# BoloniniD/CSWin-UNet

Hardware: AMD Instinct MI355X
Metric: training images/sec (224x224, cswin_tiny) (higher is better)
Workload: dtype f32; 1 GPU; cswin_tiny_224_lite, synthetic 224x224 9-class, bs=24/GPU, fp32 matmul, fwd + 0.4CE+0.6Dice + bwd + SGD(momentum) step, drop_path 0.2; global_batch=24, img_size=224, parallelism=dp1, hip_graph=True

## Files before the change

### cswin_unet_amd/_lib.py

```python
import ctypes
import os
from ctypes import c_char_p, c_double, c_float, c_int, c_long, c_size_t, c_void_p

import torch

_HERE = os.path.dirname(os.path.abspath(__file__))
LIB_PATH = os.path.join(_HERE, "libcswin_hip.so")

P, I, F, SZ, L, D = c_void_p, c_int, c_float, c_size_t, c_long, c_double

ABI_VERSION = 4

SIGNATURES = {
    "cswin_last_error": (c_char_p, []),
    "cswin_abi_version": (I, []),
    "cswin_device_ok": (I, []),
    "cswin_attn_fwd": (I, [P, P, P, P, P, P, I, I, I, I, P, P, I, F, F, ctypes.c_ulonglong, P, I, P]),
    "cswin_attn_bwd_workspace": (SZ, [I, I, I, I, P, P, I]),
    "cswin_attn_bwd": (I, [P, P, P, P, P, P, P, P, P, P, SZ, I, I, I, I, P, P, I, F, P, F, ctypes.c_ulonglong, P, I, P]),
    "cswin_img2windows": (I, [P, P, I, I, I, I, I, I, P]),
    "cswin_windows2img": (I, [P, P, I, I, I, I, I, I, P]),
    "cswin_layernorm_fwd": (I, [P, P, P, P, P, P, I, I, F, I, P]),
    "cswin_layernorm_bwd_workspace": (SZ, [I, I]),
    "cswin_layernorm_bwd": (I, [P, P, P, P, P, P, P, P, P, P, SZ, I, I, P, P, P]),
    "cswin_linear_fwd": (I, [P, P, I, P, P, P, P, P, P, I, I, I, I, I, I, P]),
    "cswin_linear_bwd_data": (I, [P, P, P, P, I, P, P, I, P, I, I, I, I, I, P]),
    "cswin_linear_bwd_weight_workspace": (SZ, [I, I, I]),
    "cswin_linear_bwd_weight": (I, [P, P, P, I, P, I, P, P, P, SZ, I, I, I, P, I, P]),
    "cswin_linear_bwd_weight_batch": (I, [P, I, P, P, I, P]),
    "cswin_linear_bwd_tail": (I, [P, P, P, I, I, I, P, I, P, P, I, P]),
    "cswin_linear_bwd_weight_batch_masked": (I, [P, I, P, P, I, P, P, P]),
    "cswin_linear_bwd_tail_masked": (I, [P, P, P, I, I, I, P, I, P, P, I, P, P, P]),
    "cswin_rows_sum_multi": (I, [P, I, P]),
    "cswin_conv_tok_fwd": (I, [P, P, P, P, I, I, I, I, I, I, I, I, I, P]),
    "cswin_conv_tok_bwd_data": (I, [P, P, P, I, I, I, I, I, I, I, I, I, P]),
    "cswin_conv_tok_bwd_weight_workspace": (SZ, [I, I, I, I, I, I, I, I]),
    "cswin_conv_tok_bwd_weight": (I, [P, P, P, P, P, SZ, I, I, I, I, I, I, I, I, I, P, I, P]),
    "cswin_conv_weight_permute": (I, [P, P, P, I, I, I, I, P]),
    "cswin_conv_weight_unpermute": (I, [P, P, I, I, I, I, P]),
    "cswin_conv_weight_flipT": (I, [P, P, I, I, I, P]),
    "cswin_conv_weight_images": (I, [P, I, P]),
    "cswin_conv_tok_bwd_weight_cpad": (I, [P, P, P, P, P, SZ, I, I, I, I, I, I, I, I, I, P, I, P]),
    "cswin_nchw_to_tokens": (I, [P, P, I, I, I, I, I, P]),
    "cswin_tokens_to_nchw": (I, [P, P, I, I, I, I, I, P]),
    "cswin_carafe_fwd": (I, [P, P, P, P, P, I, I, I, I, I, P]),
    "cswin_carafe_bwd_workspace": (SZ, [I, I, I, I, I]),
    "cswin_carafe_bwd": (I, [P, P, P, P, P, P, P, SZ, I, I, I, I, I, P, P]),
    "cswin_carafe_fwd_nchw": (I, [P, P, P, P, P, I, I, I, I, I, I, P]),
    "cswin_carafe_bwd_nchw_ok": (I, [I, I, I, I]),
    "cswin_carafe_bwd_nchw": (I, [P, P, P, P, P, P, P, SZ, I, I, I, I, I, I, P, P]),
    "cswin_head_compose": (I, [P, P, P, P, P, I, I, I, I, P]),
    "cswin_head_compose_bwd": (I, [P, P, P, P, P, P, P, P, I, I, I, P]),
    "cswin_loss_workspace": (SZ, [I, I, L]),
    "cswin_loss_sums": (I, [P, P, P, P, SZ, I, I, L, I, P]),
    "cswin_loss_finalize": (I, [P, P, P, D, I, F, F, P, P]),
    "cswin_loss_bwd": (I, [P, P, P, P, P, F, F, I, I, L, I, P]),
    "cswin_cl_loss_workspace": (SZ, [I, I, L]),
    "cswin_cl_loss_sums": (I, [P, P, P, I, P, P, P, P, SZ, I, I, I, L, F, F, F, P]),
    "cswin_cl_loss_finalize": (I, [P, P, P, D, D, I, F, F, F, F, P]),
    "cswin_cl_loss_bwd": (I, [P, P, P, I, P, P, P, P, P, F, F, F, I, I, I, L, F, F, F, P]),
    "cswin_dropout": (I, [P, P, P, P, L, L, F, ctypes.c_ulonglong, P, P]),
    "cswin_sgd_flat": (I, [P, P, P, L, P, F, F, F, P, P]),
    "cswin_multi_copy": (I, [P, I, P]),
    "cswin_chunk_sumsq": (I, [P, P, P, I, P, P]),
    "cswin_norm_finalize": (I, [P, P, I, F, F, P, P, P]),
    "cswin_adamw_flat": (I, [P, P, P, P, P, I, P, P, P, D, D, D, F, F, D, D, P, P]),
    "cswin_rate_finalize": (I, [P, P, I, F, F, P, P, P, I, I, F, P, P, P, P, P]),
    "cswin_adam_flat": (I, [P, P, P, P, P, I, P, P, P, D, D, D, F, F, D, D, I, P, P]),
    "cswin_tpgm_chunk_stats": (I, [P, P, P, P, I, I, P, P]),
    "cswin_tpgm_finalize": (I, [P, P, I, I, P, P, P, P, D, D, D, D, I, P, P, P, P]),
    "cswin_tpgm_project": (I, [P, P, P, P, P, I, P, P]),
    "cswin_eb_tiles": (I, [P, P, I, P, P]),
    "cswin_eb_finalize": (I, [P, P, P, I, P, P]),
    "cswin_pack_bf16": (I, [P, P, L, P]),
    "cswin_pack_bf16_scaled": (I, [P, P, L, F, P]),
    "cswin_unpack_bf16": (I, [P, P, L, P]),
    "cswin_seg_metrics_nbins": (I, [I, I, I]),
    "cswin_seg_metrics_workspace": (SZ, [I, I, I, I, I]),
    "cswin_seg_metrics": (I, [P, P, P, P, P, SZ, I, I, I, I, I, P]),
    "cswin_components_workspace": (SZ, [I, I, I]),
    "cswin_components_label": (I, [P, P, P, P, SZ, I, I, I, I, P]),
    "cswin_components_filter": (I, [P, P, P, P, P, P, P, SZ, I, I, I, I, P]),
    "cswin_resize_banded": (I, [P, P, P, P, I, P, P, I, I, I, I, I, I, I, P]),
    "cswin_argmax_zoom_back": (I, [P, P, P, P, I, I, I, I, I, I, P]),
    "cswin_argmax_zoom_back_classes": (I, [P, P, P, P, P, I, I, I, I, I, I, I, P]),
    "cswin_class_counts": (I, [P, I, P, I, P, I, L, I, P]),
    "cswin_augment_gather": (I, [P, P, P, I, I, I, I, I, I, P]),
    "cswin_augment_labels": (I, [P, P, P, P, P, P, P, I, I, I, I, I, I, P]),
    "cswin_gaussian_blur": (I, [P, P, P, I, I, I, I, P]),
}



class WgradDesc(ctypes.Structure):
    _fields_ = [("dy", c_void_p), ("x", c_void_p), ("row_scale", c_void_p), ("dw", c_void_p), ("dbias", c_void_p),
                ("workspace", c_void_p), ("ws_bytes", c_size_t), ("rows_per_sample", c_int), ("M", c_int), ("N", c_int),
                ("K", c_int), ("precision", c_int), ("io_bf16", c_int)]


class ReduceJob(ctypes.Structure):
    _fields_ = [("part", c_void_p), ("out", c_void_p), ("out2", c_void_p), ("n_first", ctypes.c_longlong),
                ("n", ctypes.c_longlong), ("stride", ctypes.c_longlong), ("rows", c_int), ("reserved", c_int),
                ("conv_kk", c_int), ("conv_cin", c_int)]


class ConvImageJob(ctypes.Structure):
    _fields_ = [("w", c_void_p), ("w_perm", c_void_p), ("w_permT", c_void_p), ("w_flipT", c_void_p), ("Cout", c_int),
                ("Cin", c_int), ("ks", c_int), ("Cpad", c_int)]


class AugmentDesc(ctypes.Structure):
    _fields_ = [("kind", c_int), ("k", c_int), ("axis", c_int), ("src", c_int), ("map", c_void_p)]


_lib = None

PREC_FP32, PREC_BF16 = 0, 1
_state = {"precision": PREC_FP32, "act_bf16": True}


def precision():
    return _state["precision"]


def act_bf16():
    return _state["precision"] == PREC_BF16 and _state["act_bf16"]


def set_act_bf16(on):
    prev = _state["act_bf16"]
    _state["act_bf16"] = bool(on)
    return prev


_shadows = []


class _Shadow:

    def __init__(self, owner_obj, owner, seen):
        import weakref
        self.ref = weakref.ref(owner_obj)
        self.base, self.nbytes, self.seen = owner.data_ptr(), owner.numel() * 4, seen


def register_shadow(owner_obj, owner):
    _shadows[:] = [e for e in _shadows if e.ref() is not None and e.base != owner.data_ptr()]
    _shadows.append(_Shadow(owner_obj, owner, {p.data_ptr(): p._version for p in owner_obj.params}))


def shadow_ptr(w):
    if not _shadows or w is None:
        return None
    a = w.data_ptr()
    for e in _shadows:
        if e.base <= a < e.base + e.nbytes:
            opt = e.ref()
            if opt is None:
                return None
            if e.seen.get(a) != w._version:
                opt.refresh_shadow()
                e.seen.clear()
                e.seen.update({p.data_ptr(): p._version for p in opt.params})
                e.seen[a] = w._version
            return c_void_p(opt.flat_param16.data_ptr() + (a - e.base) // 2)
    return None


def shadows_current(opt):
    if _state["precision"] != PREC_BF16:
        return
    for e in _shadows:
        if e.ref() is opt:
            if any(e.seen.get(p.data_ptr()) != p._version for p in opt.params):
                opt.refresh_shadow()
                e.seen.clear()
                e.seen.update({p.data_ptr(): p._version for p in opt.params})
            return


def set_precision(mode):
    prev = _state["precision"]
    _state["precision"] = int(mode)
    if int(mode) == PREC_BF16 and prev != PREC_BF16:
        for e in _shadows:
            opt = e.ref()
            if opt is not None:
                opt.refresh_shadow()
    return prev


class CswinHipError(RuntimeError):
    pass


def lib():
    global _lib
    if _lib is None:
        if not os.path.exists(LIB_PATH):
            raise CswinHipError(f"{LIB_PATH} not found: build it with `python -c 'import __graft_entry__ as g; g.build()'` "
                                f"(or `make -C cswin_unet_amd/csrc`). There is no fallback path.")
        handle = ctypes.CDLL(LIB_PATH)
        for name, (res, args) in SIGNATURES.items():
            try:
                fn = getattr(handle, name)
            except AttributeError as e:
                raise CswinHipError(f"{LIB_PATH} does not export {name}") from e
            fn.restype, fn.argtypes = res, args
        have = handle.cswin_abi_version()
        if have != ABI_VERSION:
            raise CswinHipError(f"{LIB_PATH} was built for C ABI version {have}, this package binds version {ABI_VERSION}: rebuild it "
                                f"(`make -C cswin_unet_amd/csrc`)")
        _lib = handle
    return _lib


def call(name, *args):
    h = lib()
    rc = getattr(h, name)(*args)
    if rc != 0:
        raise CswinHipError(f"{name} failed ({rc}): {h.cswin_last_error().decode()}")


def ptr(t):
    return None if t is None else c_void_p(t.data_ptr())


def stream():
    return c_void_p(torch.cuda.current_stream().cuda_stream)


def dev_f32(t, what="tensor"):
    if t is None:
        return None
    if not t.is_cuda:
        raise CswinHipError(f"{what} is on {t.device}: the cswin_unet_amd ops run on a HIP device only (no CPU fallback)")
    if t.dtype != torch.float32:
        raise CswinHipError(f"{what} has dtype {t.dtype}; the HIP path computes in fp32")
    return t if t.is_contiguous() else t.contiguous()
```

### cswin_unet_amd/csrc/gemm.hip

```cpp
#include <stdlib.h>

#include <type_traits>
#include "common.h"
#include "gemm_epilogue.h"

int cswin_gemm16(int mode, int epi_mode, const void* A, const void* B, const void* epilogue, int M, int NO, int R, void* stream);
int cswin_wgrad16_batch(const cswin_wgrad_desc* d, int n, const int* splits, const int* rows_per_split, const cswin_reduce_job* pending,
                        int npending, void* stream, long long* stamps);

namespace {

constexpr int BKMAX = 64;

typedef __bf16 bf16x8 __attribute__((ext_vector_type(8)));

#define CSWIN_CHECK_PRECISION(p, who) CSWIN_REQUIRE((p) == 0 || (p) == 1, CSWIN_ERR_UNSUPPORTED, who ": precision %d (0 = fp32, 1 = bf16 operands)", (p))

struct PlainSrc {
    const float* p; long ld; int rows, cols;
    const float* row_scale; int rows_per_sample;
    int bf16;
    static constexpr bool fast_div = false;
    struct Row { const float* base; float s; };
    typedef int Col;
    __device__ Col col(int j) const { return j; }
    __device__ Row row(int i) const {
        Row r;
        r.base = (i < rows) ? p + (long)i * ld : nullptr;
        r.s = (row_scale && i < rows) ? row_scale[i / rows_per_sample] : 1.0f;
        return r;
    }
    __device__ const float* ptr(const Row& r, int j) const { return (r.base && j < cols) ? r.base + j : nullptr; }
};

template <class S> constexpr bool is_plain = std::is_same<S, PlainSrc>::value;
template <class S> __device__ __forceinline__ bool src_is_bf16(const S& s) {
    if constexpr (is_plain<S>) return s.bf16 != 0;
    else return false;
}
template <class S> __device__ __forceinline__ u32x2 src_load4_bf16(const S& s, const float* p) {
    if constexpr (is_plain<S>) return *reinterpret_cast<const u32x2*>(reinterpret_cast<const __bf16*>(s.p) + (p - s.p));
    else return u32x2{0u, 0u};
}
template <class S> __device__ __forceinline__ typename S::Row src_mapped_row(const S& s, int row, float f) {
    typename S::Row r{};
    if constexpr (is_plain<S>) {
        r.base = row >= 0 ? s.p + (long)row * s.ld : nullptr;
        r.s = f;
    }
    return r;
}
template <class S> __device__ __forceinline__ const float* src_row_scale(const S& s) {
    if constexpr (is_plain<S>) return s.row_scale;
    else return nullptr;
}

struct ConcatSrc {
    const float* p0; const float* p1; long ld0, ld1; int rows, cols, c0;
    static constexpr bool fast_div = false;
    struct Row { const float* b0; const float* b1; float s; };
    typedef int Col;
    __device__ Col col(int j) const { return j; }
    __device__ Row row(int i) const {
        Row r;
        r.b0 = (i < rows) ? p0 + (long)i * ld0 : nullptr;
        r.b1 = (i < rows) ? p1 + (long)i * ld1 : nullptr;
        r.s = 1.0f;
        return r;
    }
    __device__ const float* ptr(const Row& r, int j) const {
        if (!r.b0 || j >= cols) return nullptr;
        return j < c0 ? r.b0 + j : r.b1 + (j - c0);
    }
};

template <bool FAST> __device__ __forceinline__ int qdiv(int n, int d, unsigned m) {
    if constexpr (FAST) return fdiv1(n, m);
    else return n / d;
}
struct ConvMagics { unsigned img, w, c, ks, stride; };

template <bool FAST>
struct ConvSrcT {
    const float* x; int B, H, W, C, OH, OW, ks, stride, pad; int rows, cols;
    static constexpr bool fast_div = FAST;
    ConvMagics m;
    struct Row { int b, iy0, ix0; float s; };
    struct Col { int ky, kx, ci; };
    __device__ Row row(int i) const {
        Row r;
        r.s = 1.0f;
        if (i >= rows) { r.b = -1; r.iy0 = r.ix0 = 0; return r; }
        int ohw = OH * OW;
        r.b = qdiv<FAST>(i, ohw, m.img);
        int rem = i - r.b * ohw;
        int oy = qdiv<FAST>(rem, OW, m.w);
        r.iy0 = oy * stride - pad;
        r.ix0 = (rem - oy * OW) * stride - pad;
        return r;
    }
    __device__ Col col(int j) const {
        Col c;
        if (j >= cols) { c.ky = c.kx = 0; c.ci = -1; return c; }
        int tap = qdiv<FAST>(j, C, m.c);
        c.ci = j - tap * C;
        c.ky = qdiv<FAST>(tap, ks, m.ks);
        c.kx = tap - c.ky * ks;
        return c;
    }
    __device__ const float* ptr(const Row& r, const Col& c) const {
        if (r.b < 0 || c.ci < 0) return nullptr;
        int iy = r.iy0 + c.ky, ix = r.ix0 + c.kx;
        if ((unsigned)iy >= (unsigned)H || (unsigned)ix >= (unsigned)W) return nullptr;
        return x + ((long)(r.b * H + iy) * W + ix) * C + c.ci;
    }
};

template <bool FAST>
struct ConvTSrcT {
    const float* dy; int B, H, W, C, OH, OW, ks, stride, pad; int rows, cols;
    static constexpr bool fast_div = FAST;
    ConvMagics m;
    struct Row { int b, iy, ix; float s; };
    struct Col { int ky, kx, co; };
    __device__ Row row(int i) const {
        Row r;
        r.s = 1.0f;
        if (i >= rows) { r.b = -1; r.iy = r.ix = 0; return r; }
        int hw = H * W;
        r.b = qdiv<FAST>(i, hw, m.img);
        int rem = i - r.b * hw;
        r.iy = qdiv<FAST>(rem, W, m.w);
        r.ix = rem - r.iy * W;
        return r;
    }
    __device__ Col col(int j) const {
        Col c;
        if (j >= cols) { c.ky = c.kx = 0; c.co = -1; return c; }
        int tap = qdiv<FAST>(j, C, m.c);
        c.co = j - tap * C;
        c.ky = qdiv<FAST>(tap, ks, m.ks);
        c.kx = tap - c.ky * ks;
        return c;
    }
    __device__ const float* ptr(const Row& r, const Col& c) const {
        if (r.b < 0 || c.co < 0) return nullptr;
        int ty = r.iy + pad - c.ky, tx = r.ix + pad - c.kx;
        if (ty < 0 || tx < 0) return nullptr;
        int oy = qdiv<FAST>(ty, stride, m.stride), ox = qdiv<FAST>(tx, stride, m.stride);
        if (oy * stride != ty || ox * stride != tx || oy >= OH || ox >= OW) return nullptr;
        return dy + ((long)(r.b * OH + oy) * OW + ox) * C + c.co;
    }
};

template <bool FAST>
struct ConvTS2SrcT {
    const float* dy; int B, H, W, C, OH, OW, py, px, H2, W2, kys, kxs; int rows, cols;
    static constexpr bool fast_div = FAST;
    ConvMagics m;
    struct Row { int b, iy, ix; float s; };
    struct Col { int ky, kx, co; };
    __device__ Row row(int i) const {
        Row r;
        r.s = 1.0f;
        if (i >= rows) { r.b = -1; r.iy = r.ix = 0; return r; }
        const int hw = H2 * W2;
        r.b = qdiv<FAST>(i, hw, m.img);
        const int rem = i - r.b * hw;
        const int jy = qdiv<FAST>(rem, W2, m.w);
        r.iy = 2 * jy + py;
        r.ix = 2 * (rem - jy * W2) + px;
        return r;
    }
    __device__ Col col(int j) const {
        Col c;
        if (j >= cols) { c.ky = c.kx = 0; c.co = -1; return c; }
        const int t = qdiv<FAST>(j, C, m.c);
        c.co = j - t * C;
        c.ky = (kys >> (2 * t)) & 3;
        c.kx = (kxs >> (2 * t)) & 3;
        return c;
    }
    __device__ const float* ptr(const Row& r, const Col& c) const {
        if (r.b < 0 || c.co < 0) return nullptr;
        const int oy = (r.iy + 1 - c.ky) >> 1, ox = (r.ix + 1 - c.kx) >> 1;
        if (oy >= OH || ox >= OW) return nullptr;
        return dy + ((long)(r.b * OH + oy) * OW + ox) * C + c.co;
    }
};

template <bool FAST>
struct TapRowsSrcT {
    const float* w; int Cout, Cin, taps; int rows, cols;
    unsigned m_cout;
    struct Row { const float* base; float s; };
    typedef int Col;
    __device__ Row row(int i) const {
        Row r;
        r.s = 1.0f;
        if (i >= rows) { r.base = nullptr; return r; }
        const int t = qdiv<FAST>(i, Cout, m_cout), co = i - t * Cout;
        r.base = w + ((long)((taps >> (4 * t)) & 15) * Cout + co) * Cin;
        return r;
    }
    __device__ Col col(int j) const { return j; }
    __device__ const float* ptr(const Row& r, int j) const { return (r.base && j < cols) ? r.base + j : nullptr; }
};

template <int ROWS, int BK, bool RC_, int NTH>
struct OperandTile {
    static constexpr bool RC = RC_;
    static constexpr int LD = RC ? BK + 4 : ROWS + 4;
    static constexpr int ELEMS = (RC ? ROWS : BK) * LD;
    static constexpr int Q = ROWS * BK / (4 * NTH);
    static constexpr int CPR = RC ? BK / 4 : ROWS / 4;
    static constexpr int RPP = NTH / CPR;
    static_assert(Q >= 1, "tile too small for this many wave groups");
};

template <int BM_, int BN_, int BK_, int KW_, bool A_RC, bool B_RC>
struct Tile {
    static constexpr int BM = BM_, BN = BN_, BK = BK_, KW = KW_;
    static constexpr int WGM = BM >= 64 ? 2 : 1, WGN = BN >= 64 ? 2 : 1, NW = WGM * WGN;
    static constexpr int WM = BM / WGM, WN = BN / WGN;
    static constexpr int FM = WM / 32, FN = WN / 32;
    static constexpr int THREADS = 64 * NW * KW;
    typedef OperandTile<BM, BK, A_RC, THREADS> A;
    typedef OperandTile<BN, BK, B_RC, THREADS> B;
    static constexpr int LD16 = BK + 8;
    static constexpr int PATCH = FM * FN * 16 * 64;
    static constexpr int LDS_FLOATS = A::ELEMS + B::ELEMS > NW * EP_WAVE_FLOATS ? A::ELEMS + B::ELEMS : NW * EP_WAVE_FLOATS;
    static_assert((BK / KW) % 8 == 0, "tile too small for this many wave groups");
    static_assert(KW == 1 || (KW / 2) * NW * PATCH <= LDS_FLOATS, "LDS too small for the k-group reduction");
};

template <bool S16, bool SCALED> __device__ __forceinline__ u32x2 chunk_bf16(const f32x4& v, const u32x2& raw, float s) {
    if constexpr (S16 && !SCALED) return raw;
    else if constexpr (S16) return __builtin_bit_cast(u32x2, __builtin_convertvector(widen_bf16x4(raw) * s, bf16x4));
    else if constexpr (SCALED) return __builtin_bit_cast(u32x2, __builtin_convertvector(v * s, bf16x4));
    else return __builtin_bit_cast(u32x2, __builtin_convertvector(v, bf16x4));
}
template <int LD16> __device__ __forceinline__ void store_a_transposed(unsigned short* img16, int c, int row, u32x2 h) {
    unsigned short* col = &img16[4 * c * LD16 + row];
    col[0] = (unsigned short)(h[0] & 0xffffu);
    col[LD16] = (unsigned short)(h[0] >> 16);
    col[2 * LD16] = (unsigned short)(h[1] & 0xffffu);
    col[3 * LD16] = (unsigned short)(h[1] >> 16);
}
template <int BN> __device__ __forceinline__ void store_b_swizzled(unsigned short* img16, int c, int row, u32x2 h) {
    static_assert(BN == 64, "transposed-read B image is laid out for 64-column tiles");
    *reinterpret_cast<u32x2*>(&img16[row * BN + 8 * ((c >> 1) ^ (((row >> 1) & 1) << 2)) + 4 * (c & 1)]) = h;
}
template <class G, bool IS_A, int PREC, bool S16, bool SCALED, int LD16, int BN>
__device__ __forceinline__ void stash_operand(float* img, unsigned short* img16, int c, int r, const f32x4* p, const u32x2* p16, const float* ps) {
#pragma unroll
    for (int q = 0; q < G::Q; ++q) {
        const int row = r + q * G::RPP;
        float s = 1.0f;
        if constexpr (SCALED) s = ps[q];
        if constexpr (PREC == 1) {
            const u32x2 h = chunk_bf16<S16, SCALED>(p[q], p16[q], s);
            if constexpr (G::RC) *reinterpret_cast<u32x2*>(&img16[row * LD16 + 4 * c]) = h;
            else if constexpr (IS_A) store_a_transposed<LD16>(img16, c, row, h);
            else store_b_swizzled<BN>(img16, c, row, h);
        } else {
            f32x4 v = p[q];
            if constexpr (SCALED) v *= s;
            *reinterpret_cast<f32x4*>(&img[row * G::LD + 4 * c]) = v;
        }
    }
}
struct RowMask { const float* skip; int nsamples, rows_per_sample, splits; unsigned magic; };
constexpr int MASK_MAX_SAMPLES = 256;
struct KeptList { int n; int idx[MASK_MAX_SAMPLES]; float scale[MASK_MAX_SAMPLES]; };

__device__ __forceinline__ void build_kept_list(KeptList* kept, const RowMask& mk, const float* row_scale) {
    const int tid = threadIdx.x, lane = tid & 63;
    if (tid >= 64) return;
    int n = 0;
    for (int s0 = 0; s0 < mk.nsamples; s0 += 64) {
        const int s = s0 + lane;
        const bool keep = s < mk.nsamples && mk.skip[s] != 0.0f;
        const unsigned long long bal = __ballot(keep);
        if (keep) {
            const int at = n + __popcll(bal & ((1ull << lane) - 1ull));
            kept->idx[at] = s;
            kept->scale[at] = row_scale ? row_scale[s] : 1.0f;
        }
        n += __popcll(bal);
    }
    if (tid == 0) kept->n = n;
}

__device__ __forceinline__ void stamp(const Epilogue& epi, int row, int slot) {
    if (!epi.stamps || threadIdx.x != 0) return;
    long long* s = epi.stamps + 8L * row;
    s[slot] = __builtin_amdgcn_s_memtime();
    if (slot == 0) { s[4] = __builtin_amdgcn_s_getreg(6164); s[5] = __builtin_amdgcn_s_memrealtime(); }
    if (slot == 3) s[6] = __builtin_amdgcn_s_memrealtime();
}

template <class T, int VEC, int EPI, bool SCALE_A, int PREC, class ASrc, class BSrc, bool MASKED = false>
__device__ __forceinline__ void gemm_body(float* lds, const ASrc& A, const BSrc& B, const Epilogue& epi, int M, int N, int R,
                                          int r_per_split, int tiles_m, int tiles_n, int bid, int nblk, int stamp_row,
                                          const RowMask* mk = nullptr, KeptList* kept = nullptr) {
    typedef typename T::A TA;
    typedef typename T::B TB;
    constexpr int BM = T::BM, BN = T::BN, BK = T::BK, KW = T::KW, NW = T::NW, FM = T::FM, FN = T::FN, LD16 = T::LD16;
    constexpr bool A_RC = TA::RC, B_RC = TB::RC;
    float* As = lds;
    float* Bs = lds + TA::ELEMS;
    unsigned short* As16 = reinterpret_cast<unsigned short*>(lds);
    unsigned short* Bs16 = As16 + BM * LD16;
    static_assert(PREC == 0 || ((BM + BN) * LD16 * 2 <= T::LDS_FLOATS * 4 && (BK / KW) % 16 == 0), "bf16 tile does not fit");

    const int tid = threadIdx.x, lane = tid & 63, wave = (tid >> 6) % NW, kg = tid / (64 * NW);
    const int li = lane & 31, lh = lane >> 5;
    const int lb = xcd_block_order(bid, nblk);
    const int tiles = tiles_m * tiles_n;
    const int split = lb / tiles;
    const int tile = lb - split * tiles;
    const int m0 = (tile / tiles_n) * BM, n0 = (tile % tiles_n) * BN;
    if constexpr (MASKED) {
        static_assert(!A_RC && !B_RC && VEC == 4 && BM == BN && is_plain<ASrc> && is_plain<BSrc>,
                      "the sample mask serves weight gradients of plain matrices (one row mapping for both operands)");
        build_kept_list(kept, *mk, src_row_scale(A));
        __syncthreads();
        R = __builtin_amdgcn_readfirstlane(kept->n) * mk->rows_per_sample;
        r_per_split = ((R + mk->splits - 1) / mk->splits + 7) / 8 * 8;
    }
    const int r_begin = split * r_per_split;
    const int r_end = min(R, r_begin + r_per_split);
    const int wm0 = (wave / T::WGN) * T::WM, wn0 = (wave % T::WGN) * T::WN;

    const int a_c = tid % TA::CPR, a_r = tid / TA::CPR;
    const int b_c = tid % TB::CPR, b_r = tid / TB::CPR;

    typename ASrc::Row arow[TA::Q];
    typename BSrc::Row brow[TB::Q];
    if (A_RC) {
#pragma unroll
        for (int q = 0; q < TA::Q; ++q) arow[q] = A.row(m0 + a_r + q * TA::RPP);
    }
    if (B_RC) {
#pragma unroll
        for (int q = 0; q < TB::Q; ++q) brow[q] = B.row(n0 + b_r + q * TB::RPP);
    }

    const typename ASrc::Col acol = A.col(m0 + 4 * a_c);
    const typename BSrc::Col bcol = B.col(n0 + 4 * b_c);

    f32x4 pa[TA::Q], pb[TB::Q];
    u32x2 pa16[TA::Q], pb16[TB::Q];
    float pas[TA::Q];
    auto fetch = [&](int r0, auto a16, auto b16) {
        int mrow[TA::Q];
        float msc[TA::Q];
        if constexpr (MASKED) {
#pragma unroll
            for (int q = 0; q < TA::Q; ++q) {
                const int c = r0 + a_r + q * TA::RPP;
                mrow[q] = -1;
                msc[q] = 1.0f;
                if (c < r_end) {
                    const int j = fdiv1(c, mk->magic);
                    mrow[q] = kept->idx[j] * mk->rows_per_sample + (c - j * mk->rows_per_sample);
                    msc[q] = kept->scale[j];
                }
            }
        }
#pragma unroll
        for (int q = 0; q < TA::Q; ++q) {
            typename ASrc::Row rr;
            int j;
            if (A_RC) {
                rr = arow[q];
                j = r0 + 4 * a_c;
            } else {
                const int r = r0 + a_r + q * TA::RPP;
                if constexpr (MASKED) rr = src_mapped_row(A, mrow[q], msc[q]);
                else rr = A.row(r < r_end ? r : 0x7fffffff);
                j = m0 + 4 * a_c;
            }
            if (SCALE_A) pas[q] = rr.s;
            if (VEC == 4) {
                const float* p = A_RC ? (j < r_end ? A.ptr(rr, A.col(j)) : nullptr) : A.ptr(rr, acol);
                if constexpr (decltype(a16)::value) {
                    pa16[q] = u32x2{0u, 0u};
                    if (p) pa16[q] = src_load4_bf16(A, p);
                } else {
                    pa[q] = f32x4{0.f, 0.f, 0.f, 0.f};
                    if (p) pa[q] = *reinterpret_cast<const f32x4*>(p);
                }
            } else {
#pragma unroll
                for (int e = 0; e < 4; ++e) {
                    const float* p = (!A_RC || j + e < r_end) ? A.ptr(rr, A.col(j + e)) : nullptr;
                    pa[q][e] = p ? *p : 0.f;
                }
            }
        }
#pragma unroll
        for (int q = 0; q < TB::Q; ++q) {
            typename BSrc::Row rr;
            int j;
            if (B_RC) {
                rr = brow[q];
                j = r0 + 4 * b_c;
            } else {
                const int r = r0 + b_r + q * TB::RPP;
                if constexpr (MASKED) rr = src_mapped_row(B, mrow[q], 1.0f);
                else rr = B.row(r < r_end ? r : 0x7fffffff);
                j = n0 + 4 * b_c;
            }
            if (VEC == 4) {
                const float* p = B_RC ? (j < r_end ? B.ptr(rr, B.col(j)) : nullptr) : B.ptr(rr, bcol);
                if constexpr (decltype(b16)::value) {
                    pb16[q] = u32x2{0u, 0u};
                    if (p) pb16[q] = src_load4_bf16(B, p);
                } else {
                    pb[q] = f32x4{0.f, 0.f, 0.f, 0.f};
                    if (p) pb[q] = *reinterpret_cast<const f32x4*>(p);
                }
            } else {
#pragma unroll
                for (int e = 0; e < 4; ++e) {
                    const float* p = (!B_RC || j + e < r_end) ? B.ptr(rr, B.col(j + e)) : nullptr;
                    pb[q][e] = p ? *p : 0.f;
                }
            }
        }
    };
    auto stash = [&](auto a16, auto b16) {
        stash_operand<TA, true, PREC, decltype(a16)::value, SCALE_A, LD16, BN>(As, As16, a_c, a_r, pa, pa16, pas);
        stash_operand<TB, false, PREC, decltype(b16)::value, false, LD16, BN>(Bs, Bs16, b_c, b_r, pb, pb16, nullptr);
    };

    f32x16 acc[FM][FN];
#pragma unroll
    for (int i = 0; i < FM; ++i)
#pragma unroll
        for (int j = 0; j < FN; ++j)
#pragma unroll
            for (int e = 0; e < 16; ++e) acc[i][j][e] = 0.f;

    float csum = 0.f;
    const bool do_colsum = !A_RC && epi.colsum && n0 == 0 && tid < BM;

    stamp(epi, stamp_row, 0);
    auto main_loop = [&](auto a16, auto b16) {
        fetch(r_begin, a16, b16);
        stash(a16, b16);
        __syncthreads();
        stamp(epi, stamp_row, 1);
        for (int r0 = r_begin; r0 < r_end; r0 += BK) {
            const bool more = r0 + BK < r_end;
            if (more) fetch(r0 + BK, a16, b16);
            if (do_colsum) {
                if constexpr (PREC == 1) {
#pragma unroll 8
                    for (int r = 0; r < BK; ++r)
                        csum += __builtin_bit_cast(float, (unsigned)As16[tid * LD16 + r] << 16);
                } else {
#pragma unroll 8
                    for (int r = 0; r < BK; ++r) csum += As[r * TA::LD + tid];
                }
            }
            if constexpr (PREC == 1) {
#pragma unroll
                for (int kk = kg * (BK / KW); kk < (kg + 1) * (BK / KW); kk += 16) {
                    bf16x8 af[FM], bf[FN];
#pragma unroll
                    for (int i = 0; i < FM; ++i)
                        af[i] = *reinterpret_cast<const bf16x8*>(&As16[(wm0 + i * 32 + li) * LD16 + kk + 8 * lh]);
#pragma unroll
                    for (int j = 0; j < FN; ++j) {
                        if constexpr (B_RC) {
                            bf[j] = *reinterpret_cast<const bf16x8*>(&Bs16[(wn0 + j * 32 + li) * LD16 + kk + 8 * lh]);
                        } else {
                            typedef short s16x4 __attribute__((ext_vector_type(4)));
                            typedef short s16x8 __attribute__((ext_vector_type(8)));
                            typedef __attribute__((address_space(3))) s16x4 lds_s16x4;
                            const int col = wn0 + j * 32 + 16 * ((lane >> 4) & 1) + 4 * (lane & 3);
                            const int row = kk + 8 * lh + ((lane & 15) >> 2);
                            const int sw = ((row >> 1) & 1) << 2;
                            const unsigned short* a0 = &Bs16[row * BN + 8 * ((col >> 3) ^ sw) + (col & 7)];
                            const s16x4 v0 = __builtin_amdgcn_ds_read_tr16_b64_v4i16((lds_s16x4*)a0);
                            const s16x4 v1 = __builtin_amdgcn_ds_read_tr16_b64_v4i16((lds_s16x4*)(a0 + 4 * BN));
                            const s16x8 f = {v0[0], v0[1], v0[2], v0[3], v1[0], v1[1], v1[2], v1[3]};
                            bf[j] = __builtin_bit_cast(bf16x8, f);
                        }
                    }
#pragma unroll
                    for (int i = 0; i < FM; ++i)
#pragma unroll
                        for (int j = 0; j < FN; ++j)
                            acc[i][j] = __builtin_amdgcn_mfma_f32_32x32x16_bf16(af[i], bf[j], acc[i][j], 0, 0, 0);
                }
            } else
#pragma unroll
            for (int kk = kg * (BK / KW); kk < (kg + 1) * (BK / KW); kk += 8) {
                f32x4 af[FM], bf[FN];
#pragma unroll
                for (int i = 0; i < FM; ++i) {
                    if (A_RC) {
                        af[i] = *reinterpret_cast<const f32x4*>(&As[(wm0 + i * 32 + li) * TA::LD + kk + 4 * lh]);
                    } else {
#pragma unroll
                        for (int s = 0; s < 4; ++s) af[i][s] = As[(kk + 4 * lh + s) * TA::LD + wm0 + i * 32 + li];
                    }
                }
#pragma unroll
                for (int j = 0; j < FN; ++j) {
                    if (B_RC) {
                        bf[j] = *reinterpret_cast<const f32x4*>(&Bs[(wn0 + j * 32 + li) * TB::LD + kk + 4 * lh]);
                    } else {
#pragma unroll
                        for (int s = 0; s < 4; ++s) bf[j][s] = Bs[(kk + 4 * lh + s) * TB::LD + wn0 + j * 32 + li];
                    }
                }
#pragma unroll
                for (int s = 0; s < 4; ++s)
#pragma unroll
                    for (int i = 0; i < FM; ++i)
#pragma unroll
                        for (int j = 0; j < FN; ++j)
                            acc[i][j] = __builtin_amdgcn_mfma_f32_32x32x2f32(af[i][s], bf[j][s], acc[i][j], 0, 0, 0);
            }
            __syncthreads();
            if (more) {
                stash(a16, b16);
                __syncthreads();
            }
        }
    };
    if (r_begin < r_end) {
        constexpr bool CAN_A16 = PREC == 1 && A_RC && VEC == 4 && is_plain<ASrc>;
        constexpr bool CAN_B16 = PREC == 1 && A_RC && VEC == 4 && is_plain<BSrc>;
        const bool a_is16 = CAN_A16 && src_is_bf16(A), b_is16 = CAN_B16 && src_is_bf16(B);
        if constexpr (CAN_A16 && CAN_B16) {
            if (a_is16 && b_is16) main_loop(std::true_type{}, std::true_type{});
            else if (a_is16) main_loop(std::true_type{}, std::false_type{});
            else if (b_is16) main_loop(std::false_type{}, std::true_type{});
            else main_loop(std::false_type{}, std::false_type{});
        } else if constexpr (CAN_B16) {
            if (b_is16) main_loop(std::false_type{}, std::true_type{});
            else main_loop(std::false_type{}, std::false_type{});
        } else {
            main_loop(std::false_type{}, std::false_type{});
        }
    }

    stamp(epi, stamp_row, 2);
    if (KW > 1) {
#pragma unroll
        for (int half = KW / 2; half >= 1; half >>= 1) {
            if (kg >= half && kg < 2 * half) {
                float* dst = lds + ((kg - half) * NW + wave) * T::PATCH + lane;
#pragma unroll
                for (int i = 0; i < FM; ++i)
#pragma unroll
                    for (int j = 0; j < FN; ++j)
#pragma unroll
                        for (int g = 0; g < 16; ++g) dst[((i * FN + j) * 16 + g) * 64] = acc[i][j][g];
            }
            __syncthreads();
            if (kg < half) {
                const float* src = lds + (kg * NW + wave) * T::PATCH + lane;
#pragma unroll
                for (int i = 0; i < FM; ++i)
#pragma unroll
                    for (int j = 0; j < FN; ++j)
#pragma unroll
                        for (int g = 0; g < 16; ++g) acc[i][j][g] += src[((i * FN + j) * 16 + g) * 64];
            }
            __syncthreads();
        }
        if (kg != 0) return;
    }
    Epilogue e = epi;
    e.C += (long)split * e.split_stride;
    if constexpr (EPI == EPI_GELUBWD) {
        if (e.pre_bf16) run_epilogue<EPI, FM, FN, true>(e, acc, M, N, m0 + wm0, n0 + wn0, lane, lds + wave * EP_WAVE_FLOATS, e.vec_store != 0);
        else run_epilogue<EPI, FM, FN, false>(e, acc, M, N, m0 + wm0, n0 + wn0, lane, lds + wave * EP_WAVE_FLOATS, e.vec_store != 0);
    } else {
        if constexpr (ASrc::fast_div)
            run_epilogue<EPI, FM, FN, false, true>(e, acc, M, N, m0 + wm0, n0 + wn0, lane, lds + wave * EP_WAVE_FLOATS, e.vec_store != 0, A.m.img, A.m.w);
        else
            run_epilogue<EPI, FM, FN>(e, acc, M, N, m0 + wm0, n0 + wn0, lane, lds + wave * EP_WAVE_FLOATS, e.vec_store != 0);
    }
    stamp(epi, stamp_row, 3);
    if (do_colsum && m0 + tid < M) epi.colsum[(long)split * epi.colsum_stride + m0 + tid] = csum;
}

template <int BM, int BN, int BK, int KW, bool A_RC, bool B_RC, int VEC, int EPI, bool SCALE_A, int PREC, class ASrc, class BSrc>
__global__ __launch_bounds__((Tile<BM, BN, BK, KW, A_RC, B_RC>::THREADS)) void gemm_kernel(ASrc A, BSrc B, Epilogue epi, int M, int N, int R,
                                                    int r_per_split, int tiles_m, int tiles_n) {
    typedef Tile<BM, BN, BK, KW, A_RC, B_RC> T;
    __shared__ __attribute__((aligned(16))) float lds[T::LDS_FLOATS];
    gemm_body<T, VEC, EPI, SCALE_A, PREC, ASrc, BSrc>(lds, A, B, epi, M, N, R, r_per_split, tiles_m, tiles_n, (int)blockIdx.x, (int)gridDim.x,
                                                      (int)blockIdx.x);
}

constexpr int WGRAD_BATCH = 4;
template <class ASrc, class BSrc>
struct GemmBatch {
    ASrc A[WGRAD_BATCH];
    BSrc B[WGRAD_BATCH];
    Epilogue e[WGRAD_BATCH];
    int M[WGRAD_BATCH], N[WGRAD_BATCH], R[WGRAD_BATCH], rps[WGRAD_BATCH], tm[WGRAD_BATCH], tn[WGRAD_BATCH];
    int first[WGRAD_BATCH + 1];
    int n;
    RowMask mask[WGRAD_BATCH];
};
typedef GemmBatch<PlainSrc, PlainSrc> WgradBatch;

template <class ASrc, class BSrc> __device__ __forceinline__ int batch_problem(const GemmBatch<ASrc, BSrc>& b, int bid) {
    int p = 0;
    while (p + 1 < b.n && bid >= b.first[p + 1]) ++p;
    return p;
}
template <class T, bool SCALE_A, int PREC, bool MASKED = false, class ASrc, class BSrc>
__device__ __forceinline__ void batch_body(float* lds, const GemmBatch<ASrc, BSrc>& b, int p, int bid, KeptList* kept = nullptr) {
    gemm_body<T, 4, EPI_PLAIN, SCALE_A, PREC, ASrc, BSrc, MASKED>(lds, b.A[p], b.B[p], b.e[p], b.M[p], b.N[p], b.R[p], b.rps[p], b.tm[p], b.tn[p],
                                                                  bid - b.first[p], b.first[p + 1] - b.first[p], bid, MASKED ? &b.mask[p] : nullptr, kept);
}

typedef Tile<64, 64, 64, 2, false, false> WgradTile;
template <int PREC, bool MASKED>
__device__ __forceinline__ void wgrad_batch_body(float* lds, KeptList* kept, const WgradBatch& b, int bid) {
    const int p = batch_problem(b, bid);
    if constexpr (MASKED) {
        if (b.mask[p].skip) return batch_body<WgradTile, true, PREC, true>(lds, b, p, bid, kept);
    }
    batch_body<WgradTile, true, PREC>(lds, b, p, bid);
}

template <int PREC>
__global__ __launch_bounds__(WgradTile::THREADS) void gemm_wgrad_batch_kernel(WgradBatch b) {
    __shared__ __attribute__((aligned(16))) float lds[WgradTile::LDS_FLOATS];
    wgrad_batch_body<PREC, false>(lds, nullptr, b, (int)blockIdx.x);
}
__global__ __launch_bounds__(WgradTile::THREADS) void gemm_wgrad_batch_masked_kernel(WgradBatch b) {
    __shared__ __attribute__((aligned(16))) float lds[WgradTile::LDS_FLOATS];
    __shared__ KeptList kept;
    wgrad_batch_body<0, true>(lds, &kept, b, (int)blockIdx.x);
}

struct BlockTail {
    PlainSrc dA, dB;
    Epilogue de;
    int dM, dN, dR, drps, dtm, dtn, nd;
    WgradBatch w;
    ReduceRiders r;
};
typedef Tile<64, 64, 64, 2, true, false> TailDgradTile;
static_assert(TailDgradTile::THREADS == WgradTile::THREADS, "one workgroup size for both halves of the block tail");
constexpr int BLOCK_TAIL_LDS = TailDgradTile::LDS_FLOATS > WgradTile::LDS_FLOATS ? TailDgradTile::LDS_FLOATS : WgradTile::LDS_FLOATS;
template <bool MASKED>
__device__ __forceinline__ void block_tail_body(float (&lds)[BLOCK_TAIL_LDS], KeptList* kept, const BlockTail& t) {
    const int bid = (int)blockIdx.x, nw = t.w.first[t.w.n];
    if (bid >= nw + t.nd) {
        if (threadIdx.x >= 256) return;
        static_assert(sizeof(lds) >= sizeof(float) * RS_G * (RS_COLS + 1), "reduction scratch");
        rows_sum_dispatch(t.r.j, t.r.first_block, t.r.njobs, bid - nw - t.nd, reinterpret_cast<float(*)[RS_COLS + 1]>(lds));
        return;
    }
    if (bid >= nw) {
        gemm_body<TailDgradTile, 4, EPI_PLAIN, false, 0, PlainSrc, PlainSrc>(lds, t.dA, t.dB, t.de, t.dM, t.dN, t.dR, t.drps, t.dtm, t.dtn, bid - nw,
                                                                             t.nd, bid);
        return;
    }
    wgrad_batch_body<0, MASKED>(lds, kept, t.w, bid);
}
__global__ __launch_bounds__(WgradTile::THREADS) void gemm_block_tail_kernel(BlockTail t) {
    __shared__ __attribute__((aligned(16))) float lds[BLOCK_TAIL_LDS];
    block_tail_body<false>(lds, nullptr, t);
}
__global__ __launch_bounds__(WgradTile::THREADS) void gemm_block_tail_masked_kernel(BlockTail t) {
    __shared__ __attribute__((aligned(16))) float lds[BLOCK_TAIL_LDS];
    __shared__ KeptList kept;
    block_tail_body<true>(lds, &kept, t);
}

template <int KW> using S2DgradTile = Tile<64, 64, (KW == 1 ? 32 : 64), KW, true, false>;
template <int KW, int PREC, bool FAST>
__global__ __launch_bounds__(S2DgradTile<KW>::THREADS) void gemm_conv_s2_dgrad_batch_kernel(GemmBatch<ConvTS2SrcT<FAST>, TapRowsSrcT<FAST>> b) {
    __shared__ __attribute__((aligned(16))) float lds[S2DgradTile<KW>::LDS_FLOATS];
    batch_body<S2DgradTile<KW>, false, PREC>(lds, b, batch_problem(b, (int)blockIdx.x), (int)blockIdx.x);
}

template <int BM, int BN, int BK, int KW, bool A_RC, bool B_RC, int VEC, int EPI, bool SCALE_A, int PREC, class ASrc, class BSrc>
void launch_cfg(const ASrc& A, const BSrc& B, const Epilogue& epi, int M, int N, int R, int splits, int r_per_split,
                hipStream_t st) {
    int tm = cdiv(M, BM), tn = cdiv(N, BN);
    dim3 grid(tm * tn * splits);
    const int pad_lds = cswin_tuning().gemm_pad_lds;
    hipLaunchKernelGGL((gemm_kernel<BM, BN, BK, KW, A_RC, B_RC, VEC, EPI, SCALE_A, PREC, ASrc, BSrc>), grid, dim3((Tile<BM, BN, BK, KW, A_RC, B_RC>::THREADS)), pad_lds, st, A, B, epi,
                       M, N, R, r_per_split, tm, tn);
}

int k_groups(long blocks, int r_len) {
    if (blocks < 320 && r_len >= 512) return 4;
    if (blocks < 640 && r_len >= 256) return 2;
    return 1;
}

int one_split(int R) { return cdiv(R, BKMAX) * BKMAX; }

template <bool A_RC, bool B_RC, int VEC, int EPI, bool SCALE_A, class ASrc, class BSrc>
void launch_gemm(const ASrc& A, const BSrc& B, const Epilogue& epi_in, int M, int N, int R, int splits, int r_per_split,
                 int precision, hipStream_t st) {
    Epilogue epi = epi_in;
    epi.vec_store = epilogue_vec_ok(epi, N);
    auto blocks = [&](int bm, int bn) { return (long)cdiv(M, bm) * cdiv(N, bn) * splits; };
    const int forced_kw = cswin_tuning().gemm_kw;
    const int forced_tile = cswin_tuning().gemm_tile;
    const double pen2 = cswin_tuning().gemm_pen2;
    auto cost = [&](int bm, int bn, double pen) { return (double)((blocks(bm, bn) + 255) / 256) * bm * bn * pen; };
    int tile = 1;
    if (splits == 1 && cost(64, 32, pen2) < cost(64, 64, 1.0)) tile = 2;
    if (forced_tile) tile = forced_tile;
    const int r_len = r_per_split < R ? r_per_split : R;
    const bool wgrad = !A_RC && !B_RC;
    if (precision == 1) {
        if (k_groups(blocks(64, 64), r_len) >= 2 || (wgrad && r_len >= 256))
            launch_cfg<64, 64, 64, 2, A_RC, B_RC, VEC, EPI, SCALE_A, 1>(A, B, epi, M, N, R, splits, r_per_split, st);
        else launch_cfg<64, 64, 64, 1, A_RC, B_RC, VEC, EPI, SCALE_A, 1>(A, B, epi, M, N, R, splits, r_per_split, st);
        return;
    }
    if (tile == 2) {
        if (k_groups(blocks(64, 32), r_len) >= 2)
            return launch_cfg<64, 32, 64, 2, A_RC, B_RC, VEC, EPI, SCALE_A, 0>(A, B, epi, M, N, R, splits, r_per_split, st);
        return launch_cfg<64, 32, 32, 1, A_RC, B_RC, VEC, EPI, SCALE_A, 0>(A, B, epi, M, N, R, splits, r_per_split, st);
    }
    int kw = k_groups(blocks(64, 64), r_len);
    if (wgrad && r_len >= 256 && kw < 2) kw = 2;
    if (forced_kw) kw = forced_kw;
    if (kw == 4) launch_cfg<64, 64, 64, 4, A_RC, B_RC, VEC, EPI, SCALE_A, 0>(A, B, epi, M, N, R, splits, r_per_split, st);
    else if (kw == 2) launch_cfg<64, 64, 64, 2, A_RC, B_RC, VEC, EPI, SCALE_A, 0>(A, B, epi, M, N, R, splits, r_per_split, st);
    else launch_cfg<64, 64, 32, 1, A_RC, B_RC, VEC, EPI, SCALE_A, 0>(A, B, epi, M, N, R, splits, r_per_split, st);
}

template <bool A_RC, bool B_RC, int EPI, bool SCALE_A, class ASrc, class BSrc>
void launch_gemm_vec(bool vec, const ASrc& A, const BSrc& B, const Epilogue& epi, int M, int N, int R, int splits, int r_per_split,
                     int precision, hipStream_t st) {
    if (vec) launch_gemm<A_RC, B_RC, 4, EPI, SCALE_A>(A, B, epi, M, N, R, splits, r_per_split, precision, st);
    else launch_gemm<A_RC, B_RC, 1, EPI, SCALE_A>(A, B, epi, M, N, R, splits, r_per_split, precision, st);
}

long long* g_stamps = nullptr;

Epilogue plain_epilogue(float* C, long ldc) {
    Epilogue e = {};
    e.C = C;
    e.ldc = ldc;
    e.stamps = g_stamps;
    return e;
}

template <class ASrc, class BSrc>
void push(GemmBatch<ASrc, BSrc>& b, const ASrc& A, const BSrc& B, Epilogue e, int M, int N, int R, int rps, int splits) {
    const int i = b.n++;
    e.vec_store = epilogue_vec_ok(e, N);
    b.A[i] = A; b.B[i] = B; b.e[i] = e;
    b.M[i] = M; b.N[i] = N; b.R[i] = R; b.rps[i] = rps;
    b.tm[i] = cdiv(M, 64); b.tn[i] = cdiv(N, 64);
    b.first[i + 1] = b.first[i] + b.tm[i] * b.tn[i] * splits;
}

void choose_split(int M, int out_rows, int out_cols, int* splits, int* r_per_split, int target_override = 0) {
    const int target_env = cswin_tuning().gemm_split_wgs;
    const int target = target_override > 0 ? target_override : target_env;
    long tiles = (long)cdiv(out_rows, 64) * cdiv(out_cols, 64);
    int s = (int)(target / tiles);
    if (s < 1) s = 1;
    int max_s = cdiv(M, 2 * BKMAX);
    if (s > max_s) s = max_s;
    if (s < 1) s = 1;
    int rps = cdiv(cdiv(M, s), 8) * 8;
    *splits = cdiv(M, rps);
    *r_per_split = rps;
}

struct WgradSlabs {
    float* base; long stride; int N, K;
    WgradSlabs(void* workspace, int N_, int K_) : base((float*)workspace), stride(wgrad_slab_stride(N_, K_)), N(N_), K(K_) {}
    static size_t bytes(int M, int N, int K) {
        int s0, s1, rps;
        choose_split(M, N, K, &s0, &rps);
        choose_split(M, N, K, &s1, &rps, 1024);
        return (size_t)(s0 > s1 ? s0 : s1) * wgrad_slab_stride(N, K) * sizeof(float);
    }
    Epilogue epilogue(bool with_dbias) const {
        Epilogue e = plain_epilogue(base, K);
        e.split_stride = stride;
        e.colsum = with_dbias ? base + (long)N * K : nullptr;
        e.colsum_stride = (int)stride;
        return e;
    }
    cswin_reduce_job job(float* dw, float* dbias, int splits, int conv_kk = 0, int conv_cin = 0) const {
        const long nk = (long)N * K;
        return cswin_reduce_job{base, dw, dbias, nk, nk + (dbias ? N : 0), stride, splits, 0, conv_kk, conv_cin};
    }
};

int rows_sum_multi(const cswin_reduce_job* jobs, int njobs, void* stream) {
    CSWIN_REQUIRE(jobs && njobs > 0 && njobs <= CSWIN_MAX_REDUCE_JOBS, CSWIN_ERR_SHAPE, "rows_sum_multi: 1..%d jobs", CSWIN_MAX_REDUCE_JOBS);
    ReduceJobs J = {};
    const int blocks = fill_reduce_table(jobs, njobs, J.j, J.first_block);
    CSWIN_REQUIRE(blocks >= 0, CSWIN_ERR_SHAPE, "rows_sum_multi: bad job (part / out / n / rows, or conv_kk without conv_cin)");
    J.njobs = njobs;
    hipLaunchKernelGGL(rows_sum_multi_kernel, dim3(blocks), dim3(256), 0, (hipStream_t)stream, J);
    CSWIN_LAUNCH_CHECK();
    return CSWIN_OK;
}

int wgrad_tiled(const float* dy, const float* x, const float* x2, int k_split, const float* row_scale, int rows_per_sample, float* dw,
                float* dbias, void* workspace, int M, int N, int K, cswin_reduce_job* deferred, int precision, hipStream_t st) {
    int splits, rps;
    choose_split(M, N, K, &splits, &rps);
    const WgradSlabs slabs(workspace, N, K);
    const Epilogue e = slabs.epilogue(dbias != nullptr);
    PlainSrc A = {dy, N, M, N, row_scale, rows_per_sample};
    if (x2) {
        ConcatSrc B = {x, x2, k_split, K - k_split, M, K, k_split};
        bool vec = (N % 4 == 0) && (K % 4 == 0) && (k_split % 4 == 0) && aligned16(dy) && aligned16(x) && aligned16(x2);
        launch_gemm_vec<false, false, EPI_PLAIN, true>(vec, A, B, e, N, K, M, splits, rps, precision, st);
    } else {
        PlainSrc B = {x, K, M, K, nullptr, 1};
        bool vec = (N % 4 == 0) && (K % 4 == 0) && aligned16(dy) && aligned16(x);
        if (row_scale) launch_gemm_vec<false, false, EPI_PLAIN, true>(vec, A, B, e, N, K, M, splits, rps, precision, st);
        else launch_gemm_vec<false, false, EPI_PLAIN, false>(vec, A, B, e, N, K, M, splits, rps, precision, st);
    }
    CSWIN_LAUNCH_CHECK();
    reduce_now_or_defer(slabs.job(dw, dbias, splits), deferred, st);
    CSWIN_LAUNCH_CHECK();
    return CSWIN_OK;
}

bool wgrad_aligned(const cswin_wgrad_desc& p) {
    return p.N % 4 == 0 && p.K % 4 == 0 && aligned16(p.dy) && aligned16(p.x) && aligned16(p.workspace);
}

struct TailExtras {
    const char* who; const float* dy; const float* w; float* dx; int M, N, K; const cswin_reduce_job* jobs; int njobs;
    const float* const* skip; const int* nsamples;
};

int wgrad_batch_impl(const cswin_wgrad_desc* d, int n, cswin_reduce_job* deferred, const TailExtras& x, void* stream) {
    CSWIN_REQUIRE(x.njobs >= 0 && x.njobs <= CSWIN_TAIL_RIDER_JOBS && (x.njobs == 0 || x.jobs), CSWIN_ERR_SHAPE,
                  "%s: 0..%d pending reductions", x.who, CSWIN_TAIL_RIDER_JOBS);
    CSWIN_REQUIRE(d && deferred && n >= 1 && n <= WGRAD_BATCH, CSWIN_ERR_SHAPE, "linear_bwd_weight_batch: 1..%d problems and their deferred slots", WGRAD_BATCH);
    bool fast = true, any_bf16 = false, any_mask = false;
    const int precision = d[0].precision;
    CSWIN_CHECK_PRECISION(precision, "linear_bwd_weight_batch");
    for (int i = 0; i < n; ++i) {
        CSWIN_REQUIRE(d[i].precision == precision, CSWIN_ERR_UNSUPPORTED, "linear_bwd_weight_batch: problems of one launch share one precision");
        CSWIN_REQUIRE(d[i].io_bf16 == 0 || (precision == 1 && (d[i].io_bf16 & ~3) == 0), CSWIN_ERR_UNSUPPORTED, "linear_bwd_weight_batch: bf16 storage needs precision 1");
        CSWIN_REQUIRE(d[i].dy && d[i].x && d[i].dw && d[i].M > 0 && d[i].N > 0 && d[i].K > 0, CSWIN_ERR_SHAPE, "linear_bwd_weight_batch: bad problem %d", i);
        CSWIN_REQUIRE(!d[i].row_scale || d[i].rows_per_sample > 0, CSWIN_ERR_SHAPE, "linear_bwd_weight_batch: rows_per_sample must be > 0");
        size_t need = WgradSlabs::bytes(d[i].M, d[i].N, d[i].K);
        CSWIN_REQUIRE(d[i].workspace && d[i].ws_bytes >= need, CSWIN_ERR_WORKSPACE, "linear_bwd_weight_batch: workspace %zu < %zu", d[i].ws_bytes, need);
        fast = fast && wgrad_aligned(d[i]);
        any_bf16 = any_bf16 || d[i].io_bf16;
        if (x.skip && x.skip[i]) {
            any_mask = true;
            CSWIN_REQUIRE(precision == 0, CSWIN_ERR_UNSUPPORTED, "%s: a sample mask needs precision 0", x.who);
            CSWIN_REQUIRE(x.nsamples && x.nsamples[i] >= 1 && x.nsamples[i] <= MASK_MAX_SAMPLES, CSWIN_ERR_SHAPE,
                          "%s: problem %d's mask must have 1..%d samples", x.who, i, MASK_MAX_SAMPLES);
            CSWIN_REQUIRE(d[i].rows_per_sample > 0 && (long)x.nsamples[i] * d[i].rows_per_sample == d[i].M, CSWIN_ERR_SHAPE,
                          "%s: problem %d's mask: nsamples * rows_per_sample != M", x.who, i);
            CSWIN_REQUIRE(fdiv_exact(d[i].M, d[i].rows_per_sample), CSWIN_ERR_UNSUPPORTED,
                          "%s: problem %d's mask: M * rows_per_sample must stay below 2^32", x.who, i);
        }
    }
    CSWIN_REQUIRE(!any_mask || fast, CSWIN_ERR_ALIGN, "%s: a sample mask needs N, K multiples of 4 and 16-B aligned operands", x.who);
    const bool has_dgrad = x.dy != nullptr, extra = has_dgrad || x.njobs > 0;
    const PlainSrc gA = {x.dy, x.N, x.M, x.N, nullptr, 1, 0}, gB = {x.w, x.K, x.N, x.K, nullptr, 1, 0};
    const bool g_vec = x.N % 4 == 0 && x.K % 4 == 0 && aligned16(x.dy) && aligned16(x.w);
    const bool merge_on = cswin_tuning().gemm_tail_merge != 0;
    const bool ride = extra && merge_on && fast && precision == 0 && (!has_dgrad || (g_vec && aligned16(x.dx)));
    const bool w16_path = fast && precision == 1 && (cswin_tuning().wgrad16_on || any_bf16);
    const bool jobs_ride16 = merge_on && w16_path && x.njobs > 0;
    if (extra && !ride) {
        if (has_dgrad) {
            launch_gemm_vec<true, false, EPI_PLAIN, false>(g_vec, gA, gB, plain_epilogue(x.dx, x.K), x.M, x.K, x.N, 1, one_split(x.N), precision,
                                                           (hipStream_t)stream);
            CSWIN_LAUNCH_CHECK();
        }
        if (x.njobs > 0 && !jobs_ride16) {
            int rc = rows_sum_multi(x.jobs, x.njobs, stream);
            if (rc) return rc;
        }
    }
    if (!fast) {
        for (int i = 0; i < n; ++i) CSWIN_REQUIRE(d[i].io_bf16 == 0, CSWIN_ERR_ALIGN, "linear_bwd_weight_batch: bf16 storage needs N, K multiples of 4 and 16-B alignment");
        const TailExtras none = {x.who};
        for (int i = 0; i < n; ++i) {
            int rc = precision == 1 && wgrad_aligned(d[i])
                         ? wgrad_batch_impl(&d[i], 1, &deferred[i], none, stream)
                         : wgrad_tiled(d[i].dy, d[i].x, nullptr, 0, d[i].row_scale, d[i].rows_per_sample, d[i].dw, d[i].dbias, d[i].workspace,
                                       d[i].M, d[i].N, d[i].K, &deferred[i], precision, (hipStream_t)stream);
            if (rc) return rc;
        }
        return CSWIN_OK;
    }
    if (w16_path) {
        int splits[WGRAD_BATCH], rps[WGRAD_BATCH];
        double work_total = 0.0;
        for (int i = 0; i < n; ++i) work_total += (double)d[i].M * cdiv(d[i].N, 128) * cdiv(d[i].K, 128);
        for (int i = 0; i < n; ++i) {
            const int M = d[i].M, N = d[i].N, K = d[i].K;
            const WgradSlabs slabs(d[i].workspace, N, K);
            const int tiles = cdiv(N, 128) * cdiv(K, 128);
            const int w16_wgs = cswin_tuning().w16_wgs, w16_even = cswin_tuning().w16_even;
            int s = w16_even ? (w16_wgs / n) / tiles : (int)(w16_wgs * ((double)M * tiles / work_total) / tiles + 0.5);
            const int cap = (int)(d[i].ws_bytes / (slabs.stride * (long)sizeof(float)));
            if (s > cap) s = cap;
            if (s > M / 64) s = M / 64;
            if (s < 1) s = 1;
            rps[i] = cdiv(cdiv(M, s), 32) * 32;
            splits[i] = cdiv(M, rps[i]);
            deferred[i] = slabs.job(d[i].dw, d[i].dbias, splits[i]);
        }
        CSWIN_REQUIRE(cswin_wgrad16_batch(d, n, splits, rps, jobs_ride16 ? x.jobs : nullptr, jobs_ride16 ? x.njobs : 0, stream, g_stamps) == 0,
                      CSWIN_ERR_SHAPE, "linear_bwd_weight_batch: bad pending reduction");
        CSWIN_LAUNCH_CHECK();
        return CSWIN_OK;
    }
    WgradBatch b = {};
    for (int i = 0; i < n; ++i) {
        const int M = d[i].M, N = d[i].N, K = d[i].K;
        int splits, rps;
        const int batch_env = cswin_tuning().gemm_batch_wgs;
        const int batch_even = cswin_tuning().gemm_batch_even;
        const int total_wgs = batch_env > 0 ? (batch_env < 1024 ? batch_env : 1024) * n : 1024;
        int batch_target = total_wgs / n;
        if (!batch_even) {
            double work = 0.0;
            for (int j = 0; j < n; ++j) work += (double)d[j].M * cdiv(d[j].N, 64) * cdiv(d[j].K, 64);
            batch_target = (int)(total_wgs * ((double)M * cdiv(N, 64) * cdiv(K, 64) / work) + 0.5);
            if (batch_target > 1024) batch_target = 1024;
            if (batch_target < 1) batch_target = 1;
        }
        choose_split(M, N, K, &splits, &rps, batch_target);
        const WgradSlabs slabs(d[i].workspace, N, K);
        CSWIN_REQUIRE((size_t)splits * slabs.stride * sizeof(float) <= d[i].ws_bytes, CSWIN_ERR_WORKSPACE,
                      "linear_bwd_weight_batch: %d slabs do not fit problem %d's workspace", splits, i);
        push(b, PlainSrc{d[i].dy, N, M, N, d[i].row_scale, d[i].row_scale ? d[i].rows_per_sample : 1},
             PlainSrc{d[i].x, K, M, K, nullptr, 1}, slabs.epilogue(d[i].dbias != nullptr), N, K, M, rps, splits);
        deferred[i] = slabs.job(d[i].dw, d[i].dbias, splits);
        if (x.skip && x.skip[i]) b.mask[i] = RowMask{x.skip[i], x.nsamples[i], d[i].rows_per_sample, splits, fdiv_magic(d[i].rows_per_sample)};
    }
    const int blocks = b.first[n];
    if (ride) {
        BlockTail t = {};
        if (has_dgrad) {
            t.dA = gA; t.dB = gB;
            t.de = plain_epilogue(x.dx, x.K);
            t.de.vec_store = epilogue_vec_ok(t.de, x.K);
            t.dM = x.M; t.dN = x.K; t.dR = x.N; t.drps = one_split(x.N);
            t.dtm = cdiv(x.M, 64); t.dtn = cdiv(x.K, 64);
            t.nd = t.dtm * t.dtn;
        }
        t.w = b;
        int rblocks = 0;
        if (x.njobs > 0) {
            rblocks = fill_reduce_table(x.jobs, x.njobs, t.r.j, t.r.first_block);
            CSWIN_REQUIRE(rblocks >= 0, CSWIN_ERR_SHAPE, "linear_bwd_tail: bad pending reduction");
            t.r.njobs = x.njobs;
        }
        static_assert(sizeof(BlockTail) <= 4096, "kernel argument block");
        if (any_mask) hipLaunchKernelGGL(gemm_block_tail_masked_kernel, dim3(blocks + t.nd + rblocks), dim3(512), 0, (hipStream_t)stream, t);
        else hipLaunchKernelGGL(gemm_block_tail_kernel, dim3(blocks + t.nd + rblocks), dim3(512), 0, (hipStream_t)stream, t);
    } else if (any_mask) {
        hipLaunchKernelGGL(gemm_wgrad_batch_masked_kernel, dim3(blocks), dim3(512), 0, (hipStream_t)stream, b);
    } else if (precision == 1) {
        hipLaunchKernelGGL(gemm_wgrad_batch_kernel<1>, dim3(blocks), dim3(512), 0, (hipStream_t)stream, b);
    } else {
        hipLaunchKernelGGL(gemm_wgrad_batch_kernel<0>, dim3(blocks), dim3(512), 0, (hipStream_t)stream, b);
    }
    CSWIN_LAUNCH_CHECK();
    return CSWIN_OK;
}

bool conv_magics(ConvMagics* m, long nrows, int img, int w, long ncols, int c, int ks, int cmax, int stride) {
    *m = ConvMagics{fdiv_magic(img), fdiv_magic(w), fdiv_magic(c), fdiv_magic(ks), fdiv_magic(stride)};
    return fdiv_exact(nrows + 63, img) && fdiv_exact(img - 1, w) && fdiv_exact(ncols - 1, c) && fdiv_exact((long)ks * ks - 1, ks) &&
           (stride == 0 || fdiv_exact(cmax, stride));
}
template <class F> void with_fast_div(bool fast, F f) {
    if (fast) f(std::true_type{});
    else f(std::false_type{});
}

int conv_wgrad_impl(const float* dy, const float* x, float* dw_perm, float* dbias, void* workspace, size_t ws_bytes, int B, int H,
                    int W, int Cin, int Cout, int ks, int stride, int pad, int torch_layout, int Cin_param,
                    cswin_reduce_job* deferred, int precision, void* stream) {
    CSWIN_CHECK_PRECISION(precision, "conv_tok_bwd_weight");
    CSWIN_REQUIRE(dy && x && dw_perm, CSWIN_ERR_SHAPE, "conv_tok_bwd_weight: null pointer");
    CSWIN_REQUIRE(Cin % 4 == 0 && Cout % 4 == 0 && aligned16(dy) && aligned16(x), CSWIN_ERR_ALIGN, "conv_tok_bwd_weight: channels %% 4 and 16-B alignment required");
    CSWIN_REQUIRE(!torch_layout || Cin < 65536, CSWIN_ERR_UNSUPPORTED, "conv_tok_bwd_weight: torch_layout needs Cin < 65536");
    int OH = (H + 2 * pad - ks) / stride + 1, OW = (W + 2 * pad - ks) / stride + 1;
    int M = B * OH * OW, K = ks * ks * Cin;
    size_t need = WgradSlabs::bytes(M, Cout, K);
    CSWIN_REQUIRE(workspace && ws_bytes >= need, CSWIN_ERR_WORKSPACE, "conv_tok_bwd_weight: workspace %zu < %zu", ws_bytes, need);
    hipStream_t st = (hipStream_t)stream;
    int splits, rps;
    choose_split(M, Cout, K, &splits, &rps);
    const WgradSlabs slabs(workspace, Cout, K);
    PlainSrc A = {dy, Cout, M, Cout, nullptr, 1};
    ConvMagics mg;
    with_fast_div(conv_magics(&mg, M, OH * OW, OW, K, Cin, ks, 0, 0), [&](auto fast) {
        ConvSrcT<decltype(fast)::value> Bm = {x, B, H, W, Cin, OH, OW, ks, stride, pad, M, K, mg};
        launch_gemm<false, false, 4, EPI_PLAIN, false>(A, Bm, slabs.epilogue(dbias != nullptr), Cout, K, M, splits, rps, precision, st);
    });
    CSWIN_LAUNCH_CHECK();
    reduce_now_or_defer(slabs.job(dw_perm, dbias, splits, torch_layout ? ks * ks : 0,
                                  torch_layout ? (Cin | (Cin_param != Cin ? Cin_param << 16 : 0)) : 0), deferred, st);
    CSWIN_LAUNCH_CHECK();
    return CSWIN_OK;
}

}

extern "C" {

void cswin_debug_set_stamps(void* p) { g_stamps = (long long*)p; }

int cswin_linear_bwd_weight_batch_masked(const cswin_wgrad_desc* d, int n, cswin_reduce_job* deferred, const cswin_reduce_job* pending,
                                         int npending, const float* const* skip, const int* nsamples, void* stream);
int cswin_linear_bwd_tail_masked(const float* dy, const float* w, float* dx, int M, int N, int K, const cswin_wgrad_desc* d, int n,
                                 cswin_reduce_job* deferred, const cswin_reduce_job* pending, int npending, const float* const* skip,
                                 const int* nsamples, void* stream);

int cswin_linear_fwd(const float* x, const float* x2, int k_split, const float* w, const float* bias, float* y,
                     float* y_act, const float* residual, const float* row_scale, int rows_per_sample, int M, int N,
                     int K, int precision, int io_bf16, void* stream) {
    CSWIN_CHECK_PRECISION(precision, "linear_fwd");
    CSWIN_REQUIRE(io_bf16 == 0 || (precision == 1 && (!x2 || !(io_bf16 & 1)) && (io_bf16 & ~7) == 0 && K % 4 == 0 && N % 4 == 0 && !((io_bf16 & 2) && residual)), CSWIN_ERR_UNSUPPORTED,
                  "linear_fwd: bf16 storage (io_bf16 = %d: 1 = x, 2 = y / y_act, 4 = w) needs precision 1, a plain input for bit 1, K and N multiples of 4; a residual output stays fp32", io_bf16);
    CSWIN_REQUIRE(x && w && y && M > 0 && N > 0 && K > 0, CSWIN_ERR_SHAPE, "linear_fwd: bad arguments M=%d N=%d K=%d", M, N, K);
    CSWIN_REQUIRE(!x2 || (k_split > 0 && k_split < K), CSWIN_ERR_SHAPE, "linear_fwd: bad concat split %d of K=%d", k_split, K);
    CSWIN_REQUIRE(!row_scale || rows_per_sample > 0, CSWIN_ERR_SHAPE, "linear_fwd: rows_per_sample must be > 0");
    hipStream_t st = (hipStream_t)stream;
    Epilogue e = plain_epilogue(y, N);
    e.bias = bias;
    e.Cact = y_act; e.ldact = N;
    e.residual = residual; e.ldres = N;
    e.row_scale = row_scale; e.rows_per_sample = rows_per_sample;
    e.c_bf16 = (io_bf16 & 2) != 0;
    PlainSrc B = {w, K, N, K, nullptr, 1, (io_bf16 >> 2) & 1};
    CSWIN_REQUIRE(!(y_act && residual), CSWIN_ERR_UNSUPPORTED, "linear_fwd: activation and residual epilogues are exclusive");
    const int rk = one_split(K);
    if (x2) {
        CSWIN_REQUIRE(!y_act, CSWIN_ERR_UNSUPPORTED, "linear_fwd: concat input does not support the activation epilogue");
        ConcatSrc A = {x, x2, k_split, K - k_split, M, K, k_split};
        bool vec = (k_split % 4 == 0) && (K % 4 == 0) && aligned16(x) && aligned16(x2) && aligned16(w);
        CSWIN_REQUIRE(io_bf16 == 0 || (io_bf16 == 4 && vec), CSWIN_ERR_UNSUPPORTED, "linear_fwd: a concat input takes only the bf16 weight flag (4), with 16-B aligned operands");
        if (residual) launch_gemm_vec<true, true, EPI_RES, false>(vec, A, B, e, M, N, K, 1, rk, precision, st);
        else launch_gemm_vec<true, true, EPI_PLAIN, false>(vec, A, B, e, M, N, K, 1, rk, precision, st);
    } else {
        if (precision == 1 && (io_bf16 & 5) == 5) {
            if (cswin_gemm16(0, y_act ? EPI_ACT : (residual ? EPI_RES : EPI_PLAIN), x, w, &e, M, N, K, stream) == 0) {
                CSWIN_LAUNCH_CHECK();
                return CSWIN_OK;
            }
        }
        PlainSrc A = {x, K, M, K, nullptr, 1, io_bf16 & 1};
        bool vec = (K % 4 == 0) && aligned16(x) && aligned16(w);
        CSWIN_REQUIRE(io_bf16 == 0 || (vec && aligned16(y) && (!y_act || aligned16(y_act)) && (!bias || aligned16(bias))), CSWIN_ERR_ALIGN,
                      "linear_fwd: bf16 storage needs 16-B aligned operands");
        if (y_act) launch_gemm_vec<true, true, EPI_ACT, false>(vec, A, B, e, M, N, K, 1, rk, precision, st);
        else if (residual) launch_gemm_vec<true, true, EPI_RES, false>(vec, A, B, e, M, N, K, 1, rk, precision, st);
        else launch_gemm_vec<true, true, EPI_PLAIN, false>(vec, A, B, e, M, N, K, 1, rk, precision, st);
    }
    CSWIN_LAUNCH_CHECK();
    return CSWIN_OK;
}

int cswin_linear_bwd_data(const float* dy, const float* w, float* dx, float* dx2, int k_split, const float* gelu_pre,
                          const float* row_scale, int rows_per_sample, const float* add, int M, int N, int K,
                          int precision, int io_bf16, void* stream) {
    CSWIN_CHECK_PRECISION(precision, "linear_bwd_data");
    CSWIN_REQUIRE(io_bf16 == 0 || (precision == 1 && ((!dx2 && !add) || (io_bf16 & ~4) == 0) && (io_bf16 & ~15) == 0 && K % 4 == 0 && N % 4 == 0), CSWIN_ERR_UNSUPPORTED,
                  "linear_bwd_data: bf16 storage (io_bf16 = %d: 1 = dy, 2 = dx, 4 = w, 8 = gelu_pre) needs precision 1, K and N multiples of 4; split / add outputs take only the weight flag", io_bf16);
    CSWIN_REQUIRE(dy && w && dx && M > 0 && N > 0 && K > 0, CSWIN_ERR_SHAPE, "linear_bwd_data: bad arguments");
    CSWIN_REQUIRE(!dx2 || (k_split > 0 && k_split < K), CSWIN_ERR_SHAPE, "linear_bwd_data: bad concat split");
    CSWIN_REQUIRE(!row_scale || rows_per_sample > 0, CSWIN_ERR_SHAPE, "linear_bwd_data: rows_per_sample must be > 0");
    hipStream_t st = (hipStream_t)stream;
    Epilogue e = plain_epilogue(dx, dx2 ? k_split : K);
    e.C2 = dx2; e.ldc2 = K - k_split; e.col_split = dx2 ? k_split : 0;
    e.gelu_pre = gelu_pre; e.ldpre = K;
    e.row_scale = row_scale; e.rows_per_sample = rows_per_sample;
    e.residual = add; e.ldres = K;
    e.c_bf16 = (io_bf16 & 2) != 0;
    e.pre_bf16 = (io_bf16 & 8) != 0;
    CSWIN_REQUIRE(io_bf16 == 0 || (aligned16(dy) && aligned16(w) && aligned16(dx) && (!gelu_pre || aligned16(gelu_pre))), CSWIN_ERR_ALIGN,
                  "linear_bwd_data: bf16 storage needs 16-B aligned operands");
    PlainSrc A = {dy, N, M, N, nullptr, 1, io_bf16 & 1};
    PlainSrc B = {w, K, N, K, nullptr, 1, (io_bf16 >> 2) & 1};
    bool vec = (N % 4 == 0) && (K % 4 == 0) && aligned16(dy) && aligned16(w);
    const int rn = one_split(N);
    const int modes = (dx2 != nullptr) + (gelu_pre != nullptr) + (add != nullptr);
    CSWIN_REQUIRE(modes <= 1, CSWIN_ERR_UNSUPPORTED, "linear_bwd_data: dx2 / gelu_pre / add are mutually exclusive");
    if (precision == 1 && !dx2 && !add && (io_bf16 & 5) == 5) {
        if (cswin_gemm16(1, gelu_pre ? EPI_GELUBWD : EPI_PLAIN, dy, w, &e, M, K, N, stream) == 0) {
            CSWIN_LAUNCH_CHECK();
            return CSWIN_OK;
        }
    }
    if (dx2) launch_gemm_vec<true, false, EPI_SPLIT2, false>(vec, A, B, e, M, K, N, 1, rn, precision, st);
    else if (gelu_pre) launch_gemm_vec<true, false, EPI_GELUBWD, false>(vec, A, B, e, M, K, N, 1, rn, precision, st);
    else if (add) launch_gemm_vec<true, false, EPI_RES, false>(vec, A, B, e, M, K, N, 1, rn, precision, st);
    else launch_gemm_vec<true, false, EPI_PLAIN, false>(vec, A, B, e, M, K, N, 1, rn, precision, st);
    CSWIN_LAUNCH_CHECK();
    return CSWIN_OK;
}

size_t cswin_linear_bwd_weight_workspace(int M, int N, int K) { return WgradSlabs::bytes(M, N, K); }

int cswin_linear_bwd_weight(const float* dy, const float* x, const float* x2, int k_split, const float* row_scale,
                            int rows_per_sample, float* dw, float* dbias, void* workspace, size_t ws_bytes, int M,
                            int N, int K, cswin_reduce_job* deferred, int precision, void* stream) {
    CSWIN_CHECK_PRECISION(precision, "linear_bwd_weight");
    CSWIN_REQUIRE(dy && x && dw && M > 0 && N > 0 && K > 0, CSWIN_ERR_SHAPE, "linear_bwd_weight: bad arguments");
    CSWIN_REQUIRE(!x2 || (k_split > 0 && k_split < K), CSWIN_ERR_SHAPE, "linear_bwd_weight: bad concat split");
    CSWIN_REQUIRE(!row_scale || rows_per_sample > 0, CSWIN_ERR_SHAPE, "linear_bwd_weight: rows_per_sample must be > 0");
    size_t need = WgradSlabs::bytes(M, N, K);
    CSWIN_REQUIRE(workspace && ws_bytes >= need, CSWIN_ERR_WORKSPACE, "linear_bwd_weight: workspace %zu < %zu", ws_bytes, need);
    hipStream_t st = (hipStream_t)stream;
    const cswin_wgrad_desc d1 = {dy, x, row_scale, dw, dbias, workspace, ws_bytes, rows_per_sample, M, N, K, precision, 0};
    if (precision == 1 && !x2 && wgrad_aligned(d1)) {
        cswin_reduce_job job;
        int rc = wgrad_batch_impl(&d1, 1, &job, TailExtras{"linear_bwd_weight_batch"}, stream);
        if (rc) return rc;
        reduce_now_or_defer(job, deferred, st);
        CSWIN_LAUNCH_CHECK();
        return CSWIN_OK;
    }
    return wgrad_tiled(dy, x, x2, k_split, row_scale, rows_per_sample, dw, dbias, workspace, M, N, K, deferred, precision, st);
}

int cswin_linear_bwd_weight_batch(const cswin_wgrad_desc* d, int n, cswin_reduce_job* deferred, const cswin_reduce_job* pending, int npending,
                                  void* stream) {
    return cswin_linear_bwd_weight_batch_masked(d, n, deferred, pending, npending, nullptr, nullptr, stream);
}

int cswin_linear_bwd_weight_batch_masked(const cswin_wgrad_desc* d, int n, cswin_reduce_job* deferred, const cswin_reduce_job* pending,
                                         int npending, const float* const* skip, const int* nsamples, void* stream) {
    return wgrad_batch_impl(d, n, deferred,
                            TailExtras{"linear_bwd_weight_batch", nullptr, nullptr, nullptr, 0, 0, 0, pending, npending, skip, nsamples}, stream);
}

int cswin_linear_bwd_tail(const float* dy, const float* w, float* dx, int M, int N, int K, const cswin_wgrad_desc* d, int n,
                          cswin_reduce_job* deferred, const cswin_reduce_job* pending, int npending, void* stream) {
    return cswin_linear_bwd_tail_masked(dy, w, dx, M, N, K, d, n, deferred, pending, npending, nullptr, nullptr, stream);
}

int cswin_linear_bwd_tail_masked(const float* dy, const float* w, float* dx, int M, int N, int K, const cswin_wgrad_desc* d, int n,
                                 cswin_reduce_job* deferred, const cswin_reduce_job* pending, int npending, const float* const* skip,
                                 const int* nsamples, void* stream) {
    CSWIN_REQUIRE(dy && w && dx && M > 0 && N > 0 && K > 0, CSWIN_ERR_SHAPE, "linear_bwd_tail: bad data-gradient arguments");
    return wgrad_batch_impl(d, n, deferred, TailExtras{"linear_bwd_tail", dy, w, dx, M, N, K, pending, npending, skip, nsamples}, stream);
}

int cswin_conv_tok_fwd(const float* x, const float* w_perm, const float* bias, float* y, int B, int H, int W, int Cin,
                       int Cout, int ks, int stride, int pad, int precision, void* stream) {
    CSWIN_CHECK_PRECISION(precision, "conv_tok_fwd");
    CSWIN_REQUIRE(x && w_perm && y && B > 0 && H > 0 && W > 0 && Cin > 0 && Cout > 0, CSWIN_ERR_SHAPE, "conv_tok_fwd: bad arguments");
    CSWIN_REQUIRE(Cin % 4 == 0 && aligned16(x) && aligned16(w_perm), CSWIN_ERR_ALIGN, "conv_tok_fwd: Cin %% 4 and 16-B alignment required");
    int OH = (H + 2 * pad - ks) / stride + 1, OW = (W + 2 * pad - ks) / stride + 1;
    int M = B * OH * OW, R = ks * ks * Cin;
    PlainSrc Bm = {w_perm, R, Cout, R, nullptr, 1};
    Epilogue e = plain_epilogue(y, Cout);
    e.bias = bias;
    ConvMagics mg;
    with_fast_div(conv_magics(&mg, M, OH * OW, OW, R, Cin, ks, 0, 0), [&](auto fast) {
        ConvSrcT<decltype(fast)::value> A = {x, B, H, W, Cin, OH, OW, ks, stride, pad, M, R, mg};
        launch_gemm<true, true, 4, EPI_PLAIN, false>(A, Bm, e, M, Cout, R, 1, one_split(R), precision, (hipStream_t)stream);
    });
    CSWIN_LAUNCH_CHECK();
    return CSWIN_OK;
}

int cswin_conv_tok_bwd_data(const float* dy, const float* w_permT, float* dx, int B, int H, int W, int Cin, int Cout,
                            int ks, int stride, int pad, int precision, void* stream) {
    CSWIN_CHECK_PRECISION(precision, "conv_tok_bwd_data");
    CSWIN_REQUIRE(dy && w_permT && dx, CSWIN_ERR_SHAPE, "conv_tok_bwd_data: null pointer");
    CSWIN_REQUIRE(Cin % 4 == 0 && Cout % 4 == 0 && aligned16(dy) && aligned16(w_permT), CSWIN_ERR_ALIGN, "conv_tok_bwd_data: channels %% 4 and 16-B alignment required");
    int OH = (H + 2 * pad - ks) / stride + 1, OW = (W + 2 * pad - ks) / stride + 1;
    if (ks == 3 && stride == 2 && pad == 1) {
        bool fast_ok = true;
        for (int py = 0; py < 2; ++py)
            for (int px = 0; px < 2; ++px) {
                const int H2 = (H - py + 1) / 2, W2 = (W - px + 1) / 2;
                ConvMagics mg;
                if (H2 > 0 && W2 > 0) fast_ok = fast_ok && conv_magics(&mg, (long)B * H2 * W2, H2 * W2, W2, 4L * Cout, Cout, 1, 0, 0);
            }
        with_fast_div(fast_ok, [&](auto fast) {
            constexpr bool FAST = decltype(fast)::value;
            GemmBatch<ConvTS2SrcT<FAST>, TapRowsSrcT<FAST>> b = {};
            int rmax = 0;
            for (int py = 0; py < 2; ++py)
                for (int px = 0; px < 2; ++px) {
                    const int H2 = (H - py + 1) / 2, W2 = (W - px + 1) / 2;
                    if (H2 <= 0 || W2 <= 0) continue;
                    int kys = 0, kxs = 0, taps = 0, nt = 0;
                    for (int ky = (py ? 0 : 1); ky < 3; ky += 2)
                        for (int kx = (px ? 0 : 1); kx < 3; kx += 2) {
                            kys |= ky << (2 * nt);
                            kxs |= kx << (2 * nt);
                            taps |= (ky * 3 + kx) << (4 * nt);
                            ++nt;
                        }
                    const int Mc = B * H2 * W2, Rc = nt * Cout;
                    Epilogue e = plain_epilogue(dx, Cin);
                    e.rm_on = 1; e.rm_H = H; e.rm_W = W; e.rm_H2 = H2; e.rm_W2 = W2; e.rm_py = py; e.rm_px = px;
                    ConvMagics mg;
                    conv_magics(&mg, Mc, H2 * W2, W2, Rc, Cout, 1, 0, 0);
                    push(b, ConvTS2SrcT<FAST>{dy, B, H, W, Cout, OH, OW, py, px, H2, W2, kys, kxs, Mc, Rc, mg},
                         TapRowsSrcT<FAST>{w_permT, Cout, Cin, taps, Rc, Cin, mg.c}, e, Mc, Cin, Rc, one_split(Rc), 1);
                    rmax = Rc > rmax ? Rc : rmax;
                }
            if (b.n > 0) {
                const int blocks = b.first[b.n];
                hipStream_t st = (hipStream_t)stream;
                const int kw = k_groups(blocks, rmax);
                if (precision == 1) hipLaunchKernelGGL((gemm_conv_s2_dgrad_batch_kernel<2, 1, FAST>), dim3(blocks), dim3(512), 0, st, b);
                else if (kw == 4) hipLaunchKernelGGL((gemm_conv_s2_dgrad_batch_kernel<4, 0, FAST>), dim3(blocks), dim3(1024), 0, st, b);
                else if (kw == 2) hipLaunchKernelGGL((gemm_conv_s2_dgrad_batch_kernel<2, 0, FAST>), dim3(blocks), dim3(512), 0, st, b);
                else hipLaunchKernelGGL((gemm_conv_s2_dgrad_batch_kernel<1, 0, FAST>), dim3(blocks), dim3(256), 0, st, b);
            }
        });
        CSWIN_LAUNCH_CHECK();
        return CSWIN_OK;
    }
    int M = B * H * W, R = ks * ks * Cout;
    PlainSrc Bm = {w_permT, Cin, R, Cin, nullptr, 1};
    Epilogue e = plain_epilogue(dx, Cin);
    ConvMagics mg;
    with_fast_div(conv_magics(&mg, M, H * W, W, R, Cout, ks, (H > W ? H : W) + pad, stride), [&](auto fast) {
        ConvTSrcT<decltype(fast)::value> A = {dy, B, H, W, Cout, OH, OW, ks, stride, pad, M, R, mg};
        launch_gemm<true, false, 4, EPI_PLAIN, false>(A, Bm, e, M, Cin, R, 1, one_split(R), precision, (hipStream_t)stream);
    });
    CSWIN_LAUNCH_CHECK();
    return CSWIN_OK;
}

size_t cswin_conv_tok_bwd_weight_workspace(int B, int H, int W, int Cin, int Cout, int ks, int stride, int pad) {
    int OH = (H + 2 * pad - ks) / stride + 1, OW = (W + 2 * pad - ks) / stride + 1;
    return WgradSlabs::bytes(B * OH * OW, Cout, ks * ks * Cin);
}

int cswin_conv_tok_bwd_weight(const float* dy, const float* x, float* dw_perm, float* dbias, void* workspace,
                              size_t ws_bytes, int B, int H, int W, int Cin, int Cout, int ks, int stride, int pad,
                              int torch_layout, cswin_reduce_job* deferred, int precision, void* stream) {
    return conv_wgrad_impl(dy, x, dw_perm, dbias, workspace, ws_bytes, B, H, W, Cin, Cout, ks, stride, pad, torch_layout, Cin, deferred,
                           precision, stream);
}

int cswin_conv_tok_bwd_weight_cpad(const float* dy, const float* x, float* dw, float* dbias, void* workspace, size_t ws_bytes,
                                   int B, int H, int W, int Cin, int Cin_param, int Cout, int ks, int stride, int pad,
                                   cswin_reduce_job* deferred, int precision, void* stream) {
    CSWIN_REQUIRE(Cin_param > 0 && Cin_param <= Cin && Cin < 65536, CSWIN_ERR_SHAPE, "conv_tok_bwd_weight_cpad: 0 < Cin_param <= Cin < 65536");
    return conv_wgrad_impl(dy, x, dw, dbias, workspace, ws_bytes, B, H, W, Cin, Cout, ks, stride, pad, 1, Cin_param, deferred, precision,
                           stream);
}

int cswin_rows_sum_multi(const cswin_reduce_job* jobs, int njobs, void* stream) { return rows_sum_multi(jobs, njobs, stream); }

}
```

### cswin_unet_amd/csrc/gemm_epilogue.h

```cpp
#pragma once
#include "common.h"

namespace {

__device__ __forceinline__ f32x4 widen_bf16x4(u32x2 raw) {
    return f32x4{__builtin_bit_cast(float, raw[0] << 16), __builtin_bit_cast(float, raw[0] & 0xffff0000u),
                 __builtin_bit_cast(float, raw[1] << 16), __builtin_bit_cast(float, raw[1] & 0xffff0000u)};
}
__device__ __forceinline__ void epi_store4(float* base, long idx, f32x4 v, int bf16) {
    if (bf16) *reinterpret_cast<bf16x4*>(reinterpret_cast<__bf16*>(base) + idx) = __builtin_convertvector(v, bf16x4);
    else *reinterpret_cast<f32x4*>(base + idx) = v;
}

enum { EPI_PLAIN = 0, EPI_ACT = 1, EPI_RES = 2, EPI_GELUBWD = 3, EPI_SPLIT2 = 4 };

struct Epilogue {
    float* C; long ldc;
    float* C2; long ldc2; int col_split;
    const float* bias;
    float* Cact; long ldact;
    const float* residual; long ldres;
    const float* row_scale; int rows_per_sample;
    const float* gelu_pre; long ldpre;
    long split_stride;
    float* colsum; int colsum_stride;
    int rm_on, rm_H, rm_W, rm_H2, rm_W2, rm_py, rm_px;
    int vec_store;
    int c_bf16;
    int pre_bf16;
    long long* stamps;
};

constexpr int EP_LD = 36;
constexpr int EP_WAVE_FLOATS = 32 * EP_LD;

template <int EPI, int FM, int FN, bool PRE16 = false, bool FDIV = false>
__device__ __forceinline__ void run_epilogue(const Epilogue& e, f32x16 (&acc)[FM][FN], int M, int N, int mb, int nb,
                                             int lane, float* wbuf, bool vec, unsigned m_hw = 0, unsigned m_w2 = 0) {
    const int li = lane & 31, lh = lane >> 5;
    const int rrow = lane >> 3, rcol = (lane & 7) * 4;
    const bool has_rs = e.row_scale != nullptr;
    auto out_row = [&](int m) -> long {
        if (!e.rm_on) return m;
        const int hw = e.rm_H2 * e.rm_W2;
        int b, jy;
        if constexpr (FDIV) { b = fdiv1(m, m_hw); jy = fdiv1(m - b * hw, m_w2); }
        else { b = m / hw; jy = (m - b * hw) / e.rm_W2; }
        const int rem = m - b * hw;
        return ((long)b * e.rm_H + 2 * jy + e.rm_py) * e.rm_W + 2 * (rem - jy * e.rm_W2) + e.rm_px;
    };
#pragma unroll
    for (int i = 0; i < FM; ++i) {
#pragma unroll
        for (int j = 0; j < FN; ++j) {
#pragma unroll
            for (int g = 0; g < 16; ++g) wbuf[((g & 3) + 8 * (g >> 2) + 4 * lh) * EP_LD + li] = acc[i][j][g];
            __builtin_amdgcn_fence(__ATOMIC_RELEASE, "wavefront");
            __builtin_amdgcn_wave_barrier();
            __builtin_amdgcn_fence(__ATOMIC_ACQUIRE, "wavefront");
            const int n = nb + j * 32 + rcol;
            if (vec) {
                f32x4 bias_v = {0.f, 0.f, 0.f, 0.f};
                if (e.bias && n < N) bias_v = *reinterpret_cast<const f32x4*>(e.bias + n);
                f32x4 v[4], aux[4];
                u32x2 aux16[4];
                float rs[4];
#pragma unroll
                for (int p = 0; p < 4; ++p) {
                    const int m = mb + i * 32 + rrow + 8 * p;
                    const bool ok = m < M && n < N;
                    v[p] = *reinterpret_cast<const f32x4*>(&wbuf[(rrow + 8 * p) * EP_LD + rcol]);
                    rs[p] = (has_rs && ok) ? e.row_scale[m / e.rows_per_sample] : 1.0f;
                    if (EPI == EPI_RES || EPI == EPI_GELUBWD) {
                        const float* ap = EPI == EPI_RES ? e.residual : e.gelu_pre;
                        const long ld = EPI == EPI_RES ? e.ldres : e.ldpre;
                        aux[p] = f32x4{0.f, 0.f, 0.f, 0.f};
                        aux16[p] = u32x2{0u, 0u};
                        if (ok) {
                            if constexpr (PRE16) aux16[p] = *reinterpret_cast<const u32x2*>(reinterpret_cast<const __bf16*>(ap) + (long)m * ld + n);
                            else aux[p] = *reinterpret_cast<const f32x4*>(ap + (long)m * ld + n);
                        }
                    }
                }
#pragma unroll
                for (int p = 0; p < 4; ++p) {
                    const int m = mb + i * 32 + rrow + 8 * p;
                    if (m >= M || n >= N) continue;
                    f32x4 o = v[p] + bias_v;
                    if (EPI == EPI_GELUBWD) {
                        const f32x4 pre = PRE16 ? widen_bf16x4(aux16[p]) : aux[p];
#pragma unroll
                        for (int c = 0; c < 4; ++c) o[c] *= gelu_grad_f(pre[c]);
                    }
                    if (has_rs) o *= rs[p];
                    if (EPI == EPI_RES) o += aux[p];
                    if (EPI == EPI_SPLIT2 && n >= e.col_split)
                        *reinterpret_cast<f32x4*>(e.C2 + (long)m * e.ldc2 + (n - e.col_split)) = o;
                    else
                        epi_store4(e.C, out_row(m) * e.ldc + n, o, e.c_bf16);
                    if (EPI == EPI_ACT) {
                        f32x4 a;
#pragma unroll
                        for (int c = 0; c < 4; ++c) a[c] = gelu_f(o[c]);
                        epi_store4(e.Cact, (long)m * e.ldact + n, a, e.c_bf16);
                    }
                }
            } else {
#pragma unroll
                for (int p = 0; p < 4; ++p) {
                    const int m = mb + i * 32 + rrow + 8 * p;
                    if (m >= M) continue;
                    const float rsv = has_rs ? e.row_scale[m / e.rows_per_sample] : 1.0f;
#pragma unroll
                    for (int c = 0; c < 4; ++c) {
                        const int nn = n + c;
                        if (nn >= N) continue;
                        float o = wbuf[(rrow + 8 * p) * EP_LD + rcol + c] + (e.bias ? e.bias[nn] : 0.f);
                        if (EPI == EPI_GELUBWD) o *= gelu_grad_f(e.gelu_pre[(long)m * e.ldpre + nn]);
                        o *= rsv;
                        if (EPI == EPI_RES) o += e.residual[(long)m * e.ldres + nn];
                        if (EPI == EPI_SPLIT2 && nn >= e.col_split) e.C2[(long)m * e.ldc2 + (nn - e.col_split)] = o;
                        else e.C[out_row(m) * e.ldc + nn] = o;
                        if (EPI == EPI_ACT) e.Cact[(long)m * e.ldact + nn] = gelu_f(o);
                    }
                }
            }
            __builtin_amdgcn_fence(__ATOMIC_RELEASE, "wavefront");
            __builtin_amdgcn_wave_barrier();
        }
    }
}


inline bool aligned16(const void* p) { return (reinterpret_cast<uintptr_t>(p) & 15) == 0; }

inline int epilogue_vec_ok(const Epilogue& e, int n_out) {
    auto ok = [](const void* p, long ld) { return !p || (aligned16(p) && ld % 4 == 0); };
    return n_out % 4 == 0 && aligned16(e.C) && e.ldc % 4 == 0 && ok(e.C2, e.ldc2) && (!e.C2 || e.col_split % 4 == 0) &&
           ok(e.bias, 4) && ok(e.Cact, e.ldact) && ok(e.residual, e.ldres) && ok(e.gelu_pre, e.ldpre) &&
           e.split_stride % 4 == 0;
}

}
```

### cswin_unet_amd/networks/cswin_unet.py

```python
import math

import numpy as np
import torch
import torch.nn as nn
import torch.utils.checkpoint as checkpoint

from .. import ops
from ..layers import DropPath, TokenRearrange, trunc_normal_


def _square_side(n_tokens):
    side = int(math.isqrt(n_tokens))
    if side * side != n_tokens:
        raise ValueError(f"token count {n_tokens} is not a square map")
    return side


class Mlp(nn.Module):
    def __init__(self, in_features, hidden_features=None, out_features=None, act_layer=nn.GELU, drop=0.):
        super().__init__()
        out_features = out_features or in_features
        hidden_features = hidden_features or in_features
        self.fc1 = nn.Linear(in_features, hidden_features)
        self.act = act_layer()
        self.fc2 = nn.Linear(hidden_features, out_features)
        self.drop = nn.Dropout(drop)
        if not isinstance(self.act, nn.GELU) or getattr(self.act, "approximate", "none") != "none":
            raise NotImplementedError("the HIP Mlp kernel fuses the exact (erf) GELU only")

    def forward(self, x, residual=None, row_scale=None):
        p = self.drop.p if self.training else 0.0
        return ops.mlp(x, self.fc1.weight, self.fc1.bias, self.fc2.weight, self.fc2.bias, residual, row_scale, drop_p=p)


class LePEAttention(nn.Module):

    def __init__(self, dim, resolution, idx, split_size, dim_out=None, num_heads=9, attn_drop=0., proj_drop=0.,
                 qk_scale=None):
        super().__init__()
        if idx not in (-1, 0, 1):
            raise ValueError(f"ERROR MODE {idx}")
        self.dim, self.dim_out = dim, dim_out or dim
        self.resolution, self.split_size, self.num_heads, self.idx = resolution, split_size, num_heads, idx
        self.scale = qk_scale or (dim // num_heads) ** -0.5
        self.H_sp = resolution if idx in (-1, 0) else split_size
        self.W_sp = resolution if idx in (-1, 1) else split_size
        self.get_v = nn.Conv2d(dim, dim, kernel_size=3, stride=1, padding=1, groups=dim)
        self.attn_drop = nn.Dropout(attn_drop)

    def forward(self, qkv):
        q, k, v = qkv[0], qkv[1], qkv[2]
        if q.shape[1] != self.resolution * self.resolution:
            raise AssertionError("flatten img_tokens has wrong size")
        packed = torch.cat([q, k, v], dim=-1)
        return ops.stripe_attention(packed, self.resolution, self.split_size, [self.idx], [self.num_heads],
                                    [self.get_v.weight], [self.get_v.bias], self.scale,
                                    attn_drop=self.attn_drop.p if self.training else 0.0)


class CSWinBlock(nn.Module):
    def __init__(self, dim, reso, num_heads, split_size, mlp_ratio=4., qkv_bias=False, qk_scale=None, drop=0.,
                 attn_drop=0., drop_path=0., act_layer=nn.GELU, norm_layer=nn.LayerNorm, last_stage=False):
        super().__init__()
        self.dim, self.num_heads, self.patches_resolution = dim, num_heads, reso
        self.split_size, self.mlp_ratio = split_size, mlp_ratio
        self.qkv = nn.Linear(dim, dim * 3, bias=qkv_bias)
        self.norm1 = norm_layer(dim)
        single = last_stage or reso == split_size
        self.branch_num = 1 if single else 2
        self.proj = nn.Linear(dim, dim)
        self.proj_drop = nn.Dropout(drop)
        bdim, bheads = (dim, num_heads) if single else (dim // 2, num_heads // 2)
        self.attns = nn.ModuleList(
            LePEAttention(bdim, resolution=reso, idx=(-1 if single else i), split_size=split_size, num_heads=bheads,
                          dim_out=bdim, qk_scale=qk_scale, attn_drop=attn_drop, proj_drop=drop)
            for i in range(self.branch_num))
        self.drop_path = DropPath(drop_path) if drop_path > 0. else nn.Identity()
        self.mlp = Mlp(in_features=dim, hidden_features=int(dim * mlp_ratio), out_features=dim, act_layer=act_layer,
                       drop=drop)
        self.norm2 = norm_layer(dim)

    def _keep_scales(self, x):
        dp = self.drop_path
        if isinstance(dp, DropPath) and self.training and dp.drop_prob > 0.:
            preset = getattr(self, "_dp_preset", None)
            if preset:
                return preset[0], preset[1]
            return dp.sample_scale(x.shape[0], x.device), dp.sample_scale(x.shape[0], x.device)
        return None, None

    def forward(self, x):
        B, L, C = x.shape
        if L != self.patches_resolution ** 2:
            raise AssertionError("flatten img_tokens has wrong size")
        a = self.attns
        ad = a[0].attn_drop.p if self.training else 0.0
        if type(self.norm1) is not nn.LayerNorm or type(self.norm2) is not nn.LayerNorm:
            raise NotImplementedError("the HIP block fuses nn.LayerNorm only")
        rs1, rs2 = self._keep_scales(x)
        if self.training and (self.proj_drop.p > 0 or self.mlp.drop.p > 0):
            n1, n2 = self.norm1, self.norm2
            qkv = ops.linear(ops.layer_norm(x, n1.weight, n1.bias, n1.eps), self.qkv.weight, self.qkv.bias)
            att = ops.stripe_attention(qkv, self.patches_resolution, self.split_size, [m.idx for m in a], [m.num_heads for m in a],
                                       [m.get_v.weight for m in a], [m.get_v.bias for m in a], a[0].scale, attn_drop=ad)
            x = ops.dropout(ops.linear(att, self.proj.weight, self.proj.bias), self.proj_drop.p, residual=x, row_scale=rs1)
            return self.mlp(ops.layer_norm(x, n2.weight, n2.bias, n2.eps), residual=x, row_scale=rs2)
        return ops.cswin_block(x, self.patches_resolution, self.split_size, [m.idx for m in a], [m.num_heads for m in a],
                               a[0].scale, self.norm1, self.qkv, self.proj, self.norm2, self.mlp.fc1, self.mlp.fc2,
                               [m.get_v.weight for m in a], [m.get_v.bias for m in a], rs1, rs2, attn_drop=ad)


def img2windows(img, H_sp, W_sp):
    return ops.img2windows(img, H_sp, W_sp)


def windows2img(img_splits_hw, H_sp, W_sp, H, W):
    return ops.windows2img(img_splits_hw, H_sp, W_sp, H, W)


class Merge_Block(nn.Module):
    def __init__(self, dim, dim_out, norm_layer=nn.LayerNorm):
        super().__init__()
        self.conv = nn.Conv2d(dim, dim_out, 3, 2, 1)
        self.norm = norm_layer(dim_out)

    def forward(self, x):
        side = _square_side(x.shape[1])
        y = ops.conv_tokens(x, self.conv.weight, self.conv.bias, side, side, 2, 1)
        return ops.layer_norm(y, self.norm.weight, self.norm.bias, self.norm.eps)


class _CarafeBase(nn.Module):
    def __init__(self, dim, dim_out, kernel_size, up_factor):
        super().__init__()
        if kernel_size != 3:
            raise NotImplementedError("the HIP reassembly kernel is written for the 3x3 neighbourhood the reference uses")
        self.kernel_size, self.up_factor = kernel_size, up_factor
        self.down = nn.Conv2d(dim, dim // 4, 1)
        self.encoder = nn.Conv2d(dim // 4, up_factor ** 2 * kernel_size ** 2, kernel_size, 1, kernel_size // 2)
        self.out = nn.Conv2d(dim, dim_out, 1)

    def kernel_logits(self, x, side):
        mid = ops.linear(x, self.down.weight.flatten(1), self.down.bias)
        return ops.conv_tokens(mid, self.encoder.weight, self.encoder.bias, side, side, 1, 1)

    def forward(self, x):
        side = _square_side(x.shape[1])
        mid, z = ops.linear_pair(x, self.down.weight.flatten(1), self.down.bias, self.out.weight.flatten(1), None)
        e = ops.conv_tokens(mid, self.encoder.weight, self.encoder.bias, side, side, 1, 1)
        return ops.carafe_reassemble(e, z, self.out.bias, side, side, self.up_factor)


class CARAFE(_CarafeBase):
    def __init__(self, dim, dim_out, kernel_size=3, up_factor=2):
        super().__init__(dim, dim_out, kernel_size, up_factor)


class CARAFE4(_CarafeBase):
    def __init__(self, dim, dim_out, kernel_size=3, up_factor=4):
        super().__init__(dim, dim_out, kernel_size, up_factor)


class _SumInputChannels(torch.autograd.Function):

    @staticmethod
    def forward(ctx, w):
        ctx.cin = w.shape[1]
        return w.sum(1, keepdim=True)

    @staticmethod
    def backward(ctx, g):
        return g.repeat(1, ctx.cin, 1, 1)


class _PatchEmbed(nn.Sequential):

    def conv_weight(self, img):
        w = self[0].weight
        if img.shape[1] == 1 and w.shape[1] > 1:
            w = _SumInputChannels.apply(w)
        return w

    def forward(self, img, w=None):
        conv, norm = self[0], self[2]
        if w is None:
            w = self.conv_weight(img)
        tok = ops.patch_embed_conv(img, w, conv.bias, conv.stride[0], conv.padding[0])
        return ops.layer_norm(tok, norm.weight, norm.bias, norm.eps)


class CSWinTransformer(nn.Module):

    def __init__(self, img_size=224, patch_size=16, in_chans=3, num_classes=8, embed_dim=64, depth=[1, 2, 9, 1],
                 split_size=[1, 2, 7, 7], num_heads=12, mlp_ratio=4., qkv_bias=True, qk_scale=None, drop_rate=0.,
                 attn_drop_rate=0., drop_path_rate=0, hybrid_backbone=None, norm_layer=nn.LayerNorm, use_chk=False):
        super().__init__()
        self.use_chk, self.num_classes = use_chk, num_classes
        self.num_features = self.embed_dim = embed_dim
        heads = num_heads
        E = embed_dim
        self.img_size = img_size

        self.stage1_conv_embed = _PatchEmbed(nn.Conv2d(in_chans, E, 7, 4, 2), TokenRearrange(), nn.LayerNorm(E))
        self.pos_drop = nn.Dropout(p=drop_rate)

        rates = torch.linspace(0, drop_path_rate, int(np.sum(depth))).tolist()
        first = np.concatenate([[0], np.cumsum(depth)]).astype(int)

        def make_stage(si, last=False):
            return nn.ModuleList(
                CSWinBlock(dim=E << si, num_heads=heads[si], reso=img_size // (4 << si), mlp_ratio=mlp_ratio,
                           qkv_bias=qkv_bias, qk_scale=qk_scale, split_size=split_size[si], drop=drop_rate,
                           attn_drop=attn_drop_rate, drop_path=rates[first[si] + i], norm_layer=norm_layer,
                           last_stage=last)
                for i in range(depth[si]))

        self.stage1 = make_stage(0)
        self.merge1 = Merge_Block(E, 2 * E)
        self.stage2 = make_stage(1)
        self.merge2 = Merge_Block(2 * E, 4 * E)
        self.stage3 = make_stage(2)
        self.merge3 = Merge_Block(4 * E, 8 * E)
        self.stage4 = make_stage(3, last=True)
        self.norm = norm_layer(8 * E)
        self.stage_up4 = make_stage(3, last=True)
        self.upsample4 = CARAFE(8 * E, 4 * E)
        self.concat_linear4 = nn.Linear(8 * E, 4 * E)
        self.stage_up3 = make_stage(2)
        self.upsample3 = CARAFE(4 * E, 2 * E)
        self.concat_linear3 = nn.Linear(4 * E, 2 * E)
        self.stage_up2 = make_stage(1)
        self.upsample2 = CARAFE(2 * E, E)
        self.concat_linear2 = nn.Linear(2 * E, E)
        self.stage_up1 = make_stage(0)
        self.upsample1 = CARAFE4(E, E)
        self.norm_up = norm_layer(E)
        self.output = nn.Conv2d(in_channels=E, out_channels=self.num_classes, kernel_size=1, bias=False)

        self.apply(self._init_weights)

    def _init_weights(self, m):
        if isinstance(m, nn.Linear):
            trunc_normal_(m.weight, std=.02)
            if m.bias is not None:
                nn.init.constant_(m.bias, 0)
        elif isinstance(m, (nn.LayerNorm, nn.BatchNorm2d)):
            nn.init.constant_(m.bias, 0)
            nn.init.constant_(m.weight, 1.0)

    @torch.jit.ignore
    def no_weight_decay(self):
        return {'pos_embed', 'cls_token'}

    @torch.jit.ignore
    def no_weight_decay_keywords(self):
        return {'relative_position_bias_table'}

    def _run(self, blocks, x):
        for blk in blocks:
            x = checkpoint.checkpoint(blk, x, use_reentrant=False) if self.use_chk else blk(x)
        return x

    def _predraw_drop_path(self, batch, device):
        blocks = [b for st in (self.stage1, self.stage2, self.stage3, self.stage4, self.stage_up4, self.stage_up3,
                               self.stage_up2, self.stage_up1) for b in st]
        live = [b for b in blocks if isinstance(b.drop_path, DropPath) and b.drop_path.drop_prob > 0.]
        for b in blocks:
            b._dp_preset = None
        if not (self.training and live):
            return
        cache = getattr(self, "_dp_keep", None)
        if cache is None or cache.device != device or cache.shape[0] != 2 * len(live):
            cache = torch.tensor([1.0 - b.drop_path.drop_prob for b in live for _ in (0, 1)], dtype=torch.float32,
                                 device=device)[:, None]
            self._dp_keep = cache
        keep = cache
        scales = (torch.rand(keep.shape[0], batch, device=device) < keep).to(torch.float32) / keep
        for i, b in enumerate(live):
            b._dp_preset = [scales[2 * i], scales[2 * i + 1]]

    def forward_features(self, x, pe_weight=None):
        self._predraw_drop_path(x.shape[0], x.device)
        ops.clear_twins()
        x = self.stage1_conv_embed(x, pe_weight)
        if self.pos_drop.p > 0 and self.training:
            x = ops.dropout(x, self.pos_drop.p)
        x = self._run(self.stage1, x)
        self.x1 = x
        x = self._run(self.stage2, self.merge1(x))
        self.x2 = x
        self.enc_mid_in = None
        if getattr(self, "detach_decoder_inputs", False) and torch.is_grad_enabled():
            x = x.detach().requires_grad_()
            self.enc_mid_in = x
        x = self._run(self.stage3, self.merge2(x))
        self.x3 = x
        x = self._run(self.stage4, self.merge3(x))
        return ops.layer_norm(x, self.norm.weight, self.norm.bias, self.norm.eps)

    def forward_up_features(self, x):
        _, s1, s2, s3 = getattr(self, "dec_in", None) or (None, self.x1, self.x2, self.x3)
        for blocks, up, cl, skip in ((self.stage_up4, self.upsample4, self.concat_linear4, s3),
                                    (self.stage_up3, self.upsample3, self.concat_linear3, s2),
                                    (self.stage_up2, self.upsample2, self.concat_linear2, s1)):
            x = up(self._run(blocks, x))
            x = ops.linear(skip, cl.weight, cl.bias, x2=x)
        x = self._run(self.stage_up1, x)
        return ops.layer_norm(x, self.norm_up.weight, self.norm_up.bias, self.norm_up.eps)

    def up_x4(self, x):
        up, head = self.upsample1, self.output
        side = _square_side(x.shape[1])
        ncls = head.out_channels
        cpad = max(16, 1 << (ncls - 1).bit_length())
        w_fused, b_fused = ops.head_compose(head.weight, up.out.weight, up.out.bias, cpad)
        mid, z = ops.linear_pair(x, up.down.weight.flatten(1), up.down.bias, w_fused, None)
        e = ops.conv_tokens(mid, up.encoder.weight, up.encoder.bias, side, side, 1, 1)
        return ops.carafe_reassemble_nchw(e, z, b_fused, side, side, up.up_factor, ncls)

    def _conv_specs(self, pe_weight):
        pe = self.stage1_conv_embed[0]
        specs = [(pe_weight, (pe_weight.shape[1] + 3) // 4 * 4, pe.stride[0], pe.padding[0])]
        specs += [(m.conv.weight, m.conv.weight.shape[1], 2, 1) for m in (self.merge1, self.merge2, self.merge3)]
        specs += [(u.encoder.weight, u.encoder.weight.shape[1], 1, 1)
                  for u in (self.upsample4, self.upsample3, self.upsample2, self.upsample1)]
        return specs

    def forward(self, x):
        pe_weight = self.stage1_conv_embed.conv_weight(x)
        with ops.conv_weight_images(self._conv_specs(pe_weight)):
            return self._forward(x, pe_weight)

    def _forward(self, x, pe_weight):
        x = self.forward_features(x, pe_weight)
        self.xb = x
        bound = [x, self.x1, self.x2, self.x3]
        if getattr(self, "detach_decoder_inputs", False) and torch.is_grad_enabled():
            bound = [t.detach().requires_grad_() for t in bound]
        self.dec_in = bound
        x = self.forward_up_features(bound[0])
        return self.up_x4(x)
```

### cswin_unet_amd/ops.py

```python
import ctypes
import math
import types

import numpy as np
import torch
from torch.autograd import Function
from torch.autograd.function import once_differentiable

from ._lib import AugmentDesc, ConvImageJob, CswinHipError, ReduceJob, WgradDesc, act_bf16, call, dev_f32, lib, precision, ptr, shadow_ptr, stream

__all__ = ["layer_norm", "linear", "linear_pair", "mlp", "stripe_attention", "cswin_block", "conv_tokens", "patch_embed_conv", "carafe_reassemble",
           "carafe_reassemble_nchw", "conv_weight_images", "head_compose", "tokens_to_nchw", "matmul_nn", "ce_dice_loss", "continual_loss", "dropout", "img2windows", "windows2img",
           "seg_metrics", "connected_components", "filter_components", "COMPONENT_TILE", "resize_slices", "argmax_zoom_back", "augment_batch", "class_counts", "gaussian_blur"]


MAX_REDUCE_JOBS = 48
TAIL_RIDER_JOBS = 16


class engine_backward:

    def __init__(self, opt=None):
        self._flat = opt.flat_grad if opt is not None else None
        self._slots = {p.data_ptr(): (o, p.numel()) for p, o in zip(opt.params, opt.offsets)} if opt is not None else {}
        self._queue = []
        self._given = set()

    def __enter__(self):
        global _pass
        self._outer, _pass = _pass, self
        return self

    def __exit__(self, *exc):
        global _pass
        _pass = self._outer
        if exc[0] is None:
            self.flush()
        return False

    def grad(self, param_key, shape, device):
        if param_key is None:
            return None
        n = math.prod(shape)
        o, numel = self._slots.get(param_key, (0, -1)) if param_key else (0, -1)
        if numel != n:
            return torch.empty(tuple(shape), dtype=torch.float32, device=device)
        if o in self._given:
            raise CswinHipError(f"engine_backward: two ops of one backward pass use the leaf parameter at offset {o} of flat_grad; "
                                f"the first gradient is already placed there and its reduction may still be waiting")
        self._given.add(o)
        return self._flat[o:o + n].view(shape)

    def _in_flat(self, address):
        return self._flat is not None and 0 <= address - self._flat.data_ptr() < 4 * self._flat.numel()

    def reduce(self, jobs, reads):
        now = []
        for j in jobs:
            if j.part and all(self._in_flat(a) for a in (j.out, j.out2) if a):
                self._queue.append((ReduceJob.from_buffer_copy(j), reads))
            elif j.part:
                now.append(j)
        if now:
            _rows_sum((ReduceJob * len(now))(*now))

    def queued_outputs(self):
        return [a for j, _ in self._queue for a in (j.out, j.out2) if a]

    def take_pending(self, maxn=TAIL_RIDER_JOBS):
        taken, self._queue = self._queue[:maxn], self._queue[maxn:]
        arr = (ReduceJob * len(taken))(*[j for j, _ in taken])
        return (_job_ptr(arr) if taken else None), len(taken), (arr, taken)

    def flush(self):
        while self._queue:
            _rows_sum(self.take_pending(MAX_REDUCE_JOBS)[2][0])


_pass = engine_backward()


def _param_keys(*ts):
    return tuple(None if t is None else t.data_ptr() if t.is_leaf else 0 for t in ts)


def _job_ptr(jobs, i=0):
    return ctypes.c_void_p(ctypes.addressof(jobs) + i * ctypes.sizeof(ReduceJob))


def _rows_sum(jobs):
    call("cswin_rows_sum_multi", _job_ptr(jobs), len(jobs), stream())


def _ws(nbytes, device):
    return torch.empty(max(int(nbytes), 16) // 4 + 4, dtype=torch.float32, device=device)


def _reduced(nbytes, device, launch, njobs=1):
    ws, jobs = _ws(nbytes, device), (ReduceJob * njobs)()
    launch(ptr(ws), nbytes, _job_ptr(jobs))
    _pass.reduce(jobs, (ws,))


def _int_array(vals):
    return (ctypes.c_int * len(vals))(*vals)


def _ptr_array(tensors):
    return (ctypes.c_void_p * len(tensors))(*[t.data_ptr() for t in tensors])


def _stored16(*ts):
    return sum(1 << i for i, t in enumerate(ts) if t is not None and t.dtype == torch.bfloat16)


def _rows_per_sample(t):
    return t.numel() // (t.shape[0] * t.shape[-1])


def _layernorm_fwd(x, gamma, beta, eps, dtype=torch.float32):
    C = x.shape[-1]
    M = x.numel() // C
    y = torch.empty_like(x, dtype=dtype)
    mean = torch.empty(M, dtype=torch.float32, device=x.device)
    rstd = torch.empty_like(mean)
    call("cswin_layernorm_fwd", ptr(x), ptr(gamma), ptr(beta), ptr(y), ptr(mean), ptr(rstd), M, C, eps, _stored16(y), stream())
    return y, mean, rstd


def _layernorm_bwd(dy, x, mean, rstd, gamma, dx, dg, db, slab=None, *, dres=None, dx16=None):
    C = x.shape[-1]
    M = x.numel() // C
    if slab is None:
        return _reduced(lib().cswin_layernorm_bwd_workspace(M, C), x.device,
                        lambda *s: _layernorm_bwd(dy, x, mean, rstd, gamma, dx, dg, db, s, dres=dres, dx16=dx16))
    ws, nbytes, job = slab
    call("cswin_layernorm_bwd", ptr(dy), ptr(x), ptr(mean), ptr(rstd), ptr(gamma), ptr(dres), ptr(dx), ptr(dg), ptr(db), ws, nbytes,
         M, C, job, ptr(dx16), stream())


class _LayerNorm(Function):
    @staticmethod
    def forward(ctx, x, gamma, beta, eps):
        x, gamma, beta = dev_f32(x, "layer_norm input"), dev_f32(gamma), dev_f32(beta)
        y, mean, rstd = _layernorm_fwd(x, gamma, beta, eps)
        ctx.save_for_backward(x, gamma, mean, rstd)
        ctx.keys = _param_keys(gamma, beta)
        return y

    @staticmethod
    @once_differentiable
    def backward(ctx, dy):
        x, gamma, mean, rstd = ctx.saved_tensors
        dx = torch.empty_like(x)
        dg, db = (_pass.grad(k, gamma.shape, gamma.device) for k in ctx.keys)
        _layernorm_bwd(dev_f32(dy), x, mean, rstd, gamma, dx, dg, db)
        return dx, dg, db, None


def layer_norm(x, gamma, beta, eps=1e-5):
    return _LayerNorm.apply(x, gamma, beta, eps)


_twins = {}


def _twin_put(t, t16):
    _twins[t.data_ptr()] = (t, t16)


def _twin_take(t):
    e = _twins.pop(t.data_ptr(), None)
    return e[1] if e is not None and e[0]._cdata == t._cdata else None


def clear_twins():
    _twins.clear()


def _wsrc(w):
    if act_bf16() and w.shape[0] % 4 == 0 and w.shape[1] % 4 == 0:
        sp = shadow_ptr(w)
        if sp is not None:
            return sp, 4
    return ptr(w), 0


def _linear_fwd(x, w, b, N, *, dtype=torch.float32, gelu=False, x2=None, residual=None, row_scale=None):
    pw, w16 = w if isinstance(w, tuple) else (ptr(w), 0)
    K1 = x.shape[-1]
    K = K1 + (x2.shape[-1] if x2 is not None else 0)
    y = torch.empty(x.shape[:-1] + (N,), dtype=dtype, device=x.device)
    y_act = torch.empty_like(y) if gelu else None
    call("cswin_linear_fwd", ptr(x), ptr(x2), K1 if x2 is not None else 0, pw, ptr(b), ptr(y), ptr(y_act), ptr(residual), ptr(row_scale),
         _rows_per_sample(x), x.numel() // K1, N, K, precision(), _stored16(x, y) | w16, stream())
    return (y, y_act) if gelu else y


def _linear_bwd_data(dy, w, dx, *, dx2=None, gelu_pre=None, row_scale=None, add=None):
    pw, w16 = w if isinstance(w, tuple) else (ptr(w), 0)
    N, K1 = dy.shape[-1], dx.shape[-1]
    K = K1 + (dx2.shape[-1] if dx2 is not None else 0)
    call("cswin_linear_bwd_data", ptr(dy), pw, ptr(dx), ptr(dx2), K1 if dx2 is not None else 0, ptr(gelu_pre), ptr(row_scale),
         _rows_per_sample(dy), ptr(add), dy.numel() // N, N, K, precision(), _stored16(dy, dx, None, gelu_pre) | w16, stream())


def _linear_bwd_weight(dy, x, dw, db, slab=None, *, x2=None, row_scale=None):
    N, K1 = dy.shape[-1], x.shape[-1]
    K = K1 + (x2.shape[-1] if x2 is not None else 0)
    M = dy.numel() // N
    if slab is None:
        return _reduced(lib().cswin_linear_bwd_weight_workspace(M, N, K), dy.device,
                        lambda *s: _linear_bwd_weight(dy, x, dw, db, s, x2=x2, row_scale=row_scale))
    ws, nbytes, job = slab
    call("cswin_linear_bwd_weight", ptr(dy), ptr(x), ptr(x2), K1 if x2 is not None else 0, ptr(row_scale), _rows_per_sample(dy),
         ptr(dw), ptr(db), ws, nbytes, M, N, K, job, precision(), stream())


MAX_MASK_SAMPLES = 256


def _fill_wgrad(d, dy, x, row_scale, dw, dbias, workspace, ws_bytes):
    d.dy, d.x, d.row_scale, d.dw, d.dbias = (t.data_ptr() if t is not None else None for t in (dy, x, row_scale, dw, dbias))
    d.workspace, d.ws_bytes, d.rows_per_sample = workspace, ws_bytes, _rows_per_sample(dy)
    d.N, d.K = dy.shape[-1], x.shape[-1]
    d.M, d.precision, d.io_bf16 = dy.numel() // d.N, precision(), _stored16(dy, x)


def _linear_bwd_weight_batch(wg, jobs, pending=(None, 0)):
    call("cswin_linear_bwd_weight_batch", ctypes.cast(wg, ctypes.c_void_p), len(wg), _job_ptr(jobs), *pending, stream())


class _Linear(Function):
    @staticmethod
    def forward(ctx, x, w, b, x2, residual, row_scale):
        x, w = dev_f32(x, "linear input"), dev_f32(w, "linear weight")
        b, x2, residual, row_scale = dev_f32(b), dev_f32(x2), dev_f32(residual), dev_f32(row_scale)
        K = x.shape[-1] + (x2.shape[-1] if x2 is not None else 0)
        assert w.shape[1] == K, f"linear: weight {tuple(w.shape)} vs input features {K}"
        y = _linear_fwd(x, _wsrc(w), b, w.shape[0], x2=x2, residual=residual, row_scale=row_scale)
        ctx.save_for_backward(x, w, x2, row_scale)
        ctx.has_res, ctx.keys = residual is not None, _param_keys(w, b)
        return y

    @staticmethod
    @once_differentiable
    def backward(ctx, dy):
        x, w, x2, row_scale = ctx.saved_tensors
        dy = dev_f32(dy)
        need = ctx.needs_input_grad
        dx = dx2 = dw = db = None
        if need[0] or (x2 is not None and need[3]):
            dx = torch.empty_like(x)
            dx2 = torch.empty_like(x2) if x2 is not None else None
            _linear_bwd_data(dy, _wsrc(w), dx, dx2=dx2, row_scale=row_scale)
        if need[1]:
            dw = _pass.grad(ctx.keys[0], w.shape, w.device)
            db = _pass.grad(ctx.keys[1], w.shape[:1], w.device)
            _linear_bwd_weight(dy, x, dw, db, x2=x2, row_scale=row_scale)
        return dx, dw, db, dx2, (dy if ctx.has_res else None), None


def linear(x, w, b=None, x2=None, residual=None, row_scale=None):
    return _Linear.apply(x, w, b, x2, residual, row_scale)


class _LinearPair(Function):

    @staticmethod
    def forward(ctx, x, w1, b1, w2, b2):
        x, w1, b1, w2, b2 = (dev_f32(t) for t in (x, w1, b1, w2, b2))
        assert w1.shape[1] == w2.shape[1] == x.shape[-1]
        ctx.save_for_backward(x, w1, w2)
        ctx.keys = _param_keys(w1, b1, w2, b2)
        return tuple(_linear_fwd(x, w, b, w.shape[0]) for w, b in ((w1, b1), (w2, b2)))

    @staticmethod
    @once_differentiable
    def backward(ctx, dy1, dy2):
        x, w1, w2 = ctx.saved_tensors
        dy1, dy2 = dev_f32(dy1), dev_f32(dy2)
        K = x.shape[-1]
        M = x.numel() // K
        dx = None
        if ctx.needs_input_grad[0]:
            dx = torch.empty_like(x)
            _linear_bwd_data(dy1, w1, dx)
            _linear_bwd_data(dy2, w2, dx, add=dx)
        grads, keep = [], []
        wg, jobs = (WgradDesc * 2)(), (ReduceJob * 2)()
        for i, (dy, w) in enumerate(((dy1, w1), (dy2, w2))):
            dw = _pass.grad(ctx.keys[2 * i], w.shape, w.device)
            db = _pass.grad(ctx.keys[2 * i + 1], w.shape[:1], w.device)
            nbytes = lib().cswin_linear_bwd_weight_workspace(M, w.shape[0], K)
            keep.append(_ws(nbytes, w.device))
            _fill_wgrad(wg[i], dy, x, None, dw, db, ptr(keep[-1]), nbytes)
            grads += [dw, db]
        _linear_bwd_weight_batch(wg, jobs)
        _pass.reduce(jobs, keep)
        return (dx,) + tuple(grads)


def linear_pair(x, w1, b1, w2, b2):
    return _LinearPair.apply(x, w1, b1, w2, b2)


_epoch = {}


def dropout_epoch(device):
    t = _epoch.get(device)
    if t is None:
        t = _epoch[device] = torch.zeros(1, dtype=torch.int64, device=device)
    return t


def advance_dropout_epoch(device):
    dropout_epoch(device).add_(1)


def _draw_seeds(n):
    return tuple(int(v) for v in torch.randint(0, 2 ** 62, (n,)).tolist())


def _dropout(x, y, p, seed, *, residual=None, row_scale=None):
    call("cswin_dropout", ptr(x), ptr(residual), ptr(row_scale), ptr(y), x.numel(), x.numel() // x.shape[0], float(p), int(seed),
         ptr(dropout_epoch(x.device)), stream())


class _Mlp(Function):

    @staticmethod
    def forward(ctx, x, w1, b1, w2, b2, residual, row_scale, drop_p, seeds):
        x, w1, b1, w2, b2 = (dev_f32(t) for t in (x, w1, b1, w2, b2))
        residual, row_scale = dev_f32(residual), dev_f32(row_scale)
        s1, s2 = _wsrc(w1), _wsrc(w2)
        pre, act = _linear_fwd(x, s1, b1, w1.shape[0], gelu=True)
        if drop_p > 0:
            _dropout(act, act, drop_p, seeds[0])
            y = _linear_fwd(act, s2, b2, w2.shape[0])
            _dropout(y, y, drop_p, seeds[1], residual=residual, row_scale=row_scale)
        else:
            y = _linear_fwd(act, s2, b2, w2.shape[0], residual=residual, row_scale=row_scale)
        ctx.save_for_backward(x, w1, w2, pre, act, row_scale)
        ctx.has_res, ctx.keys = residual is not None, _param_keys(w1, b1, w2, b2)
        ctx.drop = (float(drop_p), seeds)
        return y

    @staticmethod
    @once_differentiable
    def backward(ctx, dy):
        x, w1, w2, pre, act, row_scale = ctx.saved_tensors
        dy = dev_f32(dy)
        K = x.shape[-1]
        Hd, N = w1.shape[0], w2.shape[0]
        M = x.numel() // K
        dev = x.device
        drop_p, seeds = ctx.drop
        dyl, rs_gemm = dy, row_scale
        if drop_p > 0:
            dyl = torch.empty_like(dy)
            _dropout(dy, dyl, drop_p, seeds[1], row_scale=row_scale)
            rs_gemm = None
        dpre = torch.empty_like(pre)
        _linear_bwd_data(dyl, w2, dpre, gelu_pre=pre, row_scale=rs_gemm)
        if drop_p > 0:
            _dropout(dpre, dpre, drop_p, seeds[0])
        dx = None
        if ctx.needs_input_grad[0]:
            dx = torch.empty_like(x)
            _linear_bwd_data(dpre, w1, dx)
        k1, kb1, k2, kb2 = ctx.keys
        dw2, db2 = _pass.grad(k2, w2.shape, dev), _pass.grad(kb2, (N,), dev)
        nbytes = max(lib().cswin_linear_bwd_weight_workspace(M, N, Hd), lib().cswin_linear_bwd_weight_workspace(M, Hd, K))
        ws, ws1 = _ws(nbytes, dev), _ws(nbytes, dev)
        jobs = (ReduceJob * 2)()
        _linear_bwd_weight(dyl, act, dw2, db2, (ptr(ws), nbytes, _job_ptr(jobs, 0)), row_scale=rs_gemm)
        dw1, db1 = _pass.grad(k1, w1.shape, dev), _pass.grad(kb1, (Hd,), dev)
        _linear_bwd_weight(dpre, x, dw1, db1, (ptr(ws1), nbytes, _job_ptr(jobs, 1)))
        _pass.reduce(jobs, (ws, ws1))
        return dx, dw1, db1, dw2, db2, (dy if ctx.has_res else None), None, None, None


def mlp(x, w1, b1, w2, b2, residual=None, row_scale=None, drop_p=0.0):
    return _Mlp.apply(x, w1, b1, w2, b2, residual, row_scale, float(drop_p), _draw_seeds(2) if drop_p > 0 else (0, 0))


class _MatmulNN(Function):

    @staticmethod
    def forward(ctx, a, b):
        a, b = dev_f32(a), dev_f32(b)
        c = torch.empty(a.shape[0], b.shape[1], dtype=torch.float32, device=a.device)
        _linear_bwd_data(a, b, c)
        ctx.save_for_backward(a, b)
        return c

    @staticmethod
    @once_differentiable
    def backward(ctx, dc):
        a, b = ctx.saved_tensors
        dc = dev_f32(dc)
        da = _linear_fwd(dc, b, None, a.shape[1])
        db = torch.empty_like(b)
        _linear_bwd_weight(a, dc, db, None)
        return da, db


def matmul_nn(a, b):
    return _MatmulNN.apply(a, b)


ATTN_FP32, ATTN_QKV16, ATTN_IO16, ATTN_MFMA16 = 0, 1, 3, 7


def _attn_drop_args(drop, device):
    return drop[0], drop[1], ptr(dropout_epoch(device)) if drop[0] > 0 else None


def _attn_fwd(qkv, lw, lb, y, y0, lse, reso, split, idx, heads, scale, drop, mode):
    B, _, C3 = qkv.shape
    call("cswin_attn_fwd", ptr(qkv), _ptr_array(lw), _ptr_array(lb), ptr(y), ptr(y0), ptr(lse), B, reso, C3 // 3, len(idx),
         _int_array(heads), _int_array(idx), split, float(scale or 0.0), *_attn_drop_args(drop, qkv.device), mode, stream())


def _attn_bwd(qkv, lw, lb, lse, y0, dy, dqkv, dlw, dlb, reso, split, idx, heads, scale, drop, mode, slab=None):
    B, _, C3 = qkv.shape
    ha, ia = _int_array(heads), _int_array(idx)
    if slab is None:
        nbytes = lib().cswin_attn_bwd_workspace(B, reso, C3 // 3, len(idx), ha, ia, split)
        again = lambda *s: _attn_bwd(qkv, lw, lb, lse, y0, dy, dqkv, dlw, dlb, reso, split, idx, heads, scale, drop, mode, s)
        return _reduced(nbytes, qkv.device, again, njobs=2)
    ws, nbytes, jobs = slab
    call("cswin_attn_bwd", ptr(qkv), _ptr_array(lw), _ptr_array(lb), ptr(lse), ptr(y0), ptr(dy), ptr(dqkv), _ptr_array(dlw),
         _ptr_array(dlb), ws, nbytes, B, reso, C3 // 3, len(idx), ha, ia, split, float(scale or 0.0), jobs,
         *_attn_drop_args(drop, qkv.device), mode, stream())


class _StripeAttention(Function):
    @staticmethod
    def forward(ctx, qkv, reso, split, idx, heads, scale, drop, *wb):
        q16 = qkv.dtype == torch.bfloat16 and qkv.is_cuda
        qkv = qkv.contiguous() if q16 else dev_f32(qkv, "attention qkv")
        nb = len(idx)
        ws_ = [dev_f32(t).view(t.shape[0], 9) for t in wb[:nb]]
        bs_ = [dev_f32(t) for t in wb[nb:]]
        B, L, C3 = qkv.shape
        if L != reso * reso:
            raise ValueError("flatten img_tokens has wrong size")
        y = torch.empty(B, L, C3 // 3, dtype=torch.float32, device=qkv.device)
        y0 = torch.empty_like(y) if any(ctx.needs_input_grad) else None
        lse = torch.empty(B, sum(heads), L, dtype=torch.float32, device=qkv.device)
        ctx.meta = (reso, split, tuple(idx), tuple(heads), scale, drop, ATTN_QKV16 if q16 else ATTN_FP32)
        _attn_fwd(qkv, ws_, bs_, y, y0, lse, *ctx.meta)
        ctx.save_for_backward(qkv, lse, y0, *ws_, *bs_)
        ctx.keys = _param_keys(*wb)
        return y

    @staticmethod
    @once_differentiable
    def backward(ctx, dy):
        qkv, lse, y0, *wb_ = ctx.saved_tensors
        nb = len(wb_) // 2
        ws_, bs_ = wb_[:nb], wb_[nb:]
        dqkv = torch.empty_like(qkv)
        dws = [_pass.grad(k, t.shape, t.device) for k, t in zip(ctx.keys[:nb], ws_)]
        dbs = [_pass.grad(k, t.shape, t.device) for k, t in zip(ctx.keys[nb:], bs_)]
        _attn_bwd(qkv, ws_, bs_, lse, y0, dev_f32(dy), dqkv, dws, dbs, *ctx.meta)
        return (dqkv, None, None, None, None, None, None) + tuple(d.view(d.shape[0], 1, 3, 3) for d in dws) + tuple(dbs)


def _attn_drop(p):
    p = float(p)
    return (p, _draw_seeds(1)[0]) if p > 0 else (0.0, 0)


def stripe_attention(qkv, reso, split, idx, heads, lepe_w, lepe_b, scale=None, attn_drop=0.0):
    return _StripeAttention.apply(qkv, reso, split, tuple(idx), tuple(heads), scale, _attn_drop(attn_drop), *lepe_w, *lepe_b)


class _CSWinBlock(Function):

    @staticmethod
    def forward(ctx, x, reso, split, idx, heads, scale, eps1, eps2, rs1, rs2, drop, g1, b1, wqkv, bqkv, wp, bp, g2, b2, w1, bb1,
                w2, bb2, *lepe):
        x = dev_f32(x, "block input")
        B, L, C = x.shape
        if L != reso * reso:
            raise ValueError("flatten img_tokens has wrong size")
        dev = x.device
        nb = len(idx)
        lw = [dev_f32(t).view(t.shape[0], 9) for t in lepe[:nb]]
        lb = [dev_f32(t) for t in lepe[nb:]]
        rs1, rs2 = dev_f32(rs1), dev_f32(rs2)
        s16 = act_bf16() and C % 4 == 0
        t16 = torch.bfloat16 if s16 else torch.float32
        E16 = lambda *shape: torch.empty(*shape, dtype=t16, device=dev)
        sq, sp, s1, s2 = (_wsrc(w) if s16 else w for w in (wqkv, wp, w1, w2))
        attn = (reso, split, tuple(idx), tuple(heads), scale, drop, ATTN_MFMA16 if s16 else ATTN_FP32)
        h1, m1, r1 = _layernorm_fwd(x, g1, b1, eps1, t16)
        qkv = _linear_fwd(h1, sq, bqkv, 3 * C, dtype=t16)
        att, lse = E16(B, L, C), torch.empty(B, sum(heads), L, dtype=torch.float32, device=dev)
        att0 = E16(B, L, C) if any(ctx.needs_input_grad) else None
        _attn_fwd(qkv, lw, lb, att, att0, lse, *attn)
        x1 = _linear_fwd(att, sp, bp, C, residual=x, row_scale=rs1)
        h2, m2, r2 = _layernorm_fwd(x1, g2, b2, eps2, t16)
        pre, act = _linear_fwd(h2, s1, bb1, w1.shape[0], dtype=t16, gelu=True)
        y = _linear_fwd(act, s2, bb2, C, residual=x1, row_scale=rs2)
        ctx.save_for_backward(x, m1, r1, h1, qkv, lse, att, att0, x1, m2, r2, h2, pre, act, rs1, rs2, g1, wqkv, wp, g2, w1, w2, *lw, *lb)
        ctx.attn = attn
        ctx.keys = _param_keys(g1, b1, wqkv, bqkv, wp, bp, g2, b2, w1, bb1, w2, bb2, *lepe)
        return y

    @staticmethod
    @once_differentiable
    def backward(ctx, dy):
        (x, m1, r1, h1, qkv, lse, att, att0, x1, m2, r2, h2, pre, act, rs1, rs2, g1, wqkv, wp, g2, w1, w2, *lwb) = ctx.saved_tensors
        nb = len(lwb) // 2
        lw, lb = lwb[:nb], lwb[nb:]
        dy = dev_f32(dy)
        B, L, C = x.shape
        M, Hd = B * L, w1.shape[0]
        dev, h = x.device, lib()
        s16 = h1.dtype == torch.bfloat16
        wq, lq = h.cswin_linear_bwd_weight_workspace, h.cswin_layernorm_bwd_workspace
        sizes = [wq(M, C, Hd), wq(M, Hd, C), lq(M, C), wq(M, C, C), wq(M, 3 * C, C), lq(M, C)]
        sizes = [(n + 255) // 256 * 256 for n in sizes]
        ws = _ws(sum(sizes), dev)
        wsp = [ctypes.c_void_p(ws.data_ptr() + sum(sizes[:i])) for i in range(6)]
        jobs = (ReduceJob * 8)()
        sq, sp, s1, s2 = (_wsrc(w) if s16 else w for w in (wqkv, wp, w1, w2))
        dy16 = _twin_take(dy) if s16 else None
        dyg = dy16 if dy16 is not None else dy
        dpre = torch.empty_like(pre)
        _linear_bwd_data(dyg, s2, dpre, gelu_pre=pre, row_scale=rs2)
        wg = (WgradDesc * 4)()
        kg1, kb1, kwqkv, kbqkv, kwp, kbp, kg2, kb2, kw1, kbb1, kw2, kbb2, *klepe = ctx.keys
        G = lambda key, *shape: _pass.grad(key, shape, dev)
        dw2, db2 = G(kw2, *w2.shape), G(kbb2, C)
        _fill_wgrad(wg[0], dyg, act, rs2, dw2, db2, wsp[0], sizes[0])
        dw1, db1 = G(kw1, *w1.shape), G(kbb1, Hd)
        _fill_wgrad(wg[1], dpre, h2, None, dw1, db1, wsp[1], sizes[1])
        dh2 = torch.empty_like(x)
        _linear_bwd_data(dpre, s1, dh2)
        dx1, dg2, dbt2 = torch.empty_like(x), G(kg2, C), G(kb2, C)
        dx1_16 = torch.empty_like(x, dtype=torch.bfloat16) if s16 else None
        _layernorm_bwd(dh2, x1, m2, r2, g2, dx1, dg2, dbt2, (wsp[2], sizes[2], _job_ptr(jobs, 2)), dres=dy, dx16=dx1_16)
        dx1g = dx1_16 if s16 else dx1
        datt = dh2
        _linear_bwd_data(dx1g, sp, datt, row_scale=rs1)
        dwp, dbp = G(kwp, *wp.shape), G(kbp, C)
        _fill_wgrad(wg[2], dx1g, att, rs1, dwp, dbp, wsp[3], sizes[3])
        dqkv = torch.empty_like(qkv)
        dlw = [G(k, *t.shape) for k, t in zip(klepe[:nb], lw)]
        dlb = [G(k, *t.shape) for k, t in zip(klepe[nb:], lb)]
        reso, split, idx, heads = ctx.attn[:4]
        naw = h.cswin_attn_bwd_workspace(B, reso, C, nb, _int_array(heads), _int_array(idx), split)
        aws = _ws(naw, dev)
        _attn_bwd(qkv, lw, lb, lse, att0, datt, dqkv, dlw, dlb, *ctx.attn, (ptr(aws), naw, _job_ptr(jobs, 6)))
        dwqkv, dbqkv = G(kwqkv, *wqkv.shape), G(kbqkv, 3 * C)
        _fill_wgrad(wg[3], dqkv, h1, None, dwqkv, dbqkv, wsp[4], sizes[4])
        wjobs = (ReduceJob * 4)()
        dh1 = datt
        pend, npend, riders = _pass.take_pending()
        if precision() == 0:
            tail = (ptr(dqkv), ptr(wqkv), ptr(dh1), M, 3 * C, C, ctypes.cast(wg, ctypes.c_void_p), 4, _job_ptr(wjobs), pend, npend)
            masks = (rs2, rs2, rs1, rs1) if B <= MAX_MASK_SAMPLES else (None,) * 4
            if any(m is not None for m in masks):
                skip = (ctypes.c_void_p * 4)(*[m.data_ptr() if m is not None else None for m in masks])
                call("cswin_linear_bwd_tail_masked", *tail, skip, _int_array([B] * 4), stream())
            else:
                call("cswin_linear_bwd_tail", *tail, stream())
        else:
            _linear_bwd_weight_batch(wg, wjobs, (pend, npend))
            _linear_bwd_data(dqkv, sq, dh1)
        for slot, ji in enumerate((0, 1, 3, 4)):
            jobs[ji] = wjobs[slot]
        dx, dg1, dbt1 = torch.empty_like(x), G(kg1, C), G(kb1, C)
        dx16 = torch.empty_like(x, dtype=torch.bfloat16) if s16 else None
        _layernorm_bwd(dh1, x, m1, r1, g1, dx, dg1, dbt1, (wsp[5], sizes[5], _job_ptr(jobs, 5)), dres=dx1, dx16=dx16)
        if s16:
            _twin_put(dx, dx16)
        _pass.reduce(jobs, (ws, aws))
        grads = (dx, None, None, None, None, None, None, None, None, None, None, dg1, dbt1, dwqkv, dbqkv, dwp, dbp, dg2, dbt2, dw1, db1,
                 dw2, db2)
        return grads + tuple(d.view(d.shape[0], 1, 3, 3) for d in dlw) + tuple(dlb)


def cswin_block(x, reso, split, idx, heads, scale, norm1, qkv, proj, norm2, fc1, fc2, lepe_w, lepe_b, rs1=None, rs2=None, attn_drop=0.0):
    return _CSWinBlock.apply(x, reso, split, tuple(idx), tuple(heads), scale, norm1.eps, norm2.eps, rs1, rs2, _attn_drop(attn_drop),
                             norm1.weight, norm1.bias, qkv.weight, qkv.bias, proj.weight, proj.bias, norm2.weight,
                             norm2.bias, fc1.weight, fc1.bias, fc2.weight, fc2.bias, *lepe_w, *lepe_b)


MAX_CONV_IMAGE_JOBS = 16
_conv_images = {}


def _same_conv(w, stride, pad):
    return stride == 1 and 2 * pad == w.shape[2] - 1 and w.shape[0] % 4 == 0


class conv_weight_images:

    def __init__(self, specs):
        self._specs = [sp for sp in specs if sp[0] is not None and sp[0].is_cuda and sp[0].dtype == torch.float32 and sp[0].is_contiguous()]

    def __enter__(self):
        global _conv_images
        self._outer = _conv_images
        images, jobs = {}, []
        grad = torch.is_grad_enabled()
        for w, cpad, stride, pad in self._specs[:MAX_CONV_IMAGE_JOBS]:
            Cout, Cin, ks, _ = w.shape
            E = lambda *shape: torch.empty(*shape, dtype=torch.float32, device=w.device)
            same = _same_conv(w, stride, pad)
            need_dx = grad and cpad == Cin
            wp = E(Cout, ks * ks, cpad)
            wpt = E(ks * ks, Cout, cpad) if need_dx and not same else None
            wf = E(Cin, ks * ks, Cout) if need_dx and same else None
            images[w.data_ptr()] = (w, cpad, wp, wpt, wf)
            jobs.append(ConvImageJob(w.data_ptr(), wp.data_ptr(), wpt.data_ptr() if wpt is not None else None,
                                     wf.data_ptr() if wf is not None else None, Cout, Cin, ks, cpad))
        if jobs:
            arr = (ConvImageJob * len(jobs))(*jobs)
            call("cswin_conv_weight_images", ctypes.cast(arr, ctypes.c_void_p), len(jobs), stream())
        _conv_images = images
        return self

    def __exit__(self, *exc):
        global _conv_images
        _conv_images = self._outer
        return False


def _images_of(w, cpad):
    e = _conv_images.get(w.data_ptr())
    if e is not None and e[0].shape == w.shape and e[1] == cpad:
        return e[2:]
    return None


def _permute_w(w, cpad, want_t):
    Cout, Cin, ks, _ = w.shape
    wp = torch.empty(Cout, ks * ks, cpad, dtype=torch.float32, device=w.device)
    wpt = torch.empty(ks * ks, Cout, cpad, dtype=torch.float32, device=w.device) if want_t else None
    call("cswin_conv_weight_permute", ptr(w), ptr(wp), ptr(wpt), Cout, Cin, ks, cpad, stream())
    return wp, wpt


def _conv_tok_fwd(x, w_img, b, y, H, W, ks, stride, pad):
    call("cswin_conv_tok_fwd", ptr(x), ptr(w_img), ptr(b), ptr(y), x.shape[0], H, W, x.shape[-1], y.shape[-1], ks, stride, pad,
         precision(), stream())


class _ConvTokens(Function):
    @staticmethod
    def forward(ctx, x, w, b, H, W, stride, pad):
        x, w, b = dev_f32(x, "conv input"), dev_f32(w), dev_f32(b)
        B, L, Cin = x.shape
        assert L == H * W and w.shape[1] == Cin
        Cout, ks = w.shape[0], w.shape[2]
        OH, OW = (H + 2 * pad - ks) // stride + 1, (W + 2 * pad - ks) // stride + 1
        need_dx = ctx.needs_input_grad[0]
        same = _same_conv(w, stride, pad)
        img = _images_of(w, Cin)
        wf = None
        if img is not None and (img[1] is not None or same or not need_dx):
            wp, wpt, wf = img
        else:
            wp, wpt = _permute_w(w, Cin, need_dx and not same)
        y = torch.empty(B, OH * OW, Cout, dtype=torch.float32, device=x.device)
        _conv_tok_fwd(x, wp, b, y, H, W, ks, stride, pad)
        ctx.save_for_backward(x, w, wpt, wf if need_dx else None)
        ctx.meta = (H, W, stride, pad)
        ctx.keys = _param_keys(w, b)
        return y

    @staticmethod
    @once_differentiable
    def backward(ctx, dy):
        x, w, wpt, wf = ctx.saved_tensors
        H, W, stride, pad = ctx.meta
        dy = dev_f32(dy)
        B, L, Cin = x.shape
        Cout, ks = w.shape[0], w.shape[2]
        dx = None
        if ctx.needs_input_grad[0]:
            dx = torch.empty_like(x)
            if _same_conv(w, stride, pad):
                if wf is None:
                    wf = torch.empty(Cin, ks * ks, Cout, dtype=torch.float32, device=x.device)
                    call("cswin_conv_weight_flipT", ptr(w), ptr(wf), Cout, Cin, ks, stream())
                _conv_tok_fwd(dy, wf, None, dx, H, W, ks, 1, pad)
            else:
                if wpt is None:
                    _, wpt = _permute_w(w, Cin, True)
                call("cswin_conv_tok_bwd_data", ptr(dy), ptr(wpt), ptr(dx), B, H, W, Cin, Cout, ks, stride, pad, precision(), stream())
        dw = _pass.grad(ctx.keys[0], w.shape, x.device)
        db = _pass.grad(ctx.keys[1], (Cout,), x.device)
        _reduced(lib().cswin_conv_tok_bwd_weight_workspace(B, H, W, Cin, Cout, ks, stride, pad), x.device,
                 lambda ws, nbytes, job: call("cswin_conv_tok_bwd_weight", ptr(dy), ptr(x), ptr(dw), ptr(db), ws, nbytes, B, H, W, Cin,
                                              Cout, ks, stride, pad, 1, job, precision(), stream()))
        return dx, dw, db, None, None, None, None


def conv_tokens(x, w, b, H, W, stride, pad):
    return _ConvTokens.apply(x, w, b, H, W, stride, pad)


class _PatchEmbedConv(Function):

    @staticmethod
    def forward(ctx, img, w, b, stride, pad):
        img, w, b = dev_f32(img, "image"), dev_f32(w), dev_f32(b)
        B, Cin, H, W = img.shape
        Cout, ks = w.shape[0], w.shape[2]
        cpad = (Cin + 3) // 4 * 4
        st = stream()
        x = torch.empty(B, H * W, cpad, dtype=torch.float32, device=img.device)
        call("cswin_nchw_to_tokens", ptr(img), ptr(x), B, Cin, H, W, cpad, st)
        images = _images_of(w, cpad)
        wp = images[0] if images is not None else _permute_w(w, cpad, False)[0]
        OH, OW = (H + 2 * pad - ks) // stride + 1, (W + 2 * pad - ks) // stride + 1
        y = torch.empty(B, OH * OW, Cout, dtype=torch.float32, device=img.device)
        _conv_tok_fwd(x, wp, b, y, H, W, ks, stride, pad)
        ctx.save_for_backward(x, w)
        ctx.meta = (H, W, stride, pad)
        ctx.keys = _param_keys(w, b)
        return y

    @staticmethod
    @once_differentiable
    def backward(ctx, dy):
        x, w = ctx.saved_tensors
        H, W, stride, pad = ctx.meta
        dy = dev_f32(dy)
        B, cpad = x.shape[0], x.shape[-1]
        Cout, Cin, ks, _ = w.shape
        dw = _pass.grad(ctx.keys[0], w.shape, x.device)
        db = _pass.grad(ctx.keys[1], (Cout,), x.device)
        _reduced(lib().cswin_conv_tok_bwd_weight_workspace(B, H, W, cpad, Cout, ks, stride, pad), x.device,
                 lambda ws, nbytes, job: call("cswin_conv_tok_bwd_weight_cpad", ptr(dy), ptr(x), ptr(dw), ptr(db), ws, nbytes, B, H, W,
                                              cpad, Cin, Cout, ks, stride, pad, job, precision(), stream()))
        return None, dw, db, None, None


def patch_embed_conv(img, w, b, stride=4, pad=2):
    return _PatchEmbedConv.apply(img, w, b, stride, pad)


class _CarafeReassemble(Function):

    @staticmethod
    def forward(ctx, e, z, bias, H, W, S, C):
        e, z, bias = dev_f32(e, "carafe kernel logits"), dev_f32(z, "carafe features"), dev_f32(bias)
        B, L, Cz = z.shape
        assert L == H * W and e.shape == (B, L, 9 * S * S) and (C is None or 0 < C <= Cz)
        out = torch.empty((B, L * S * S, Cz) if C is None else (B, C, S * H, S * W), dtype=torch.float32, device=z.device)
        wt = torch.empty_like(e)
        if C is None:
            call("cswin_carafe_fwd", ptr(e), ptr(z), ptr(bias), ptr(out), ptr(wt), B, H, W, Cz, S, stream())
        else:
            call("cswin_carafe_fwd_nchw", ptr(e), ptr(z), ptr(bias), ptr(out), ptr(wt), B, H, W, Cz, C, S, stream())
        ctx.save_for_backward(z, wt)
        ctx.meta = (H, W, S, C)
        ctx.keys = _param_keys(bias)
        return out

    @staticmethod
    @once_differentiable
    def backward(ctx, dout):
        z, wt = ctx.saved_tensors
        H, W, S, C = ctx.meta
        dout = dev_f32(dout)
        B, L, Cz = z.shape
        de = torch.empty_like(wt)
        dz = torch.empty_like(z)
        db = _pass.grad(ctx.keys[0], (Cz,), z.device)
        io = (ptr(dout), ptr(z), ptr(wt), ptr(de), ptr(dz), ptr(db))
        if C is None:
            launch = lambda ws, nbytes, job: call("cswin_carafe_bwd", *io, ws, nbytes, B, H, W, Cz, S, job, stream())
        else:
            launch = lambda ws, nbytes, job: call("cswin_carafe_bwd_nchw", *io, ws, nbytes, B, H, W, Cz, C, S, job, stream())
        _reduced(lib().cswin_carafe_bwd_workspace(B, H, W, Cz, S), z.device, launch)
        return de, dz, db, None, None, None, None


def carafe_reassemble(e, z, bias, H, W, S):
    return _CarafeReassemble.apply(e, z, bias, H, W, S, None)


def carafe_reassemble_nchw(e, z, bias, H, W, S, C):
    if lib().cswin_carafe_bwd_nchw_ok(H, W, z.shape[-1], S):
        return _CarafeReassemble.apply(e, z, bias, H, W, S, C)
    return tokens_to_nchw(carafe_reassemble(e, z, bias, H, W, S), C, S * H, S * W)


class _HeadCompose(Function):

    @staticmethod
    def forward(ctx, w_head, w_out, b_out, cpad):
        w_head, w_out, b_out = dev_f32(w_head, "head weight"), dev_f32(w_out, "out weight"), dev_f32(b_out)
        ncls, E = w_head.shape[0], w_head.numel() // w_head.shape[0]
        C = w_out.numel() // w_out.shape[0]
        assert w_out.shape[0] == E and cpad >= ncls and (b_out is None or b_out.numel() == E)
        wf = torch.empty(cpad, C, dtype=torch.float32, device=w_head.device)
        bf = torch.empty(cpad, dtype=torch.float32, device=w_head.device)
        call("cswin_head_compose", ptr(w_head), ptr(w_out), ptr(b_out), ptr(wf), ptr(bf), ncls, E, C, cpad, stream())
        ctx.save_for_backward(w_head, w_out, b_out)
        ctx.keys = _param_keys(w_head, w_out, b_out)
        return wf, bf

    @staticmethod
    @once_differentiable
    def backward(ctx, dwf, dbf):
        w_head, w_out, b_out = ctx.saved_tensors
        ncls, E = w_head.shape[0], w_head.numel() // w_head.shape[0]
        C = w_out.numel() // w_out.shape[0]
        dev = w_head.device
        dwf = dev_f32(dwf) if dwf is not None else torch.zeros(ncls, C, dtype=torch.float32, device=dev)
        dbf = dev_f32(dbf)
        dwh = _pass.grad(ctx.keys[0], w_head.shape, dev)
        dwo = _pass.grad(ctx.keys[1], w_out.shape, dev)
        dbo = _pass.grad(ctx.keys[2], (E,), dev)
        call("cswin_head_compose_bwd", ptr(w_head), ptr(w_out), ptr(b_out), ptr(dwf), ptr(dbf), ptr(dwh), ptr(dwo), ptr(dbo),
             ncls, E, C, stream())
        return dwh, dwo, dbo, None


def head_compose(w_head, w_out, b_out, cpad):
    return _HeadCompose.apply(w_head, w_out, b_out, int(cpad))


class _TokensToNchw(Function):
    @staticmethod
    def forward(ctx, x, C, H, W):
        x = dev_f32(x)
        B, L, Cpad = x.shape
        assert L == H * W and C <= Cpad
        y = torch.empty(B, C, H, W, dtype=torch.float32, device=x.device)
        call("cswin_tokens_to_nchw", ptr(x), ptr(y), B, C, H, W, Cpad, stream())
        ctx.meta = (C, H, W, Cpad)
        return y

    @staticmethod
    @once_differentiable
    def backward(ctx, dy):
        C, H, W, Cpad = ctx.meta
        dy = dev_f32(dy)
        B = dy.shape[0]
        dx = torch.empty(B, H * W, Cpad, dtype=torch.float32, device=dy.device)
        call("cswin_nchw_to_tokens", ptr(dy), ptr(dx), B, C, H, W, Cpad, stream())
        return dx, None, None, None


def tokens_to_nchw(x, C, H, W):
    return _TokensToNchw.apply(x, C, H, W)


def img2windows(img, H_sp, W_sp):
    img = dev_f32(img, "img2windows input")
    B, C, H, W = img.shape
    out = torch.empty(B * (H // H_sp) * (W // W_sp), H_sp * W_sp, C, dtype=torch.float32, device=img.device)
    call("cswin_img2windows", ptr(img), ptr(out), B, C, H, W, H_sp, W_sp, stream())
    return out


def windows2img(img_splits_hw, H_sp, W_sp, H, W):
    x = dev_f32(img_splits_hw, "windows2img input")
    C = x.shape[-1]
    B = int(x.shape[0] / (H * W / H_sp / W_sp))
    out = torch.empty(B, H, W, C, dtype=torch.float32, device=x.device)
    call("cswin_windows2img", ptr(x), ptr(out), B, C, H, W, H_sp, W_sp, stream())
    return out


def _pixels(logits):
    B, ncls = logits.shape[:2]
    return B, ncls, logits.numel() // (B * ncls)


class CeDiceObjective:
    n_stats = 3

    def __init__(self, w_ce=0.4, w_dice=0.6, class_weight=None, probs=False):
        self.w_ce, self.w_dice, self.class_weight, self.probs = w_ce, w_dice, class_weight, probs

    @staticmethod
    def n_sums(ncls):
        return 1 + 3 * ncls

    def sums(self, logits, labels, sums, teacher=None):
# ... 375 lines not shown
```

### include/cswin_hip.h

```cpp
#ifndef CSWIN_HIP_H
#define CSWIN_HIP_H

#include <stddef.h>

#ifdef __cplusplus
extern "C" {
#endif

#define CSWIN_ABI_VERSION 4

#define CSWIN_OK 0
#define CSWIN_ERR_SHAPE (-1)
#define CSWIN_ERR_ALIGN (-2)
#define CSWIN_ERR_WORKSPACE (-3)
#define CSWIN_ERR_HIP (-4)
#define CSWIN_ERR_UNSUPPORTED (-5)

typedef struct cswin_reduce_job {
    const float* part;
    float* out;
    float* out2;
    long long n_first, n, stride;
    int rows, reserved;
    int conv_kk, conv_cin;
} cswin_reduce_job;

const char* cswin_last_error(void);
int cswin_abi_version(void);
int cswin_device_ok(void);

int cswin_attn_fwd(const float* qkv, const float* const* lepe_w, const float* const* lepe_b, float* y, float* y0, float* lse,
                   int B, int reso, int C, int nbranch, const int* heads, const int* idx, int split, float scale,
                   float drop_p, unsigned long long drop_seed, const unsigned long long* drop_epoch, int qkv_bf16, void* stream);
size_t cswin_attn_bwd_workspace(int B, int reso, int C, int nbranch, const int* heads, const int* idx, int split);
int cswin_attn_bwd(const float* qkv, const float* const* lepe_w, const float* const* lepe_b, const float* lse,
                   const float* y0, const float* dy, float* dqkv, float* const* dlepe_w, float* const* dlepe_b,
                   void* workspace, size_t ws_bytes, int B, int reso, int C, int nbranch, const int* heads, const int* idx,
                   int split, float scale, cswin_reduce_job* deferred, float drop_p, unsigned long long drop_seed,
                   const unsigned long long* drop_epoch, int qkv_bf16, void* stream);

int cswin_img2windows(const float* img, float* out, int B, int C, int H, int W, int H_sp, int W_sp, void* stream);
int cswin_windows2img(const float* win, float* out, int B, int C, int H, int W, int H_sp, int W_sp, void* stream);

int cswin_layernorm_fwd(const float* x, const float* gamma, const float* beta, float* y, float* mean, float* rstd,
                        int M, int C, float eps, int y_bf16, void* stream);
size_t cswin_layernorm_bwd_workspace(int M, int C);
int cswin_layernorm_bwd(const float* dy, const float* x, const float* mean, const float* rstd, const float* gamma,
                        const float* dres, float* dx, float* dgamma, float* dbeta, void* workspace, size_t ws_bytes,
                        int M, int C, cswin_reduce_job* deferred, void* dx_bf16, void* stream);

int cswin_linear_fwd(const float* x, const float* x2, int k_split, const float* w, const float* bias, float* y,
                     float* y_act, const float* residual, const float* row_scale, int rows_per_sample, int M, int N,
                     int K, int precision, int io_bf16, void* stream);
int cswin_linear_bwd_data(const float* dy, const float* w, float* dx, float* dx2, int k_split, const float* gelu_pre,
                          const float* row_scale, int rows_per_sample, const float* add, int M, int N, int K,
                          int precision, int io_bf16, void* stream);
size_t cswin_linear_bwd_weight_workspace(int M, int N, int K);
int cswin_linear_bwd_weight(const float* dy, const float* x, const float* x2, int k_split, const float* row_scale,
                            int rows_per_sample, float* dw, float* dbias, void* workspace, size_t ws_bytes, int M,
                            int N, int K, cswin_reduce_job* deferred, int precision, void* stream);
typedef struct cswin_wgrad_desc {
    const float* dy;
    const float* x;
    const float* row_scale;
    float* dw;
    float* dbias;
    void* workspace;
    size_t ws_bytes;
    int rows_per_sample, M, N, K;
    int precision;
    int io_bf16;
} cswin_wgrad_desc;
int cswin_linear_bwd_weight_batch(const cswin_wgrad_desc* problems, int n, cswin_reduce_job* deferred, const cswin_reduce_job* pending,
                                  int npending, void* stream);
int cswin_linear_bwd_tail(const float* dy, const float* w, float* dx, int M, int N, int K, const cswin_wgrad_desc* problems, int n,
                          cswin_reduce_job* deferred, const cswin_reduce_job* pending, int npending, void* stream);
int cswin_linear_bwd_weight_batch_masked(const cswin_wgrad_desc* problems, int n, cswin_reduce_job* deferred,
                                         const cswin_reduce_job* pending, int npending, const float* const* skip, const int* nsamples,
                                         void* stream);
int cswin_linear_bwd_tail_masked(const float* dy, const float* w, float* dx, int M, int N, int K, const cswin_wgrad_desc* problems, int n,
                                 cswin_reduce_job* deferred, const cswin_reduce_job* pending, int npending, const float* const* skip,
                                 const int* nsamples, void* stream);
int cswin_rows_sum_multi(const cswin_reduce_job* jobs, int njobs, void* stream);

int cswin_conv_tok_fwd(const float* x, const float* w_perm, const float* bias, float* y, int B, int H, int W, int Cin,
                       int Cout, int ks, int stride, int pad, int precision, void* stream);
int cswin_conv_tok_bwd_data(const float* dy, const float* w_permT, float* dx, int B, int H, int W, int Cin, int Cout,
                            int ks, int stride, int pad, int precision, void* stream);
size_t cswin_conv_tok_bwd_weight_workspace(int B, int H, int W, int Cin, int Cout, int ks, int stride, int pad);
int cswin_conv_tok_bwd_weight(const float* dy, const float* x, float* dw, float* dbias, void* workspace,
                              size_t ws_bytes, int B, int H, int W, int Cin, int Cout, int ks, int stride, int pad,
                              int torch_layout, cswin_reduce_job* deferred, int precision, void* stream);
int cswin_conv_weight_permute(const float* w, float* w_perm, float* w_permT, int Cout, int Cin, int ks, int Cpad,
                              void* stream);
int cswin_conv_weight_unpermute(const float* dw_perm, float* dw, int Cout, int Cin, int ks, int Cpad, void* stream);
int cswin_conv_weight_flipT(const float* w, float* wf, int Cout, int Cin, int ks, void* stream);
typedef struct cswin_conv_image_job {
    const float* w;
    float* w_perm;
    float* w_permT;
    float* w_flipT;
    int Cout, Cin, ks, Cpad;
} cswin_conv_image_job;
int cswin_conv_weight_images(const cswin_conv_image_job* jobs, int njobs, void* stream);
int cswin_conv_tok_bwd_weight_cpad(const float* dy, const float* x, float* dw, float* dbias, void* workspace, size_t ws_bytes,
                                   int B, int H, int W, int Cin, int Cin_param, int Cout, int ks, int stride, int pad,
                                   cswin_reduce_job* deferred, int precision, void* stream);

int cswin_nchw_to_tokens(const float* x, float* y, int B, int C, int H, int W, int Cpad, void* stream);
int cswin_tokens_to_nchw(const float* x, float* y, int B, int C, int H, int W, int Cpad, void* stream);

int cswin_carafe_fwd(const float* e, const float* z, const float* bias, float* out, float* wt_save, int B, int H,
                     int W, int Cz, int S, void* stream);
size_t cswin_carafe_bwd_workspace(int B, int H, int W, int Cz, int S);
int cswin_carafe_bwd(const float* dout, const float* z, const float* wt_save, float* de, float* dz, float* dbias,
                     void* workspace, size_t ws_bytes, int B, int H, int W, int Cz, int S, cswin_reduce_job* deferred, void* stream);
int cswin_carafe_fwd_nchw(const float* e, const float* z, const float* bias, float* out, float* wt_save, int B, int H, int W,
                          int Cz, int C, int S, void* stream);
int cswin_carafe_bwd_nchw_ok(int H, int W, int Cz, int S);
int cswin_carafe_bwd_nchw(const float* dout, const float* z, const float* wt_save, float* de, float* dz, float* dbias,
                          void* workspace, size_t ws_bytes, int B, int H, int W, int Cz, int C, int S, cswin_reduce_job* deferred,
                          void* stream);

int cswin_head_compose(const float* w_head, const float* w_out, const float* b_out, float* w_fused, float* b_fused, int ncls,
                       int E, int C, int Cpad, void* stream);
int cswin_head_compose_bwd(const float* w_head, const float* w_out, const float* b_out, const float* dw_fused,
                           const float* db_fused, float* dw_head, float* dw_out, float* db_out, int ncls, int E, int C,
                           void* stream);

size_t cswin_loss_workspace(int B, int ncls, long HW);
int cswin_loss_sums(const float* logits, const long long* labels, float* sums, void* workspace, size_t ws_bytes, int B,
                    int ncls, long HW, int inputs_are_probs, void* stream);
int cswin_loss_finalize(const float* sums, float* out3, float* coef, double n_pixels, int ncls, float w_ce,
                        float w_dice, const float* class_weight, void* stream);
int cswin_loss_bwd(const float* logits, const long long* labels, const float* coef, const float* grad_out,
                   float* dlogits, float ce_scale, float dice_scale, int B, int ncls, long HW, int inputs_are_probs,
                   void* stream);

size_t cswin_cl_loss_workspace(int B, int ncls, long HW);
int cswin_cl_loss_sums(const float* logits, const long long* labels, const int* label_map, int n_map, const float* teacher,
                       const float* class_weight, float* sums, void* workspace, size_t ws_bytes, int B, int ncls, int nold,
                       long HW, float temperature, float focal_alpha, float focal_gamma, void* stream);
int cswin_cl_loss_finalize(const float* sums, float* out5, float* coef, double n_pixels, double batch, int ncls, float w_focal,
                           float w_dice, float kd_weight, float temperature, void* stream);
int cswin_cl_loss_bwd(const float* logits, const long long* labels, const int* label_map, int n_map, const float* teacher,
                      const float* class_weight, const float* coef, const float* grad_out, float* dlogits, float focal_scale,
                      float dice_scale, float kd_scale, int B, int ncls, int nold, long HW, float temperature, float focal_alpha,
                      float focal_gamma, void* stream);

int cswin_sgd_flat(float* p, const float* g, float* m, long n, const float* lr_dev, float momentum,
                   float weight_decay, float grad_scale, void* shadow_bf16, void* stream);
int cswin_multi_copy(const void* table, int nchunks, void* stream);


int cswin_chunk_sumsq(const float* g, const float* p, const void* chunks, int nchunks, float* partial, void* stream);
int cswin_norm_finalize(const float* partial, const int* first_chunk, int ntensors, float grad_scale, float max_norm,
                        float* tensor_sumsq, float* scalars, void* stream);
int cswin_adamw_flat(float* p, const float* g, float* m, float* v, const void* chunks, int nchunks, const float* lr_dev,
                     const float* lr_mult, const float* scalars, double beta1, double beta2, double eps, float weight_decay,
                     float grad_scale, double bc1, double bc2, void* shadow_bf16, void* stream);

int cswin_rate_finalize(const float* partial, const int* first_chunk, int ntensors, float grad_scale, float max_norm,
                        const int* group_first, const int* group_tensors, const int* group_of, int ngroups, int statistic,
                        float default_mult, float* tensor_sumsq, float* scalars, float* group_stat, float* lr_mult, void* stream);
int cswin_adam_flat(float* p, const float* g, float* m, float* v, const void* chunks, int nchunks, const float* lr_dev,
                    const float* lr_mult, const float* scalars, double beta1, double beta2, double eps, float weight_decay,
                    float grad_scale, double bc1, double bc2, int flags, void* shadow_bf16, void* stream);

int cswin_tpgm_chunk_stats(const float* p, const float* anchor, const float* g, const void* chunks, int nchunks, int l1,
                           float* partial, void* stream);
int cswin_tpgm_finalize(const float* partial, const int* first_chunk, int ntensors, int l1, const int* flags, float* gamma,
                        float* gm, float* gv, double grad_scale, double proj_lr, double bc1, double bc2, int mode, float* ratio,
                        float* norm, float* scalars, void* stream);
int cswin_tpgm_project(const float* src, const float* anchor, float* dst, const float* ratio, const void* chunks, int nchunks,
                       void* shadow_bf16, void* stream);

int cswin_eb_tiles(const float* g, const void* tiles, int ntiles, float* partial, void* stream);
int cswin_eb_finalize(const float* partial, const int* first_tile, const int* numel, int ntensors, float* evidence, void* stream);

int cswin_dropout(const float* x, const float* residual, const float* row_scale, float* y, long n, long elems_per_sample,
                  float p, unsigned long long seed, const unsigned long long* seed_epoch, void* stream);
int cswin_pack_bf16(const float* src, void* dst_bf16, long n, void* stream);
int cswin_pack_bf16_scaled(const float* src, void* dst_bf16, long n, float scale, void* stream);
int cswin_unpack_bf16(const void* src_bf16, float* dst, long n, void* stream);

int    cswin_seg_metrics_nbins(int D, int H, int W);
size_t cswin_seg_metrics_workspace(int D, int H, int W, int ndim, int ncls);
int    cswin_seg_metrics(const unsigned char* pred, const unsigned char* label, long long* counts, unsigned int* hist,
                         void* workspace, size_t ws_bytes, int D, int H, int W, int ndim, int ncls, void* stream);

size_t cswin_components_workspace(int D, int H, int W);
int    cswin_components_label(const unsigned char* vol, int* labels, int* sizes, void* workspace, size_t ws_bytes, int D, int H,
                              int W, int ncls, void* stream);
int    cswin_components_filter(const unsigned char* vol, const int* labels, const int* sizes, const long long* min_size,
                               const double* min_fraction, unsigned char* out, void* workspace, size_t ws_bytes, int D, int H,
                               int W, int ncls, void* stream);

int cswin_resize_banded(const void* x, float* y, const double* wh, const int* sh, int Th, const double* ww, const int* sw, int Tw,
                        int D, int H, int W, int h, int w, int x_f64, void* stream);
int cswin_argmax_zoom_back(const float* logits, unsigned char* out, const int* src_row, const int* src_col, int B, int ncls, int h,
                           int w, int H, int W, void* stream);
int cswin_argmax_zoom_back_classes(const float* logits, unsigned char* out, const int* src_row, const int* src_col,
                                   const int* classes, int nsel, int B, int ncls, int h, int w, int H, int W, void* stream);

int cswin_class_counts(const void* labels, int label_bytes, const int* label_map, int nmap, long long* counts, int N,
                       long long slice_elems, int ncls, void* stream);

int cswin_gaussian_blur(const float* x, float* y, const double* taps, int radius, int D, int H, int W, void* stream);

typedef struct cswin_augment_desc {
    int kind, k, axis;
    int src;
    const int* map;
} cswin_augment_desc;
int cswin_augment_gather(const float* x, float* y, const void* table, int n, int B, int H, int W, int Ho, int Wo, void* stream);
int cswin_augment_labels(const unsigned char* lab, long long* out, const void* table, const int* src_row, const int* src_col,
                         const int* src_row_t, const int* src_col_t, int n, int B, int H, int W, int h, int w, void* stream);

#ifdef __cplusplus
}
#endif
#endif
```

Before: 1960 images/sec.

## Skip Linear GEMM rows of DropPath-dropped samples via a per-block sample order

Adds a kernel that turns DropPath draws into per-sample scales plus an order list with kept samples first. It also adds row-mapped GEMM variants: the forward Linears, the data-gradient Linears and the block-tail dgrad in CSWin blocks read A rows through this order. Tiles beyond the kept rows do no K-loop work. The aim is to avoid GEMM work on samples whose residual branch is zeroed by stochastic depth. In exchange it adds a small order kernel, an extra shared-memory order load and sync per workgroup, and indexed row addressing. Correctness depends on the epilogue still producing correct residual and garbage-free outputs for the dropped rows.

Result: faster. 1995 images/sec (median of 6 runs) (+1.8%).

```diff
diff --git a/cswin_unet_amd/_lib.py b/cswin_unet_amd/_lib.py
--- a/cswin_unet_amd/_lib.py
+++ b/cswin_unet_amd/_lib.py
@@ -31,6 +31,10 @@
     "cswin_linear_bwd_tail": (I, [P, P, P, I, I, I, P, I, P, P, I, P]),
     "cswin_linear_bwd_weight_batch_masked": (I, [P, I, P, P, I, P, P, P]),
     "cswin_linear_bwd_tail_masked": (I, [P, P, P, I, I, I, P, I, P, P, I, P, P, P]),
+    "cswin_drop_path_order": (I, [P, P, P, P, I, I, P]),
+    "cswin_linear_fwd_skip": (I, [P, P, I, P, P, P, P, P, P, I, I, I, I, I, I, P, I, P]),
+    "cswin_linear_bwd_data_skip": (I, [P, P, P, P, I, P, P, I, P, I, I, I, I, I, P, I, P]),
+    "cswin_linear_bwd_tail_skip": (I, [P, P, P, I, I, I, P, I, P, P, I, P, P, P, I, P]),
     "cswin_rows_sum_multi": (I, [P, I, P]),
     "cswin_conv_tok_fwd": (I, [P, P, P, P, I, I, I, I, I, I, I, I, I, P]),
     "cswin_conv_tok_bwd_data": (I, [P, P, P, I, I, I, I, I, I, I, I, I, P]),
diff --git a/cswin_unet_amd/csrc/gemm.hip b/cswin_unet_amd/csrc/gemm.hip
--- a/cswin_unet_amd/csrc/gemm.hip
+++ b/cswin_unet_amd/csrc/gemm.hip
@@ -292,6 +292,34 @@
     if (tid == 0) kept->n = n;
 }
 
+struct RowMap { const int* order; int nsamples, rows_per_sample; unsigned magic; };
+
+__global__ __launch_bounds__(64) void drop_path_order_kernel(const float* __restrict__ u, const float* __restrict__ keep,
+                                                             float* __restrict__ scales, int* __restrict__ order, int B) {
+    const int r = blockIdx.x, lane = threadIdx.x;
+    const float k = keep[r];
+    const float* ur = u + (long)r * B;
+    int* ord = order + (long)r * (B + 1);
+    int nk = 0;
+    for (int s0 = 0; s0 < B; s0 += 64) {
+        const int s = s0 + lane;
+        const bool kept = s < B && ur[s] < k;
+        const unsigned long long bal = __ballot(kept);
+        if (kept) ord[1 + nk + __popcll(bal & ((1ull << lane) - 1ull))] = s;
+        if (s < B) scales[(long)r * B + s] = __fdiv_rn(kept ? 1.0f : 0.0f, k);
+        nk += __popcll(bal);
+    }
+    if (lane == 0) ord[0] = nk;
+    int nd = nk;
+    for (int s0 = 0; s0 < B; s0 += 64) {
+        const int s = s0 + lane;
+        const bool dropped = s < B && !(ur[s] < k);
+        const unsigned long long bal = __ballot(dropped);
+        if (dropped) ord[1 + nd + __popcll(bal & ((1ull << lane) - 1ull))] = s;
+        nd += __popcll(bal);
+    }
+}
+
 __device__ __forceinline__ void stamp(const Epilogue& epi, int row, int slot) {
     if (!epi.stamps || threadIdx.x != 0) return;
     long long* s = epi.stamps + 8L * row;
@@ -300,10 +328,11 @@
     if (slot == 3) s[6] = __builtin_amdgcn_s_memrealtime();
 }
 
-template <class T, int VEC, int EPI, bool SCALE_A, int PREC, class ASrc, class BSrc, bool MASKED = false>
+template <class T, int VEC, int EPI, bool SCALE_A, int PREC, class ASrc, class BSrc, bool MASKED = false, bool MAPPED = false>
 __device__ __forceinline__ void gemm_body(float* lds, const ASrc& A, const BSrc& B, const Epilogue& epi, int M, int N, int R,
                                           int r_per_split, int tiles_m, int tiles_n, int bid, int nblk, int stamp_row,
-                                          const RowMask* mk = nullptr, KeptList* kept = nullptr) {
+                                          const RowMask* mk = nullptr, KeptList* kept = nullptr, const RowMap* rm = nullptr,
+                                          int* ord = nullptr) {
     typedef typename T::A TA;
     typedef typename T::B TB;
     constexpr int BM = T::BM, BN = T::BN, BK = T::BK, KW = T::KW, NW = T::NW, FM = T::FM, FN = T::FN, LD16 = T::LD16;
@@ -316,11 +345,27 @@
 
     const int tid = threadIdx.x, lane = tid & 63, wave = (tid >> 6) % NW, kg = tid / (64 * NW);
     const int li = lane & 31, lh = lane >> 5;
-    const int lb = xcd_block_order(bid, nblk);
+    bool mapped = false;
+    int kept_rows = M, nlive = nblk;
+    if constexpr (MAPPED) {
+        static_assert(A_RC && VEC == 4 && PREC == 0 && !MASKED && !SCALE_A && is_plain<ASrc> && is_plain<BSrc> && EPI != EPI_SPLIT2,
+                      "the row map serves forward and data-gradient Linears of plain fp32 matrices");
+        for (int s = tid; s < rm->nsamples; s += T::THREADS) ord[s] = min(max(rm->order[1 + s], 0), rm->nsamples - 1);
+        const int nk = __builtin_amdgcn_readfirstlane(rm->order[0]);
+        mapped = nk < rm->nsamples;
+        if (mapped) {
+            kept_rows = max(nk, 0) * rm->rows_per_sample;
+            nlive = (kept_rows + BM - 1) / BM * tiles_n;
+        }
+    }
+    const int lb = (!MAPPED || bid < nlive) ? xcd_block_order(bid, nlive) : bid;
     const int tiles = tiles_m * tiles_n;
     const int split = lb / tiles;
     const int tile = lb - split * tiles;
     const int m0 = (tile / tiles_n) * BM, n0 = (tile % tiles_n) * BN;
+    if constexpr (MAPPED) {
+        if (mapped) __syncthreads();
+    }
     if constexpr (MASKED) {
         static_assert(!A_RC && !B_RC && VEC == 4 && BM == BN && is_plain<ASrc> && is_plain<BSrc>,
                       "the sample mask serves weight gradients of plain matrices (one row mapping for both operands)");
@@ -330,7 +375,7 @@
         r_per_split = ((R + mk->splits - 1) / mk->splits + 7) / 8 * 8;
     }
     const int r_begin = split * r_per_split;
-    const int r_end = min(R, r_begin + r_per_split);
+    const int r_end = (MAPPED && mapped && m0 >= kept_rows) ? r_begin : min(R, r_begin + r_per_split);
     const int wm0 = (wave / T::WGN) * T::WM, wn0 = (wave % T::WGN) * T::WN;
 
     const int a_c = tid % TA::CPR, a_r = tid / TA::CPR;
@@ -340,7 +385,19 @@
     typename BSrc::Row brow[TB::Q];
     if (A_RC) {
 #pragma unroll
-        for (int q = 0; q < TA::Q; ++q) arow[q] = A.row(m0 + a_r + q * TA::RPP);
+        for (int q = 0; q < TA::Q; ++q) {
+            if constexpr (MAPPED) {
+                const int m = m0 + a_r + q * TA::RPP;
+                int row = -1;
+                if (mapped && m < kept_rows) {
+                    const int j = fdiv1(m, rm->magic);
+                    row = ord[j] * rm->rows_per_sample + (m - j * rm->rows_per_sample);
+                }
+                arow[q] = mapped ? src_mapped_row(A, row, 1.0f) : A.row(m);
+            } else {
+                arow[q] = A.row(m0 + a_r + q * TA::RPP);
+            }
+        }
     }
     if (B_RC) {
 #pragma unroll
@@ -580,7 +637,10 @@
     }
     Epilogue e = epi;
     e.C += (long)split * e.split_stride;
-    if constexpr (EPI == EPI_GELUBWD) {
+    if constexpr (MAPPED) {
+        run_epilogue<EPI, FM, FN, false, false, true>(e, acc, M, N, m0 + wm0, n0 + wn0, lane, lds + wave * EP_WAVE_FLOATS, true, 0, 0,
+                                                      mapped ? ord : nullptr, kept_rows, rm->rows_per_sample, rm->magic);
+    } else if constexpr (EPI == EPI_GELUBWD) {
         if (e.pre_bf16) run_epilogue<EPI, FM, FN, true>(e, acc, M, N, m0 + wm0, n0 + wn0, lane, lds + wave * EP_WAVE_FLOATS, e.vec_store != 0);
         else run_epilogue<EPI, FM, FN, false>(e, acc, M, N, m0 + wm0, n0 + wn0, lane, lds + wave * EP_WAVE_FLOATS, e.vec_store != 0);
     } else {
@@ -600,6 +660,16 @@
     __shared__ __attribute__((aligned(16))) float lds[T::LDS_FLOATS];
     gemm_body<T, VEC, EPI, SCALE_A, PREC, ASrc, BSrc>(lds, A, B, epi, M, N, R, r_per_split, tiles_m, tiles_n, (int)blockIdx.x, (int)gridDim.x,
                                                       (int)blockIdx.x);
+}
+
+template <int BM, int BN, int BK, int KW, bool B_RC, int EPI>
+__global__ __launch_bounds__((Tile<BM, BN, BK, KW, true, B_RC>::THREADS)) void gemm_mapped_kernel(PlainSrc A, PlainSrc B, Epilogue epi, int M, int N, int R,
+                                                    int r_per_split, int tiles_m, int tiles_n, RowMap rm) {
+    typedef Tile<BM, BN, BK, KW, true, B_RC> T;
+    __shared__ __attribute__((aligned(16))) float lds[T::LDS_FLOATS];
+    __shared__ int ord[MASK_MAX_SAMPLES];
+    gemm_body<T, 4, EPI, false, 0, PlainSrc, PlainSrc, false, true>(lds, A, B, epi, M, N, R, r_per_split, tiles_m, tiles_n, (int)blockIdx.x,
+                                                                    (int)gridDim.x, (int)blockIdx.x, nullptr, nullptr, &rm, ord);
 }
 
 constexpr int WGRAD_BATCH = 4;
@@ -657,8 +727,9 @@
 typedef Tile<64, 64, 64, 2, true, false> TailDgradTile;
 static_assert(TailDgradTile::THREADS == WgradTile::THREADS, "one workgroup size for both halves of the block tail");
 constexpr int BLOCK_TAIL_LDS = TailDgradTile::LDS_FLOATS > WgradTile::LDS_FLOATS ? TailDgradTile::LDS_FLOATS : WgradTile::LDS_FLOATS;
-template <bool MASKED>
-__device__ __forceinline__ void block_tail_body(float (&lds)[BLOCK_TAIL_LDS], KeptList* kept, const BlockTail& t) {
+template <bool MASKED, bool MAPPED = false>
+__device__ __forceinline__ void block_tail_body(float (&lds)[BLOCK_TAIL_LDS], KeptList* kept, const BlockTail& t, const RowMap* rm = nullptr,
+                                                int* ord = nullptr) {
     const int bid = (int)blockIdx.x, nw = t.w.first[t.w.n];
     if (bid >= nw + t.nd) {
         if (threadIdx.x >= 256) return;
@@ -667,8 +738,12 @@
         return;
     }
     if (bid >= nw) {
-        gemm_body<TailDgradTile, 4, EPI_PLAIN, false, 0, PlainSrc, PlainSrc>(lds, t.dA, t.dB, t.de, t.dM, t.dN, t.dR, t.drps, t.dtm, t.dtn, bid - nw,
-                                                                             t.nd, bid);
+        if constexpr (MAPPED)
+            gemm_body<TailDgradTile, 4, EPI_PLAIN, false, 0, PlainSrc, PlainSrc, false, true>(lds, t.dA, t.dB, t.de, t.dM, t.dN, t.dR, t.drps, t.dtm,
+                                                                                              t.dtn, bid - nw, t.nd, bid, nullptr, nullptr, rm, ord);
+        else
+            gemm_body<TailDgradTile, 4, EPI_PLAIN, false, 0, PlainSrc, PlainSrc>(lds, t.dA, t.dB, t.de, t.dM, t.dN, t.dR, t.drps, t.dtm, t.dtn, bid - nw,
+                                                                                 t.nd, bid);
         return;
     }
     wgrad_batch_body<0, MASKED>(lds, kept, t.w, bid);
@@ -681,6 +756,12 @@
     __shared__ __attribute__((aligned(16))) float lds[BLOCK_TAIL_LDS];
     __shared__ KeptList kept;
     block_tail_body<true>(lds, &kept, t);
+}
+__global__ __launch_bounds__(WgradTile::THREADS) void gemm_block_tail_skip_kernel(BlockTail t, RowMap rm) {
+    __shared__ __attribute__((aligned(16))) float lds[BLOCK_TAIL_LDS];
+    __shared__ KeptList kept;
+    __shared__ int ord[MASK_MAX_SAMPLES];
+    block_tail_body<true, true>(lds, &kept, t, &rm, ord);
 }
 
 template <int KW> using S2DgradTile = Tile<64, 64, (KW == 1 ? 32 : 64), KW, true, false>;
@@ -692,10 +773,17 @@
 
 template <int BM, int BN, int BK, int KW, bool A_RC, bool B_RC, int VEC, int EPI, bool SCALE_A, int PREC, class ASrc, class BSrc>
 void launch_cfg(const ASrc& A, const BSrc& B, const Epilogue& epi, int M, int N, int R, int splits, int r_per_split,
-                hipStream_t st) {
+                hipStream_t st, const RowMap* rm = nullptr) {
     int tm = cdiv(M, BM), tn = cdiv(N, BN);
     dim3 grid(tm * tn * splits);
     const int pad_lds = cswin_tuning().gemm_pad_lds;
+    if constexpr (A_RC && VEC == 4 && PREC == 0 && !SCALE_A && is_plain<ASrc> && is_plain<BSrc> && EPI != EPI_SPLIT2 && (B_RC || EPI != EPI_RES)) {
+        if (rm) {
+            hipLaunchKernelGGL((gemm_mapped_kernel<BM, BN, BK, KW, B_RC, EPI>), grid, dim3((Tile<BM, BN, BK, KW, A_RC, B_RC>::THREADS)), pad_lds, st, A, B,
+                               epi, M, N, R, r_per_split, tm, tn, *rm);
+            return;
+        }
+    }
     hipLaunchKernelGGL((gemm_kernel<BM, BN, BK, KW, A_RC, B_RC, VEC, EPI, SCALE_A, PREC, ASrc, BSrc>), grid, dim3((Tile<BM, BN, BK, KW, A_RC, B_RC>::THREADS)), pad_lds, st, A, B, epi,
                        M, N, R, r_per_split, tm, tn);
 }
@@ -710,7 +798,7 @@
 
 template <bool A_RC, bool B_RC, int VEC, int EPI, bool SCALE_A, class ASrc, class BSrc>
 void launch_gemm(const ASrc& A, const BSrc& B, const Epilogue& epi_in, int M, int N, int R, int splits, int r_per_split,
-                 int precision, hipStream_t st) {
+                 int precision, hipStream_t st, const RowMap* rm = nullptr) {
     Epilogue epi = epi_in;
     epi.vec_store = epilogue_vec_ok(epi, N);
     auto blocks = [&](int bm, int bn) { return (long)cdiv(M, bm) * cdiv(N, bn) * splits; };
@@ -731,15 +819,15 @@
     }
     if (tile == 2) {
         if (k_groups(blocks(64, 32), r_len) >= 2)
-            return launch_cfg<64, 32, 64, 2, A_RC, B_RC, VEC, EPI, SCALE_A, 0>(A, B, epi, M, N, R, splits, r_per_split, st);
-        return launch_cfg<64, 32, 32, 1, A_RC, B_RC, VEC, EPI, SCALE_A, 0>(A, B, epi, M, N, R, splits, r_per_split, st);
+            return launch_cfg<64, 32, 64, 2, A_RC, B_RC, VEC, EPI, SCALE_A, 0>(A, B, epi, M, N, R, splits, r_per_split, st, rm);
+        return launch_cfg<64, 32, 32, 1, A_RC, B_RC, VEC, EPI, SCALE_A, 0>(A, B, epi, M, N, R, splits, r_per_split, st, rm);
     }
     int kw = k_groups(blocks(64, 64), r_len);
     if (wgrad && r_len >= 256 && kw < 2) kw = 2;
     if (forced_kw) kw = forced_kw;
-    if (kw == 4) launch_cfg<64, 64, 64, 4, A_RC, B_RC, VEC, EPI, SCALE_A, 0>(A, B, epi, M, N, R, splits, r_per_split, st);
-    else if (kw == 2) launch_cfg<64, 64, 64, 2, A_RC, B_RC, VEC, EPI, SCALE_A, 0>(A, B, epi, M, N, R, splits, r_per_split, st);
-    else launch_cfg<64, 64, 32, 1, A_RC, B_RC, VEC, EPI, SCALE_A, 0>(A, B, epi, M, N, R, splits, r_per_split, st);
+    if (kw == 4) launch_cfg<64, 64, 64, 4, A_RC, B_RC, VEC, EPI, SCALE_A, 0>(A, B, epi, M, N, R, splits, r_per_split, st, rm);
+    else if (kw == 2) launch_cfg<64, 64, 64, 2, A_RC, B_RC, VEC, EPI, SCALE_A, 0>(A, B, epi, M, N, R, splits, r_per_split, st, rm);
+    else launch_cfg<64, 64, 32, 1, A_RC, B_RC, VEC, EPI, SCALE_A, 0>(A, B, epi, M, N, R, splits, r_per_split, st, rm);
 }
 
 template <bool A_RC, bool B_RC, int EPI, bool SCALE_A, class ASrc, class BSrc>
@@ -846,7 +934,22 @@
 struct TailExtras {
     const char* who; const float* dy; const float* w; float* dx; int M, N, K; const cswin_reduce_job* jobs; int njobs;
     const float* const* skip; const int* nsamples;
+    const int* order; int order_samples;
 };
+
+int row_map_checked(RowMap* rm, const char* who, const int* order, int nsamples, int rows_per_sample, int M, int precision, int io_bf16,
+                    bool two_part, bool add) {
+    CSWIN_REQUIRE(precision == 0 && io_bf16 == 0, CSWIN_ERR_UNSUPPORTED, "%s: a sample order needs precision 0 and fp32 storage", who);
+    CSWIN_REQUIRE(!two_part, CSWIN_ERR_UNSUPPORTED, "%s: a sample order takes no concat / split operand", who);
+    CSWIN_REQUIRE(!add, CSWIN_ERR_UNSUPPORTED, "%s: a sample order takes no add operand", who);
+    CSWIN_REQUIRE(order && nsamples >= 1 && nsamples <= MASK_MAX_SAMPLES, CSWIN_ERR_SHAPE, "%s: the order must list 1..%d samples", who,
+                  MASK_MAX_SAMPLES);
+    CSWIN_REQUIRE(M > 0 && rows_per_sample > 0 && (long)nsamples * rows_per_sample == M, CSWIN_ERR_SHAPE,
+                  "%s: nsamples * rows_per_sample != M", who);
+    CSWIN_REQUIRE(fdiv_exact((long)M + 63, rows_per_sample), CSWIN_ERR_UNSUPPORTED, "%s: M * rows_per_sample must stay below 2^32", who);
+    *rm = RowMap{order, nsamples, rows_per_sample, fdiv_magic(rows_per_sample)};
+    return CSWIN_OK;
+}
 
 int wgrad_batch_impl(const cswin_wgrad_desc* d, int n, cswin_reduce_job* deferred, const TailExtras& x, void* stream) {
     CSWIN_REQUIRE(x.njobs >= 0 && x.njobs <= CSWIN_TAIL_RIDER_JOBS && (x.njobs == 0 || x.jobs), CSWIN_ERR_SHAPE,
@@ -854,6 +957,14 @@
     CSWIN_REQUIRE(d && deferred && n >= 1 && n <= WGRAD_BATCH, CSWIN_ERR_SHAPE, "linear_bwd_weight_batch: 1..%d problems and their deferred slots", WGRAD_BATCH);
     bool fast = true, any_bf16 = false, any_mask = false;
     const int precision = d[0].precision;
+    RowMap dmap = {};
+    if (x.order) {
+        CSWIN_REQUIRE(x.dy && x.order_samples >= 1 && x.M % x.order_samples == 0, CSWIN_ERR_SHAPE, "%s: nsamples * rows_per_sample != M", x.who);
+        int rc = row_map_checked(&dmap, x.who, x.order, x.order_samples, x.M / x.order_samples, x.M, precision, 0, false, false);
+        if (rc) return rc;
+        CSWIN_REQUIRE(x.N % 4 == 0 && x.K % 4 == 0 && aligned16(x.dy) && aligned16(x.w) && aligned16(x.dx), CSWIN_ERR_ALIGN,
+                      "%s: a sample order needs N, K multiples of 4 and 16-B aligned operands", x.who);
+    }
     CSWIN_CHECK_PRECISION(precision, "linear_bwd_weight_batch");
     for (int i = 0; i < n; ++i) {
         CSWIN_REQUIRE(d[i].precision == precision, CSWIN_ERR_UNSUPPORTED, "linear_bwd_weight_batch: problems of one launch share one precision");
@@ -885,8 +996,11 @@
     const bool jobs_ride16 = merge_on && w16_path && x.njobs > 0;
     if (extra && !ride) {
         if (has_dgrad) {
-            launch_gemm_vec<true, false, EPI_PLAIN, false>(g_vec, gA, gB, plain_epilogue(x.dx, x.K), x.M, x.K, x.N, 1, one_split(x.N), precision,
-                                                           (hipStream_t)stream);
+            if (x.order)
+                launch_gemm<true, false, 4, EPI_PLAIN, false>(gA, gB, plain_epilogue(x.dx, x.K), x.M, x.K, x.N, 1, one_split(x.N), 0, (hipStream_t)stream, &dmap);
+            else
+                launch_gemm_vec<true, false, EPI_PLAIN, false>(g_vec, gA, gB, plain_epilogue(x.dx, x.K), x.M, x.K, x.N, 1, one_split(x.N), precision,
+                                                               (hipStream_t)stream);
             CSWIN_LAUNCH_CHECK();
         }
         if (x.njobs > 0 && !jobs_ride16) {
@@ -972,7 +1086,9 @@
             t.r.njobs = x.njobs;
         }
         static_assert(sizeof(BlockTail) <= 4096, "kernel argument block");
-        if (any_mask) hipLaunchKernelGGL(gemm_block_tail_masked_kernel, dim3(blocks + t.nd + rblocks), dim3(512), 0, (hipStream_t)stream, t);
+        static_assert(sizeof(BlockTail) + sizeof(RowMap) <= 4096, "kernel argument block");
+        if (x.order) hipLaunchKernelGGL(gemm_block_tail_skip_kernel, dim3(blocks + t.nd + rblocks), dim3(512), 0, (hipStream_t)stream, t, dmap);
+        else if (any_mask) hipLaunchKernelGGL(gemm_block_tail_masked_kernel, dim3(blocks + t.nd + rblocks), dim3(512), 0, (hipStream_t)stream, t);
         else hipLaunchKernelGGL(gemm_block_tail_kernel, dim3(blocks + t.nd + rblocks), dim3(512), 0, (hipStream_t)stream, t);
     } else if (any_mask) {
         hipLaunchKernelGGL(gemm_wgrad_batch_masked_kernel, dim3(blocks), dim3(512), 0, (hipStream_t)stream, b);
@@ -1034,6 +1150,10 @@
 int cswin_linear_bwd_tail_masked(const float* dy, const float* w, float* dx, int M, int N, int K, const cswin_wgrad_desc* d, int n,
                                  cswin_reduce_job* deferred, const cswin_reduce_job* pending, int npending, const float* const* skip,
                                  const int* nsamples, void* stream);
+
+int cswin_linear_bwd_tail_skip(const float* dy, const float* w, float* dx, int M, int N, int K, const cswin_wgrad_desc* d, int n,
+                               cswin_reduce_job* deferred, const cswin_reduce_job* pending, int npending, const float* const* skip,
+                               const int* nsamples, const int* order, int order_samples, void* stream);
 
 int cswin_linear_fwd(const float* x, const float* x2, int k_split, const float* w, const float* bias, float* y,
                      float* y_act, const float* residual, const float* row_scale, int rows_per_sample, int M, int N,
@@ -1119,6 +1239,58 @@
     return CSWIN_OK;
 }
 
+int cswin_linear_fwd_skip(const float* x, const float* x2, int k_split, const float* w, const float* bias, float* y, float* y_act,
+                          const float* residual, const float* row_scale, int rows_per_sample, int M, int N, int K, int precision,
+                          int io_bf16, const int* order, int nsamples, void* stream) {
+    RowMap rm;
+    int rc = row_map_checked(&rm, "linear_fwd_skip", order, nsamples, rows_per_sample, M, precision, io_bf16, x2 != nullptr, false);
+    if (rc) return rc;
+    CSWIN_REQUIRE(x && w && y && N > 0 && K > 0, CSWIN_ERR_SHAPE, "linear_fwd_skip: bad arguments M=%d N=%d K=%d", M, N, K);
+    CSWIN_REQUIRE(!(y_act && residual), CSWIN_ERR_UNSUPPORTED, "linear_fwd_skip: activation and residual epilogues are exclusive");
+    Epilogue e = plain_epilogue(y, N);
+    e.bias = bias;
+    e.Cact = y_act; e.ldact = N;
+    e.residual = residual; e.ldres = N;
+    e.row_scale = row_scale; e.rows_per_sample = rows_per_sample;
+    CSWIN_REQUIRE(K % 4 == 0 && aligned16(x) && aligned16(w) && epilogue_vec_ok(e, N), CSWIN_ERR_ALIGN,
+                  "linear_fwd_skip: a sample order needs N, K multiples of 4 and 16-B aligned operands");
+    const PlainSrc A = {x, K, M, K, nullptr, 1, 0}, B = {w, K, N, K, nullptr, 1, 0};
+    hipStream_t st = (hipStream_t)stream;
+    if (y_act) launch_gemm<true, true, 4, EPI_ACT, false>(A, B, e, M, N, K, 1, one_split(K), 0, st, &rm);
+    else if (residual) launch_gemm<true, true, 4, EPI_RES, false>(A, B, e, M, N, K, 1, one_split(K), 0, st, &rm);
+    else launch_gemm<true, true, 4, EPI_PLAIN, false>(A, B, e, M, N, K, 1, one_split(K), 0, st, &rm);
+    CSWIN_LAUNCH_CHECK();
+    return CSWIN_OK;
+}
+
+int cswin_linear_bwd_data_skip(const float* dy, const float* w, float* dx, float* dx2, int k_split, const float* gelu_pre,
+                               const float* row_scale, int rows_per_sample, const float* add, int M, int N, int K, int precision,
+                               int io_bf16, const int* order, int nsamples, void* stream) {
+    RowMap rm;
+    int rc = row_map_checked(&rm, "linear_bwd_data_skip", order, nsamples, rows_per_sample, M, precision, io_bf16, dx2 != nullptr, add != nullptr);
+    if (rc) return rc;
+    CSWIN_REQUIRE(dy && w && dx && N > 0 && K > 0, CSWIN_ERR_SHAPE, "linear_bwd_data_skip: bad arguments");
+    Epilogue e = plain_epilogue(dx, K);
+    e.gelu_pre = gelu_pre; e.ldpre = K;
+    e.row_scale = row_scale; e.rows_per_sample = rows_per_sample;
+    CSWIN_REQUIRE(N % 4 == 0 && aligned16(dy) && aligned16(w) && epilogue_vec_ok(e, K), CSWIN_ERR_ALIGN,
+                  "linear_bwd_data_skip: a sample order needs N, K multiples of 4 and 16-B aligned operands");
+    const PlainSrc A = {dy, N, M, N, nullptr, 1, 0}, B = {w, K, N, K, nullptr, 1, 0};
+    hipStream_t st = (hipStream_t)stream;
+    if (gelu_pre) launch_gemm<true, false, 4, EPI_GELUBWD, false>(A, B, e, M, K, N, 1, one_split(N), 0, st, &rm);
+    else launch_gemm<true, false, 4, EPI_PLAIN, false>(A, B, e, M, K, N, 1, one_split(N), 0, st, &rm);
+    CSWIN_LAUNCH_CHECK();
+    return CSWIN_OK;
+}
+
+int cswin_drop_path_order(const float* u, const float* keep, float* scales, int* order, int rows, int B, void* stream) {
+    CSWIN_REQUIRE(u && keep && scales && order && rows > 0, CSWIN_ERR_SHAPE, "drop_path_order: bad arguments");
+    CSWIN_REQUIRE(B >= 1 && B <= MASK_MAX_SAMPLES, CSWIN_ERR_SHAPE, "drop_path_order: 1..%d samples", MASK_MAX_SAMPLES);
+    hipLaunchKernelGGL(drop_path_order_kernel, dim3(rows), dim3(64), 0, (hipStream_t)stream, u, keep, scales, order, B);
+    CSWIN_LAUNCH_CHECK();
+    return CSWIN_OK;
+}
+
 size_t cswin_linear_bwd_weight_workspace(int M, int N, int K) { return WgradSlabs::bytes(M, N, K); }
 
 int cswin_linear_bwd_weight(const float* dy, const float* x, const float* x2, int k_split, const float* row_scale,
@@ -1164,6 +1336,16 @@
                                  const int* nsamples, void* stream) {
     CSWIN_REQUIRE(dy && w && dx && M > 0 && N > 0 && K > 0, CSWIN_ERR_SHAPE, "linear_bwd_tail: bad data-gradient arguments");
     return wgrad_batch_impl(d, n, deferred, TailExtras{"linear_bwd_tail", dy, w, dx, M, N, K, pending, npending, skip, nsamples}, stream);
+}
+
+int cswin_linear_bwd_tail_skip(const float* dy, const float* w, float* dx, int M, int N, int K, const cswin_wgrad_desc* d, int n,
+                               cswin_reduce_job* deferred, const cswin_reduce_job* pending, int npending, const float* const* skip,
+                               const int* nsamples, const int* order, int order_samples, void* stream) {
+    CSWIN_REQUIRE(dy && w && dx && M > 0 && N > 0 && K > 0, CSWIN_ERR_SHAPE, "linear_bwd_tail_skip: bad data-gradient arguments");
+    CSWIN_REQUIRE(order, CSWIN_ERR_SHAPE, "linear_bwd_tail_skip: the order must list 1..%d samples", MASK_MAX_SAMPLES);
+    CSWIN_REQUIRE(d && n >= 1 && n <= WGRAD_BATCH, CSWIN_ERR_SHAPE, "linear_bwd_tail_skip: 1..%d weight-gradient problems", WGRAD_BATCH);
+    return wgrad_batch_impl(d, n, deferred, TailExtras{"linear_bwd_tail_skip", dy, w, dx, M, N, K, pending, npending, skip, nsamples, order, order_samples},
+                            stream);
 }
 
 int cswin_conv_tok_fwd(const float* x, const float* w_perm, const float* bias, float* y, int B, int H, int W, int Cin,
diff --git a/cswin_unet_amd/csrc/gemm_epilogue.h b/cswin_unet_amd/csrc/gemm_epilogue.h
--- a/cswin_unet_amd/csrc/gemm_epilogue.h
+++ b/cswin_unet_amd/csrc/gemm_epilogue.h
@@ -34,9 +34,10 @@
 constexpr int EP_LD = 36;
 constexpr int EP_WAVE_FLOATS = 32 * EP_LD;
 
-template <int EPI, int FM, int FN, bool PRE16 = false, bool FDIV = false>
+template <int EPI, int FM, int FN, bool PRE16 = false, bool FDIV = false, bool MAPPED = false>
 __device__ __forceinline__ void run_epilogue(const Epilogue& e, f32x16 (&acc)[FM][FN], int M, int N, int mb, int nb,
-                                             int lane, float* wbuf, bool vec, unsigned m_hw = 0, unsigned m_w2 = 0) {
+                                             int lane, float* wbuf, bool vec, unsigned m_hw = 0, unsigned m_w2 = 0,
+                                             const int* ord = nullptr, int kept_rows = 0, int map_rps = 1, unsigned map_magic = 0) {
     const int li = lane & 31, lh = lane >> 5;
     const int rrow = lane >> 3, rcol = (lane & 7) * 4;
     const bool has_rs = e.row_scale != nullptr;
@@ -65,11 +66,30 @@
                 f32x4 v[4], aux[4];
                 u32x2 aux16[4];
                 float rs[4];
+                int pm[4];
 #pragma unroll
                 for (int p = 0; p < 4; ++p) {
                     const int m = mb + i * 32 + rrow + 8 * p;
                     const bool ok = m < M && n < N;
                     v[p] = *reinterpret_cast<const f32x4*>(&wbuf[(rrow + 8 * p) * EP_LD + rcol]);
+                    if constexpr (MAPPED) {
+                        pm[p] = m;
+                        int smp = 0;
+                        if (ord && m < M) {
+                            const int j = fdiv1(m, map_magic);
+                            smp = ord[j];
+                            pm[p] = smp * map_rps + (m - j * map_rps);
+                        }
+                        const bool dropped = ord && m >= kept_rows;
+                        rs[p] = (has_rs && ok) ? e.row_scale[ord ? smp : m / e.rows_per_sample] : 1.0f;
+                        if (EPI == EPI_RES || EPI == EPI_GELUBWD) {
+                            const float* ap = EPI == EPI_RES ? e.residual : e.gelu_pre;
+                            const long ld = EPI == EPI_RES ? e.ldres : e.ldpre;
+                            aux[p] = f32x4{0.f, 0.f, 0.f, 0.f};
+                            if (ok && !(EPI == EPI_GELUBWD && dropped)) aux[p] = *reinterpret_cast<const f32x4*>(ap + (long)pm[p] * ld + n);
+                        }
+                        continue;
+                    }
                     rs[p] = (has_rs && ok) ? e.row_scale[m / e.rows_per_sample] : 1.0f;
                     if (EPI == EPI_RES || EPI == EPI_GELUBWD) {
                         const float* ap = EPI == EPI_RES ? e.residual : e.gelu_pre;
@@ -93,6 +113,19 @@
                         for (int c = 0; c < 4; ++c) o[c] *= gelu_grad_f(pre[c]);
                     }
                     if (has_rs) o *= rs[p];
+                    if constexpr (MAPPED) {
+                        static_assert(EPI != EPI_SPLIT2 && !PRE16 && !FDIV, "row-mapped launches: one fp32 output matrix");
+                        if (EPI == EPI_RES && ord && m >= kept_rows) o = f32x4{0.f, 0.f, 0.f, 0.f};
+                        if (EPI == EPI_RES) o += aux[p];
+                        *reinterpret_cast<f32x4*>(e.C + (long)pm[p] * e.ldc + n) = o;
+                        if (EPI == EPI_ACT) {
+                            f32x4 a;
+#pragma unroll
+                            for (int c = 0; c < 4; ++c) a[c] = gelu_f(o[c]);
+                            *reinterpret_cast<f32x4*>(e.Cact + (long)pm[p] * e.ldact + n) = a;
+                        }
+                        continue;
+                    }
                     if (EPI == EPI_RES) o += aux[p];
                     if (EPI == EPI_SPLIT2 && n >= e.col_split)
                         *reinterpret_cast<f32x4*>(e.C2 + (long)m * e.ldc2 + (n - e.col_split)) = o;
diff --git a/cswin_unet_amd/networks/cswin_unet.py b/cswin_unet_amd/networks/cswin_unet.py
--- a/cswin_unet_amd/networks/cswin_unet.py
+++ b/cswin_unet_amd/networks/cswin_unet.py
@@ -88,6 +88,12 @@
                 return preset[0], preset[1]
             return dp.sample_scale(x.shape[0], x.device), dp.sample_scale(x.shape[0], x.device)
         return None, None
+
+    def _keep_orders(self, rs1):
+        preset = getattr(self, "_dp_preset", None)
+        if preset and len(preset) == 4 and preset[2] is not None and rs1 is preset[0]:
+            return preset[2], preset[3]
+        return None
 
     def forward(self, x):
         B, L, C = x.shape
@@ -107,7 +113,8 @@
             return self.mlp(ops.layer_norm(x, n2.weight, n2.bias, n2.eps), residual=x, row_scale=rs2)
         return ops.cswin_block(x, self.patches_resolution, self.split_size, [m.idx for m in a], [m.num_heads for m in a],
                                a[0].scale, self.norm1, self.qkv, self.proj, self.norm2, self.mlp.fc1, self.mlp.fc2,
-                               [m.get_v.weight for m in a], [m.get_v.bias for m in a], rs1, rs2, attn_drop=ad)
+                               [m.get_v.weight for m in a], [m.get_v.bias for m in a], rs1, rs2, attn_drop=ad,
+                               orders=self._keep_orders(rs1))
 
 
 def img2windows(img, H_sp, W_sp):
@@ -275,9 +282,15 @@
                                  device=device)[:, None]
             self._dp_keep = cache
         keep = cache
-        scales = (torch.rand(keep.shape[0], batch, device=device) < keep).to(torch.float32) / keep
+        u = torch.rand(keep.shape[0], batch, device=device)
+        if u.is_cuda and batch <= ops.MAX_MASK_SAMPLES:
+            scales, order = ops.drop_path_order(u, keep)
+        else:
+            scales, order = (u < keep).to(torch.float32) / keep, None
         for i, b in enumerate(live):
             b._dp_preset = [scales[2 * i], scales[2 * i + 1]]
+            if order is not None:
+                b._dp_preset += [order[2 * i], order[2 * i + 1]]
 
     def forward_features(self, x, pe_weight=None):
         self._predraw_drop_path(x.shape[0], x.device)
diff --git a/cswin_unet_amd/ops.py b/cswin_unet_amd/ops.py
--- a/cswin_unet_amd/ops.py
+++ b/cswin_unet_amd/ops.py
@@ -186,23 +186,31 @@
     return ptr(w), 0
 
 
-def _linear_fwd(x, w, b, N, *, dtype=torch.float32, gelu=False, x2=None, residual=None, row_scale=None):
+def _linear_fwd(x, w, b, N, *, dtype=torch.float32, gelu=False, x2=None, residual=None, row_scale=None, order=None):
     pw, w16 = w if isinstance(w, tuple) else (ptr(w), 0)
     K1 = x.shape[-1]
     K = K1 + (x2.shape[-1] if x2 is not None else 0)
     y = torch.empty(x.shape[:-1] + (N,), dtype=dtype, device=x.device)
     y_act = torch.empty_like(y) if gelu else None
-    call("cswin_linear_fwd", ptr(x), ptr(x2), K1 if x2 is not None else 0, pw, ptr(b), ptr(y), ptr(y_act), ptr(residual), ptr(row_scale),
-         _rows_per_sample(x), x.numel() // K1, N, K, precision(), _stored16(x, y) | w16, stream())
+    args = (ptr(x), ptr(x2), K1 if x2 is not None else 0, pw, ptr(b), ptr(y), ptr(y_act), ptr(residual), ptr(row_scale),
+            _rows_per_sample(x), x.numel() // K1, N, K, precision(), _stored16(x, y) | w16)
+    if order is not None:
+        call("cswin_linear_fwd_skip", *args, ptr(order), x.shape[0], stream())
+    else:
+        call("cswin_linear_fwd", *args, stream())
     return (y, y_act) if gelu else y
 
 
-def _linear_bwd_data(dy, w, dx, *, dx2=None, gelu_pre=None, row_scale=None, add=None):
+def _linear_bwd_data(dy, w, dx, *, dx2=None, gelu_pre=None, row_scale=None, add=None, order=None):
     pw, w16 = w if isinstance(w, tuple) else (ptr(w), 0)
     N, K1 = dy.shape[-1], dx.shape[-1]
     K = K1 + (dx2.shape[-1] if dx2 is not None else 0)
-    call("cswin_linear_bwd_data", ptr(dy), pw, ptr(dx), ptr(dx2), K1 if dx2 is not None else 0, ptr(gelu_pre), ptr(row_scale),
-         _rows_per_sample(dy), ptr(add), dy.numel() // N, N, K, precision(), _stored16(dy, dx, None, gelu_pre) | w16, stream())
+    args = (ptr(dy), pw, ptr(dx), ptr(dx2), K1 if dx2 is not None else 0, ptr(gelu_pre), ptr(row_scale),
+            _rows_per_sample(dy), ptr(add), dy.numel() // N, N, K, precision(), _stored16(dy, dx, None, gelu_pre) | w16)
+    if order is not None:
+        call("cswin_linear_bwd_data_skip", *args, ptr(order), dy.shape[0], stream())
+    else:
+        call("cswin_linear_bwd_data", *args, stream())
 
 
 def _linear_bwd_weight(dy, x, dw, db, slab=None, *, x2=None, row_scale=None):
@@ -218,6 +226,16 @@
 
 
 MAX_MASK_SAMPLES = 256
+
+
+def drop_path_order(u, keep):
+    u, keep = dev_f32(u, "DropPath draws"), dev_f32(keep, "keep probabilities")
+    rows, B = u.shape
+    assert keep.numel() == rows and B <= MAX_MASK_SAMPLES
+    scales = torch.empty_like(u)
+    order = torch.empty(rows, 1 + B, dtype=torch.int32, device=u.device)
+    call("cswin_drop_path_order", ptr(u), ptr(keep), ptr(scales), ptr(order), rows, B, stream())
+    return scales, order
 
 
 def _fill_wgrad(d, dy, x, row_scale, dw, dbias, workspace, ws_bytes):
@@ -482,7 +500,7 @@
 class _CSWinBlock(Function):
 
     @staticmethod
-    def forward(ctx, x, reso, split, idx, heads, scale, eps1, eps2, rs1, rs2, drop, g1, b1, wqkv, bqkv, wp, bp, g2, b2, w1, bb1,
+    def forward(ctx, x, reso, split, idx, heads, scale, eps1, eps2, rs1, rs2, orders, drop, g1, b1, wqkv, bqkv, wp, bp, g2, b2, w1, bb1,
                 w2, bb2, *lepe):
         x = dev_f32(x, "block input")
         B, L, C = x.shape
@@ -498,15 +516,19 @@
         E16 = lambda *shape: torch.empty(*shape, dtype=t16, device=dev)
         sq, sp, s1, s2 = (_wsrc(w) if s16 else w for w in (wqkv, wp, w1, w2))
         attn = (reso, split, tuple(idx), tuple(heads), scale, drop, ATTN_MFMA16 if s16 else ATTN_FP32)
+        o1 = o2 = None
+        if orders is not None and precision() == 0 and B <= MAX_MASK_SAMPLES and C % 4 == 0 and w1.shape[0] % 4 == 0:
+            o1, o2 = orders
+        ctx.orders = (o1, o2)
         h1, m1, r1 = _layernorm_fwd(x, g1, b1, eps1, t16)
-        qkv = _linear_fwd(h1, sq, bqkv, 3 * C, dtype=t16)
+        qkv = _linear_fwd(h1, sq, bqkv, 3 * C, dtype=t16, order=o1)
         att, lse = E16(B, L, C), torch.empty(B, sum(heads), L, dtype=torch.float32, device=dev)
         att0 = E16(B, L, C) if any(ctx.needs_input_grad) else None
         _attn_fwd(qkv, lw, lb, att, att0, lse, *attn)
-        x1 = _linear_fwd(att, sp, bp, C, residual=x, row_scale=rs1)
+        x1 = _linear_fwd(att, sp, bp, C, residual=x, row_scale=rs1, order=o1)
         h2, m2, r2 = _layernorm_fwd(x1, g2, b2, eps2, t16)
-        pre, act = _linear_fwd(h2, s1, bb1, w1.shape[0], dtype=t16, gelu=True)
-        y = _linear_fwd(act, s2, bb2, C, residual=x1, row_scale=rs2)
+        pre, act = _linear_fwd(h2, s1, bb1, w1.shape[0], dtype=t16, gelu=True, order=o2)
+        y = _linear_fwd(act, s2, bb2, C, residual=x1, row_scale=rs2, order=o2)
         ctx.save_for_backward(x, m1, r1, h1, qkv, lse, att, att0, x1, m2, r2, h2, pre, act, rs1, rs2, g1, wqkv, wp, g2, w1, w2, *lw, *lb)
         ctx.attn = attn
         ctx.keys = _param_keys(g1, b1, wqkv, bqkv, wp, bp, g2, b2, w1, bb1, w2, bb2, *lepe)
@@ -519,6 +541,7 @@
         nb = len(lwb) // 2
         lw, lb = lwb[:nb], lwb[nb:]
         dy = dev_f32(dy)
+        o1, o2 = ctx.orders
         B, L, C = x.shape
         M, Hd = B * L, w1.shape[0]
         dev, h = x.device, lib()
@@ -533,7 +556,7 @@
         dy16 = _twin_take(dy) if s16 else None
         dyg = dy16 if dy16 is not None else dy
         dpre = torch.empty_like(pre)
-        _linear_bwd_data(dyg, s2, dpre, gelu_pre=pre, row_scale=rs2)
+        _linear_bwd_data(dyg, s2, dpre, gelu_pre=pre, row_scale=rs2, order=o2)
         wg = (WgradDesc * 4)()
         kg1, kb1, kwqkv, kbqkv, kwp, kbp, kg2, kb2, kw1, kbb1, kw2, kbb2, *klepe = ctx.keys
         G = lambda key, *shape: _pass.grad(key, shape, dev)
@@ -542,13 +565,13 @@
         dw1, db1 = G(kw1, *w1.shape), G(kbb1, Hd)
         _fill_wgrad(wg[1], dpre, h2, None, dw1, db1, wsp[1], sizes[1])
         dh2 = torch.empty_like(x)
-        _linear_bwd_data(dpre, s1, dh2)
+        _linear_bwd_data(dpre, s1, dh2, order=o2)
         dx1, dg2, dbt2 = torch.empty_like(x), G(kg2, C), G(kb2, C)
         dx1_16 = torch.empty_like(x, dtype=torch.bfloat16) if s16 else None
         _layernorm_bwd(dh2, x1, m2, r2, g2, dx1, dg2, dbt2, (wsp[2], sizes[2], _job_ptr(jobs, 2)), dres=dy, dx16=dx1_16)
         dx1g = dx1_16 if s16 else dx1
         datt = dh2
-        _linear_bwd_data(dx1g, sp, datt, row_scale=rs1)
+        _linear_bwd_data(dx1g, sp, datt, row_scale=rs1, order=o1)
         dwp, dbp = G(kwp, *wp.shape), G(kbp, C)
         _fill_wgrad(wg[2], dx1g, att, rs1, dwp, dbp, wsp[3], sizes[3])
         dqkv = torch.empty_like(qkv)
@@ -568,7 +591,10 @@
             masks = (rs2, rs2, rs1, rs1) if B <= MAX_MASK_SAMPLES else (None,) * 4
             if any(m is not None for m in masks):
                 skip = (ctypes.c_void_p * 4)(*[m.data_ptr() if m is not None else None for m in masks])
-                call("cswin_linear_bwd_tail_masked", *tail, skip, _int_array([B] * 4), stream())
+                if o1 is not None:
+                    call("cswin_linear_bwd_tail_skip", *tail, skip, _int_array([B] * 4), ptr(o1), B, stream())
+                else:
+                    call("cswin_linear_bwd_tail_masked", *tail, skip, _int_array([B] * 4), stream())
             else:
                 call("cswin_linear_bwd_tail", *tail, stream())
         else:
@@ -582,13 +608,14 @@
         if s16:
             _twin_put(dx, dx16)
         _pass.reduce(jobs, (ws, aws))
-        grads = (dx, None, None, None, None, None, None, None, None, None, None, dg1, dbt1, dwqkv, dbqkv, dwp, dbp, dg2, dbt2, dw1, db1,
+        grads = (dx, None, None, None, None, None, None, None, None, None, None, None, dg1, dbt1, dwqkv, dbqkv, dwp, dbp, dg2, dbt2, dw1, db1,
                  dw2, db2)
         return grads + tuple(d.view(d.shape[0], 1, 3, 3) for d in dlw) + tuple(dlb)
 
 
-def cswin_block(x, reso, split, idx, heads, scale, norm1, qkv, proj, norm2, fc1, fc2, lepe_w, lepe_b, rs1=None, rs2=None, attn_drop=0.0):
-    return _CSWinBlock.apply(x, reso, split, tuple(idx), tuple(heads), scale, norm1.eps, norm2.eps, rs1, rs2, _attn_drop(attn_drop),
+def cswin_block(x, reso, split, idx, heads, scale, norm1, qkv, proj, norm2, fc1, fc2, lepe_w, lepe_b, rs1=None, rs2=None, attn_drop=0.0,
+                orders=None):
+    return _CSWinBlock.apply(x, reso, split, tuple(idx), tuple(heads), scale, norm1.eps, norm2.eps, rs1, rs2, orders, _attn_drop(attn_drop),
                              norm1.weight, norm1.bias, qkv.weight, qkv.bias, proj.weight, proj.bias, norm2.weight,
                              norm2.bias, fc1.weight, fc1.bias, fc2.weight, fc2.bias, *lepe_w, *lepe_b)
 
diff --git a/include/cswin_hip.h b/include/cswin_hip.h
--- a/include/cswin_hip.h
+++ b/include/cswin_hip.h
@@ -81,6 +81,16 @@
 int cswin_linear_bwd_tail_masked(const float* dy, const float* w, float* dx, int M, int N, int K, const cswin_wgrad_desc* problems, int n,
                                  cswin_reduce_job* deferred, const cswin_reduce_job* pending, int npending, const float* const* skip,
                                  const int* nsamples, void* stream);
+int cswin_drop_path_order(const float* u, const float* keep, float* scales, int* order, int rows, int B, void* stream);
+int cswin_linear_fwd_skip(const float* x, const float* x2, int k_split, const float* w, const float* bias, float* y,
+                          float* y_act, const float* residual, const float* row_scale, int rows_per_sample, int M, int N,
+                          int K, int precision, int io_bf16, const int* order, int nsamples, void* stream);
+int cswin_linear_bwd_data_skip(const float* dy, const float* w, float* dx, float* dx2, int k_split, const float* gelu_pre,
+                               const float* row_scale, int rows_per_sample, const float* add, int M, int N, int K,
+                               int precision, int io_bf16, const int* order, int nsamples, void* stream);
+int cswin_linear_bwd_tail_skip(const float* dy, const float* w, float* dx, int M, int N, int K, const cswin_wgrad_desc* problems, int n,
+                               cswin_reduce_job* deferred, const cswin_reduce_job* pending, int npending, const float* const* skip,
+                               const int* nsamples, const int* order, int nsamples_order, void* stream);
 int cswin_rows_sum_multi(const cswin_reduce_job* jobs, int njobs, void* stream);
 
 int cswin_conv_tok_fwd(const float* x, const float* w_perm, const float* bias, float* y, int B, int H, int W, int Cin,
```
